# francescovidaich964/TensorNetworkForML

Hardware: AMD Instinct MI355X
Metric: sweep-steps/sec, 28x28 MNIST-shaped, bond=20, batch=5000 per GPU (higher is better)
Workload: dtype f32; 1 GPU; c3: N=784 sites, D=2, L=2, bond 20, batch 5000/GPU, softmax+full_cross_ent, trunc=fixed, L2_flag=True; pass = hand-over of one of 4 staged batches + forward + 783-step sweep; global_batch=5000, sweep_steps_per_pass=783, parallelism=dp1, distinct_batches=4

## Files before the change

include/tnml.h:

```cpp
#ifndef TNML_H
#define TNML_H

#include <stddef.h>
#include <stdint.h>

#ifdef __cplusplus
extern "C" {
#endif

typedef struct tnml_ctx tnml_ctx;

typedef enum {
  TNML_OK = 0,
  TNML_ERR_ARG = -1,
  TNML_ERR_STATE = -2,
  TNML_ERR_HIP = -3,
  TNML_ERR_NOGPU = -4,
  TNML_ERR_COMM = -5,
  TNML_ERR_SHAPE = -6,
  TNML_ERR_NONFINITE = -7
} tnml_status;

enum { TNML_ACT_LINEAR = 0, TNML_ACT_SIGMOID = 1, TNML_ACT_SOFTMAX = 2 };
enum { TNML_LOSS_MSE = 0, TNML_LOSS_CROSS_ENTROPY = 1, TNML_LOSS_FULL_CROSS_ENT = 2 };
// ... 10 lines not shown
};

const char *tnml_last_error(void);
const char *tnml_version(void);
int tnml_device_count(void);

int tnml_create(tnml_ctx **out, int N, int D, int L, int Mmax, int b_capacity, int device);
int tnml_destroy(tnml_ctx *ctx);
int tnml_synchronize(tnml_ctx *ctx);

int tnml_comm_unique_id(void *uid128);
int tnml_comm_init(tnml_ctx *ctx, int rank, int nranks, const void *uid128);
int tnml_set_comm_overlap(tnml_ctx *ctx, int on);
int tnml_comm_probe(tnml_ctx *ctx, int n_floats, int reps, double *us_per_allreduce);

int tnml_set_cores(tnml_ctx *ctx, const float *cores_flat, size_t n_floats, const int32_t *bond,
                   int l_pos);
int tnml_cores_size(tnml_ctx *ctx, size_t *n_floats);
int tnml_get_cores(tnml_ctx *ctx, float *cores_flat, size_t capacity, int32_t *bond, int *l_pos);
int tnml_scale_cores(tnml_ctx *ctx, double factor);
int tnml_get_core_slots(tnml_ctx *ctx, float *slots, size_t slots_capacity, float *label_buffer, size_t label_capacity);

int tnml_set_input(tnml_ctx *ctx, const float *X, const int32_t *y, int b);
int tnml_stage_batch(tnml_ctx *ctx, int slot, const float *X, const int32_t *y, int b);
int tnml_select_batch(tnml_ctx *ctx, int slot);
int tnml_set_labels(tnml_ctx *ctx, const int32_t *y, int b);

int tnml_forward(tnml_ctx *ctx, float *f_out);
int tnml_f_absmax(tnml_ctx *ctx, double *out);
int tnml_forward_logabsmax(tnml_ctx *ctx, double *out);
int tnml_set_f(tnml_ctx *ctx, const float *f);
int tnml_get_f(tnml_ctx *ctx, float *f_out);

int tnml_sweep(tnml_ctx *ctx, int left_dir, int n_steps, int first_of_sweep, float lr,
               float weight_dec, int l2_flag, int act_fn, int loss_fn, float T, int trunc_policy,
               float *metrics_out, float *f_out);

int tnml_update_B(tnml_ctx *ctx, const float *B_canon, int left_dir, float lr, float weight_dec, int l2_flag,
                  int act_fn, int loss_fn, float T, double *Bnew_canon, size_t capacity, float *metrics2);
int tnml_l2_term(tnml_ctx *ctx, const float *B_canon, int left_dir, float weight_dec, double *loss,
                 double *grad_canon, size_t capacity);
int tnml_svd_split(tnml_ctx *ctx, const float *mat, int rows, int cols, int m, float *US, float *SVh,
                   double *sigma);

int tnml_predict(tnml_ctx *ctx, const float *X, int b, float *f_out);

int tnml_set_any_position(tnml_ctx *ctx, int on);

enum { TNML_DATASET_FEATURES = 0, TNML_DATASET_PIXELS = 1 };
int tnml_dataset_attach(tnml_ctx *ctx, const float *data, const int32_t *labels, int n, int N, int D, int form);
int tnml_dataset_detach(tnml_ctx *ctx);
int tnml_dataset_size(tnml_ctx *ctx);
int tnml_select_indices(tnml_ctx *ctx, const int32_t *idx, int b);
int tnml_predict_indices(tnml_ctx *ctx, const int32_t *idx, int b, float *f_out);
int tnml_eval_indices(tnml_ctx *ctx, const int32_t *idx, int b, int act_fn, float T, double *out3);
int tnml_resident_metrics(tnml_ctx *ctx, int act_fn, float T, double *out3);
int tnml_dataset_read(tnml_ctx *ctx, const int32_t *idx, int b, float *X_out);

enum { TNML_WRT_FEATURES = 0, TNML_WRT_PIXELS = 1 };
int tnml_input_grad(tnml_ctx *ctx, const float *X, int b, const float *cot, float *grad_out, float *cf_out);
int tnml_input_grad_indices(tnml_ctx *ctx, const int32_t *idx, int b, const float *cot, int wrt, float *grad_out, float *cf_out);
int tnml_set_input_grad_chunk(tnml_ctx *ctx, int samples);

int tnml_core_grad(tnml_ctx *ctx, const float *X, int b, const float *cot, float *grad_flat, size_t capacity, float *cf_out);
int tnml_core_grad_indices(tnml_ctx *ctx, const int32_t *idx, int b, const float *cot, float *grad_flat, size_t capacity, float *cf_out);
int tnml_set_core_grad_chunk(tnml_ctx *ctx, int samples);

enum { TNML_OPT_SGD = 0, TNML_OPT_ADAM = 1 };
int tnml_optim_config(tnml_ctx *ctx, int kind, double momentum, double beta1, double beta2, double eps, int clip);
int tnml_optim_reset(tnml_ctx *ctx);
int tnml_gd_train_indices(tnml_ctx *ctx, const int32_t *idx, int n, int batch, float lr, float weight_dec, int act_fn, int loss_fn,
                          float T, double *metrics_out);
int tnml_gd_step(tnml_ctx *ctx, const float *X, const int32_t *y, int b, float lr, float weight_dec, int act_fn, int loss_fn, float T,
                 double *metrics3);

int tnml_set_chain_scaling(tnml_ctx *ctx, int on);
int tnml_predict_scaled(tnml_ctx *ctx, const float *X, int b, float *mant_out, int32_t *expo_out);

int tnml_set_svd_stop(tnml_ctx *ctx, double stop2);

int tnml_set_step_pipeline(tnml_ctx *ctx, int on);

int tnml_set_persistent(tnml_ctx *ctx, int on);

int tnml_set_sync_interval(tnml_ctx *ctx, int n_steps);

int tnml_set_narrow_path(tnml_ctx *ctx, int force_large);

int tnml_set_flag_handoffs(tnml_ctx *ctx, int on);

int tnml_set_chain_path(tnml_ctx *ctx, int force_plain);

int tnml_set_trunc_threshold(tnml_ctx *ctx, double threshold);

int tnml_activation(tnml_ctx *ctx, int act_fn, int loss_fn, float T, int input_is_activated,
                    float *act_out, float *lossder_out);

int tnml_get_env(tnml_ctx *ctx, int side, int site, float *out, size_t capacity, int *m);
int tnml_debug_enable(tnml_ctx *ctx, int on);
int tnml_get_step_debug(tnml_ctx *ctx, int what, double *out, size_t capacity, size_t *n);
int tnml_l_pos(tnml_ctx *ctx);
int tnml_batch(tnml_ctx *ctx);

int tnml_timer_start(tnml_ctx *ctx);
int tnml_marker(tnml_ctx *ctx, int id);
int tnml_timer_stop(tnml_ctx *ctx, double *elapsed_ms);
int tnml_profile_enable(tnml_ctx *ctx, int on);
int tnml_profile_get(tnml_ctx *ctx, int which, double *ms, long long *launches);
int tnml_profile_reset(tnml_ctx *ctx);
int tnml_get_counters(tnml_ctx *ctx, double *out8);
int tnml_svd_stats(tnml_ctx *ctx, int reset, double *out3);
int tnml_svd_stats_ex(tnml_ctx *ctx, int reset, double *out, int capacity);

int tnml_orthogonalize(tnml_ctx *ctx, double rank_tol, int32_t *bond_out, double *log_norm_out);
int tnml_compress(tnml_ctx *ctx, int m_max, double threshold, double rank_tol, int32_t *bond_out, double *sigma_out,
                  double *discarded_out, double *log_norm_out);
int tnml_bond_spectra(tnml_ctx *ctx, double rank_tol, int32_t *rank_out, double *sigma_out, double *log_norm_out);

int tnml_trunc_rank(int policy, int left_dir, int p, int N, int ml, int D, int mr, int L, int M);

#ifdef __cplusplus
}
#endif
#endif
```

tensornetworkforml_amd/_hip.py:

```python
import ctypes as C
import os

import numpy as np

_HERE = os.path.dirname(os.path.abspath(__file__))
LIB_PATH = os.environ.get('TNML_LIB', os.path.join(_HERE, 'libtnml_hip.so'))

ACT = {'linear': 0, 'sigmoid': 1, 'softmax': 2}
LOSS = {'MSE': 0, 'cross_entropy': 1, 'full_cross_ent': 2}
TRUNC = {'reference': 0, 'fixed': 1, 'adaptive': 2}
SIDE_LEFT, SIDE_RIGHT = 0, 1
DATASET_FORM = {'features': 0, 'pixels': 1}
WRT = {'features': 0, 'pixels': 1}
OPTIM = {'sgd': 0, 'adam': 1}
DBG = {'B': 0, 'dB_raw': 1, 'B_new': 2, 'sigma': 3, 'scalars': 4, 'L2_grad': 5}

SYMBOLS = [
    'tnml_last_error', 'tnml_version', 'tnml_device_count', 'tnml_create', 'tnml_destroy',
    'tnml_synchronize', 'tnml_comm_unique_id', 'tnml_comm_init', 'tnml_set_cores', 'tnml_cores_size',
    'tnml_get_cores', 'tnml_scale_cores', 'tnml_set_input', 'tnml_set_labels', 'tnml_forward', 'tnml_forward_logabsmax', 'tnml_f_absmax',
    'tnml_set_f', 'tnml_get_f', 'tnml_sweep', 'tnml_activation', 'tnml_get_env', 'tnml_debug_enable',
    'tnml_get_step_debug', 'tnml_l_pos', 'tnml_batch', 'tnml_timer_start', 'tnml_timer_stop',
    'tnml_profile_enable', 'tnml_profile_get', 'tnml_profile_reset', 'tnml_svd_stats', 'tnml_trunc_rank',
    'tnml_update_B', 'tnml_l2_term', 'tnml_svd_split', 'tnml_set_svd_stop', 'tnml_set_narrow_path', 'tnml_predict', 'tnml_set_trunc_threshold',
    'tnml_set_sync_interval', 'tnml_set_step_pipeline', 'tnml_stage_batch', 'tnml_select_batch', 'tnml_get_counters',
    'tnml_svd_stats_ex', 'tnml_set_persistent', 'tnml_set_chain_path', 'tnml_marker', 'tnml_set_comm_overlap', 'tnml_comm_probe', 'tnml_set_flag_handoffs',
    'tnml_dataset_attach', 'tnml_dataset_detach', 'tnml_dataset_size', 'tnml_select_indices', 'tnml_predict_indices', 'tnml_eval_indices',
    'tnml_resident_metrics', 'tnml_dataset_read', 'tnml_set_any_position',
    'tnml_input_grad', 'tnml_input_grad_indices', 'tnml_set_input_grad_chunk',
    'tnml_core_grad', 'tnml_core_grad_indices', 'tnml_set_core_grad_chunk',
    'tnml_optim_config', 'tnml_optim_reset', 'tnml_gd_train_indices', 'tnml_gd_step', 'tnml_get_core_slots',
    'tnml_orthogonalize', 'tnml_compress', 'tnml_bond_spectra',
    'tnml_set_chain_scaling', 'tnml_predict_scaled',
]


class TnmlError(RuntimeError):
    def __init__(self, code, msg):
        super().__init__('tnml error %d: %s' % (code, msg))
        self.code = code


_lib = None


def lib():
    global _lib
    if _lib is None:
        if not os.path.exists(LIB_PATH):
            raise RuntimeError(
                "%s is missing: build the HIP extension first (python -c 'import __graft_entry__ as g; "
                "g.build()' or make -C tensornetworkforml_amd/csrc).  There is no CPU fallback." % LIB_PATH)
        L = C.CDLL(LIB_PATH)
        L.tnml_last_error.restype = C.c_char_p
        L.tnml_version.restype = C.c_char_p
        f32p, i32p, f64p = C.POINTER(C.c_float), C.POINTER(C.c_int32), C.POINTER(C.c_double)
        vp = C.c_void_p
        L.tnml_create.argtypes = [C.POINTER(vp), C.c_int, C.c_int, C.c_int, C.c_int, C.c_int, C.c_int]
        L.tnml_destroy.argtypes = [vp]
        L.tnml_synchronize.argtypes = [vp]
        L.tnml_comm_unique_id.argtypes = [vp]
        L.tnml_comm_init.argtypes = [vp, C.c_int, C.c_int, vp]
        L.tnml_set_cores.argtypes = [vp, f32p, C.c_size_t, i32p, C.c_int]
        L.tnml_cores_size.argtypes = [vp, C.POINTER(C.c_size_t)]
        L.tnml_get_cores.argtypes = [vp, f32p, C.c_size_t, i32p, C.POINTER(C.c_int)]
        L.tnml_scale_cores.argtypes = [vp, C.c_double]
        L.tnml_set_input.argtypes = [vp, f32p, i32p, C.c_int]
        L.tnml_set_labels.argtypes = [vp, i32p, C.c_int]
        L.tnml_forward.argtypes = [vp, f32p]
        L.tnml_f_absmax.argtypes = [vp, f64p]
        L.tnml_forward_logabsmax.argtypes = [vp, f64p]
        L.tnml_set_f.argtypes = [vp, f32p]
        L.tnml_get_f.argtypes = [vp, f32p]
        L.tnml_sweep.argtypes = [vp, C.c_int, C.c_int, C.c_int, C.c_float, C.c_float, C.c_int, C.c_int,
                                 C.c_int, C.c_float, C.c_int, f32p, f32p]
        L.tnml_activation.argtypes = [vp, C.c_int, C.c_int, C.c_float, C.c_int, f32p, f32p]
        L.tnml_get_env.argtypes = [vp, C.c_int, C.c_int, f32p, C.c_size_t, C.POINTER(C.c_int)]
        L.tnml_debug_enable.argtypes = [vp, C.c_int]
        L.tnml_get_step_debug.argtypes = [vp, C.c_int, f64p, C.c_size_t, C.POINTER(C.c_size_t)]
        L.tnml_l_pos.argtypes = [vp]
        L.tnml_batch.argtypes = [vp]
        L.tnml_timer_start.argtypes = [vp]
        L.tnml_timer_stop.argtypes = [vp, f64p]
        L.tnml_profile_enable.argtypes = [vp, C.c_int]
        L.tnml_profile_get.argtypes = [vp, C.c_int, f64p, C.POINTER(C.c_longlong)]
        L.tnml_profile_reset.argtypes = [vp]
        L.tnml_svd_stats.argtypes = [vp, C.c_int, f64p]
        L.tnml_svd_stats_ex.argtypes = [vp, C.c_int, f64p, C.c_int]
        L.tnml_set_persistent.argtypes = [vp, C.c_int]
        L.tnml_trunc_rank.argtypes = [C.c_int] * 9
        L.tnml_update_B.argtypes = [vp, f32p, C.c_int, C.c_float, C.c_float, C.c_int, C.c_int, C.c_int, C.c_float,
                                    f64p, C.c_size_t, f32p]
        L.tnml_l2_term.argtypes = [vp, f32p, C.c_int, C.c_float, f64p, f64p, C.c_size_t]
        L.tnml_set_svd_stop.argtypes = [vp, C.c_double]
        L.tnml_set_narrow_path.argtypes = [vp, C.c_int]
        L.tnml_set_chain_path.argtypes = [vp, C.c_int]
        L.tnml_set_any_position.argtypes = [vp, C.c_int]
        L.tnml_marker.argtypes = [vp, C.c_int]
        L.tnml_set_comm_overlap.argtypes = [vp, C.c_int]
        L.tnml_set_flag_handoffs.argtypes = [vp, C.c_int]
        L.tnml_comm_probe.argtypes = [vp, C.c_int, C.c_int, C.POINTER(C.c_double)]
        L.tnml_predict.argtypes = [vp, f32p, C.c_int, f32p]
        L.tnml_set_trunc_threshold.argtypes = [vp, C.c_double]
        L.tnml_set_sync_interval.argtypes = [vp, C.c_int]
        L.tnml_set_step_pipeline.argtypes = [vp, C.c_int]
        L.tnml_stage_batch.argtypes = [vp, C.c_int, f32p, i32p, C.c_int]
        L.tnml_select_batch.argtypes = [vp, C.c_int]
        L.tnml_get_counters.argtypes = [vp, f64p]
        L.tnml_svd_split.argtypes = [vp, f32p, C.c_int, C.c_int, C.c_int, f32p, f32p, f64p]
        L.tnml_dataset_attach.argtypes = [vp, f32p, i32p, C.c_int, C.c_int, C.c_int, C.c_int]
        L.tnml_dataset_detach.argtypes = [vp]
        L.tnml_dataset_size.argtypes = [vp]
        L.tnml_select_indices.argtypes = [vp, i32p, C.c_int]
        L.tnml_predict_indices.argtypes = [vp, i32p, C.c_int, f32p]
        L.tnml_eval_indices.argtypes = [vp, i32p, C.c_int, C.c_int, C.c_float, f64p]
        L.tnml_resident_metrics.argtypes = [vp, C.c_int, C.c_float, f64p]
        L.tnml_dataset_read.argtypes = [vp, i32p, C.c_int, f32p]
        L.tnml_input_grad.argtypes = [vp, f32p, C.c_int, f32p, f32p, f32p]
        L.tnml_input_grad_indices.argtypes = [vp, i32p, C.c_int, f32p, C.c_int, f32p, f32p]
        L.tnml_set_input_grad_chunk.argtypes = [vp, C.c_int]
        L.tnml_core_grad.argtypes = [vp, f32p, C.c_int, f32p, f32p, C.c_size_t, f32p]
        L.tnml_core_grad_indices.argtypes = [vp, i32p, C.c_int, f32p, f32p, C.c_size_t, f32p]
        L.tnml_set_core_grad_chunk.argtypes = [vp, C.c_int]
        L.tnml_optim_config.argtypes = [vp, C.c_int, C.c_double, C.c_double, C.c_double, C.c_double, C.c_int]
        L.tnml_optim_reset.argtypes = [vp]
        L.tnml_get_core_slots.argtypes = [vp, f32p, C.c_size_t, f32p, C.c_size_t]
        L.tnml_gd_train_indices.argtypes = [vp, i32p, C.c_int, C.c_int, C.c_float, C.c_float, C.c_int, C.c_int, C.c_float, f64p]
        L.tnml_gd_step.argtypes = [vp, f32p, i32p, C.c_int, C.c_float, C.c_float, C.c_int, C.c_int, C.c_float, f64p]
        L.tnml_orthogonalize.argtypes = [vp, C.c_double, i32p, f64p]
        L.tnml_compress.argtypes = [vp, C.c_int, C.c_double, C.c_double, i32p, f64p, f64p, f64p]
        L.tnml_bond_spectra.argtypes = [vp, C.c_double, i32p, f64p, f64p]
        L.tnml_set_chain_scaling.argtypes = [vp, C.c_int]
        L.tnml_predict_scaled.argtypes = [vp, f32p, C.c_int, f32p, i32p]
        _lib = L
    return _lib


def device_count():
    return int(lib().tnml_device_count())


def _chk(rc):
    if rc != 0:
        raise TnmlError(rc, lib().tnml_last_error().decode('utf-8', 'replace'))


def _f32(a):
    return np.ascontiguousarray(a, dtype=np.float32)


def _ptr(a, ctype):
    return a.ctypes.data_as(C.POINTER(ctype))


def trunc_rank(policy, left_dir, p, N, ml, D, mr, L, M):
    return int(lib().tnml_trunc_rank(TRUNC[policy], int(left_dir), p, N, ml, D, mr, L, M))


def comm_unique_id():
    buf = (C.c_ubyte * 128)()
    _chk(lib().tnml_comm_unique_id(C.cast(buf, C.c_void_p)))
    return bytes(buf)


def core_shapes(bond, l_pos, D, L):
    N = len(bond) + 1
    shapes = []
    for i in range(N):
        ml = 1 if i == 0 else int(bond[i - 1])
        mr = 1 if i == N - 1 else int(bond[i])
        shapes.append((ml, D, mr, L) if i == l_pos else (ml, D, mr))
    return shapes
# ... 282 lines not shown

    def set_f(self, f):
        f = _f32(f)
        assert f.shape == (self.L, self.b)
        _chk(lib().tnml_set_f(self._h, _ptr(f, C.c_float)))

    def get_f(self):
        f = np.empty((self.L, self.b), dtype=np.float32)
        _chk(lib().tnml_get_f(self._h, _ptr(f, C.c_float)))
        return f

    def sweep(self, left_dir, n_steps, first_of_sweep, lr, weight_dec, L2_flag, act_fn, loss_fn, T, trunc,
              want_metrics=True, want_f=True):
        met = np.empty((n_steps, 2), dtype=np.float32) if want_metrics else None
        f = np.empty((self.L, self.b), dtype=np.float32) if want_f else None
        _chk(lib().tnml_sweep(self._h, int(bool(left_dir)), int(n_steps), int(bool(first_of_sweep)), float(lr),
                              float(weight_dec), int(bool(L2_flag)), ACT[act_fn], LOSS[loss_fn], float(T),
                              TRUNC[trunc], _ptr(met, C.c_float) if want_metrics else None,
                              _ptr(f, C.c_float) if want_f else None))
        return met, f

    def update_B(self, B, left_dir, lr, weight_dec, L2_flag, act_fn, loss_fn, T):
        shape = None
        bp = None
        if B is not None:
            B = _f32(B)
            shape = B.shape
            bp = _ptr(B, C.c_float)
        cap = 4 * max(self.M, self.D * self.L) ** 2 * self.D * self.D * self.L
        out = np.empty(cap, dtype=np.float64)
        met = np.empty(2, dtype=np.float32)
        _chk(lib().tnml_update_B(self._h, bp, int(bool(left_dir)), float(lr), float(weight_dec), int(bool(L2_flag)),
                                 ACT[act_fn], LOSS[loss_fn], float(T), _ptr(out, C.c_double), out.size,
                                 _ptr(met, C.c_float)))
        return (out[:int(np.prod(shape))].reshape(shape).copy() if shape is not None else out), met

    def l2_term(self, B, left_dir, weight_dec):
        B = _f32(B)
        grad = np.empty(B.size, dtype=np.float64)
        loss = C.c_double()
        _chk(lib().tnml_l2_term(self._h, _ptr(B, C.c_float), int(bool(left_dir)), float(weight_dec), C.byref(loss),
                                _ptr(grad, C.c_double), grad.size))
        return loss.value, grad.reshape(B.shape)

    def svd_split(self, mat, m):
        mat = _f32(mat)
        rows, cols = mat.shape
        US = np.empty((rows, int(m)), dtype=np.float32)
        SVh = np.empty((int(m), cols), dtype=np.float32)
        sig = np.empty(min(rows, cols), dtype=np.float64)
        _chk(lib().tnml_svd_split(self._h, _ptr(mat, C.c_float), rows, cols, int(m), _ptr(US, C.c_float),
                                  _ptr(SVh, C.c_float), _ptr(sig, C.c_double)))
        return US, SVh, sig

    def activation(self, act_fn, loss_fn, T, want_act=True, want_der=False, input_is_activated=False):
        a = np.empty((self.L, self.b), dtype=np.float32) if want_act else None
        d = np.empty((self.L, self.b), dtype=np.float32) if want_der else None
        _chk(lib().tnml_activation(self._h, ACT[act_fn], LOSS[loss_fn], float(T), int(bool(input_is_activated)),
                                   _ptr(a, C.c_float) if want_act else None,
                                   _ptr(d, C.c_float) if want_der else None))
        return a, d

    def loss_derivative_of_activated(self, act_fn, loss_fn, T):
        return self.activation(act_fn, loss_fn, T, want_act=False, want_der=True, input_is_activated=True)[1]

    def get_env(self, side, site):
        out = np.empty(self.b * max(self.M, self.D * self.L) * 2, dtype=np.float32)
        m = C.c_int()
        _chk(lib().tnml_get_env(self._h, int(side), int(site), _ptr(out, C.c_float), out.size, C.byref(m)))
        return out[:self.b * m.value].reshape(self.b, m.value).copy()

    def set_svd_stop(self, stop2):
        _chk(lib().tnml_set_svd_stop(self._h, float(stop2)))

    def set_trunc_threshold(self, threshold):
        _chk(lib().tnml_set_trunc_threshold(self._h, float(threshold)))

    def set_step_pipeline(self, on):
        _chk(lib().tnml_set_step_pipeline(self._h, int(on)))

    def set_persistent(self, on=True):
        _chk(lib().tnml_set_persistent(self._h, int(on)))

    def set_sync_interval(self, n_steps):
        _chk(lib().tnml_set_sync_interval(self._h, int(n_steps)))

    def set_comm_overlap(self, on=True):
        _chk(lib().tnml_set_comm_overlap(self._h, int(bool(on))))

    def comm_probe(self, n_floats, reps=200):
        v = C.c_double()
        _chk(lib().tnml_comm_probe(self._h, int(n_floats), int(reps), C.byref(v)))
        return v.value

    def set_flag_handoffs(self, on=True):
        _chk(lib().tnml_set_flag_handoffs(self._h, int(bool(on))))

    def set_chain_path(self, force_plain):
        _chk(lib().tnml_set_chain_path(self._h, int(bool(force_plain))))

    def set_any_position(self, on=True):
        _chk(lib().tnml_set_any_position(self._h, int(bool(on))))

    def set_chain_scaling(self, on=True):
        _chk(lib().tnml_set_chain_scaling(self._h, int(on)))

    def set_narrow_path(self, force_large):
        _chk(lib().tnml_set_narrow_path(self._h, int(bool(force_large))))

    def debug_enable(self, on=True):
        _chk(lib().tnml_debug_enable(self._h, int(on)))

    def step_debug(self, what):
        cap = max(4 * max(self.M, self.D * self.L) ** 2 * self.D * self.D * self.L + 64, 512)
        out = np.empty(cap, dtype=np.float64)
        n = C.c_size_t()
        _chk(lib().tnml_get_step_debug(self._h, DBG[what], _ptr(out, C.c_double), out.size, C.byref(n)))
        return out[:n.value].copy()

    @property
    def l_pos(self):
        return int(lib().tnml_l_pos(self._h))

    def synchronize(self):
        _chk(lib().tnml_synchronize(self._h))

    def marker(self, marker_id):
        _chk(lib().tnml_marker(self._h, int(marker_id)))

    def timer_start(self):
        _chk(lib().tnml_timer_start(self._h))

    def timer_stop(self):
        ms = C.c_double()
        _chk(lib().tnml_timer_stop(self._h, C.byref(ms)))
        return ms.value

    def profile_enable(self, on=True):
        _chk(lib().tnml_profile_enable(self._h, int(on)))

    def profile_reset(self):
        _chk(lib().tnml_profile_reset(self._h))

    def svd_stats(self, reset=False):
        out = (C.c_double * 4)()
        _chk(lib().tnml_svd_stats_ex(self._h, int(bool(reset)), out, 4))
        self.cholesky_steps = out[3]
        return out[0], out[1], out[2]

    def counters(self):
        out = (C.c_double * 8)()
        _chk(lib().tnml_get_counters(self._h, out))
        keys = ('sweep_steps', 'algorithmic_bytes', 'algorithmic_flops', 'forwards', 'forward_bytes', 'launches', 'pipelined_steps', 'sweep_device_ms')
        return dict(zip(keys, [float(v) for v in out]))

    def profile_get(self, which):
        ms, n = C.c_double(), C.c_longlong()
        _chk(lib().tnml_profile_get(self._h, int(which), C.byref(ms), C.byref(n)))
        return ms.value, n.value
```

tensornetworkforml_amd/csrc/kernels_narrow.hip:

```cpp
#include "tnml_internal.h"
#include "jacobi_device.h"
#include "small_gemm_device.h"
#include "wide_pipe_device.h"

namespace tnml {

__device__ inline double wave_sum_f64(double v) {
  v += dpp_f64<0xB1>(v);
  v += dpp_f64<0x4E>(v);
  v += dpp_f64<0x141>(v);
  v += dpp_f64<0x140>(v);
  const double r0 = wave_read_f64(v, 0), r1 = wave_read_f64(v, 16), r2 = wave_read_f64(v, 32), r3 = wave_read_f64(v, 48);
  return (r0 + r1) + (r2 + r3);
}

template <int BUF>
__device__ inline void block_sum3(double &a, double &b, double &c, double *scratch) {
  const int lane = threadIdx.x & 63, wave = threadIdx.x >> 6, nw = blockDim.x >> 6;
  double *s = scratch + BUF * 64;
  a = wave_sum_f64(a); b = wave_sum_f64(b); c = wave_sum_f64(c);
  if (lane == 0) { s[wave] = a; s[16 + wave] = b; s[32 + wave] = c; }
  lds_barrier();
  const int w = lane & 15;
  double ta = w < nw ? s[w] : 0.0, tb = w < nw ? s[16 + w] : 0.0, tc = w < nw ? s[32 + w] : 0.0;
// ... 32 lines not shown
  k.dVs = d; d += (size_t)ne * m;
  float *f = (float *)d;
  k.fB = f; f += Bs;
  k.fBp = f; f += Bs + (size_t)(D * h < D * g * L ? D * h : D * g * L) + 4;
  k.sLab = f; f += (size_t)h * D * s * L;
  k.sPl = f; f += (size_t)s * D * g;
  k.sCb = f; f += (size_t)r * m;
  f += (size_t)m * c;
  int *ip = (int *)f;
  k.sOrd = ip; ip += ne;
  k.sFlag = ip; ip += 8;
  k.sPi = ip; ip += ne;
  k.sPiInv = ip; ip += ne;
  k.sTail = (float *)ip; ip += kMetricSlots;
  k.sWave = ip; ip += 16;
  k.bytes = (size_t)((unsigned char *)ip - base);
  return k;
}

size_t narrow_lds_bytes(int h, int g, int s, int L, int m) {
  alignas(16) static unsigned char origin[16];
  return narrow_carve(origin, h, g, s, L, m).bytes + 16;
}

__device__ inline void narrow_helper_block(const NarrowParams &p, unsigned char *smem_raw) {
  const int tid = threadIdx.x;
  const int h = p.h, g = p.g, s = p.s, L = p.L, Bs = p.bsize;
  const int blk = blockIdx.x - 1;
  const unsigned long long t_start = __builtin_amdgcn_s_memrealtime();
  if (blk < p.nred) {
    float *part = (float *)smem_raw;
    const int el = tid & 63, chunk = tid >> 6;
    const int e = blk * 64 + el, n = Bs + kMetricSlots;
    const int per = (p.nslabs + 15) / 16;
    const int k0 = chunk * per, k1 = min(p.nslabs, k0 + per);
    float a0 = 0.f, a1 = 0.f;
    if (e < n) {
      int kk = k0;
      for (; kk + 2 <= k1; kk += 2) {
        a0 += p.slabs[(size_t)kk * p.slab_stride + e];
        a1 += p.slabs[(size_t)(kk + 1) * p.slab_stride + e];
      }
      if (kk < k1) a0 += p.slabs[(size_t)kk * p.slab_stride + e];
    }
    part[chunk * 64 + el] = a0 + a1;
    __syncthreads();
    if (chunk == 0 && e < n) {
      float t = 0.f;
#pragma unroll
      for (int c = 0; c < 16; ++c) t += part[c * 64 + el];
      __hip_atomic_store(p.red_out + e, t, __ATOMIC_RELAXED, __HIP_MEMORY_SCOPE_AGENT);
    }
  } else {
    PrepParams q{};
    q.lab = p.lab; q.pl = p.pl; q.Nh = p.Nh; q.Ng = p.Ng; q.h = h; q.g = g; q.s = s; q.L = L; q.l2_flag = p.l2_flag;
    q.prepB = p.prepB; q.prepG = p.prepG;
    q.nparts = p.pipe ? (p.wait_count - p.nred) / (kD * kD) : 1;
    prep_slice_block(q, blk - p.nred, smem_raw, true);
  }
  asm volatile("s_waitcnt vmcnt(0)" ::: "memory");
  __syncthreads();
  if (tid == 0) {
    if (p.stamps && p.counters) {
      atomicMin(p.counters + (blk < p.nred ? 4 : 5), t_start);
      atomicMax(p.counters + (blk < p.nred ? 6 : 7), __builtin_amdgcn_s_memrealtime());
    }
    __hip_atomic_fetch_add(p.sync, 1u, __ATOMIC_RELAXED, __HIP_MEMORY_SCOPE_AGENT);
  }
}

struct StepArgs : NarrowParams {
  __device__ __forceinline__ StepArgs(const NarrowParams &q) : NarrowParams(q) {}
  static constexpr int persist = 0;
};

template <class T>
struct RecField {
  const __attribute__((address_space(4))) T *a;
  __device__ __forceinline__ operator T() const { return *a; }
};
template <class T>
__device__ __forceinline__ RecField<T> rec_field(const T *field) { return RecField<T>{(const __attribute__((address_space(4))) T *)field}; }

struct PersistArgs {
  int L, h, g, s, m, bsize, l2_flag;
  float lr, wd;
  const double *Nh;
  int persist_off, Mcap;
  const unsigned *pready; unsigned pwant;
  unsigned *abort_flag;
  const float *zred; int zsize;
  const float *prepRaw; float *prepB; double *prepG;
  float *Bnew;
  unsigned *flag; unsigned token;
  double chol_thr, svd_stop2;
  double *stamps;
  RecField<float *> out_behind, out_ahead;
  RecField<int> ob_s_h, ob_s_d, ob_s_m, oa_s_m, oa_s_d, oa_s_g, write_ahead;
  RecField<double *> Nh_new, Apub;
  RecField<float *> metrics;
  RecField<unsigned long long *> counters;
  RecField<int *> status;
  RecField<unsigned *> aflag, coreflag;
  RecField<unsigned> coretoken;
  static constexpr int D = kD, fused = 0, prep_ready = 0, pipe = 1, persist = 1, z_first = 0, z_rows = 0, stop_after_update = 0, left_dir = 0;
  static constexpr int wait_count = 0;
  static constexpr unsigned zpoll_want = 0, done_val = 0;
  static constexpr double trunc_thr = 0.0;
  static constexpr const float *red = nullptr, *Bdirect = nullptr;
  static constexpr const double *Ng = nullptr;
  static constexpr double *dbg = nullptr;
  static constexpr int *m_out = nullptr;
  unsigned *sync = nullptr, *done_flag = nullptr;
  const unsigned *zpoll_flag = nullptr;
  CoreView lab{}, pl{}, zcore{};

  __device__ __forceinline__ explicit PersistArgs(const NarrowParams *rec)
      : out_behind(rec_field(&rec->out_behind)), out_ahead(rec_field(&rec->out_ahead)),
        ob_s_h(rec_field(&rec->ob_s_h)), ob_s_d(rec_field(&rec->ob_s_d)), ob_s_m(rec_field(&rec->ob_s_m)),
        oa_s_m(rec_field(&rec->oa_s_m)), oa_s_d(rec_field(&rec->oa_s_d)), oa_s_g(rec_field(&rec->oa_s_g)),
        write_ahead(rec_field(&rec->write_ahead)), Nh_new(rec_field(&rec->Nh_new)), Apub(rec_field(&rec->Apub)),
        metrics(rec_field(&rec->metrics)), counters(rec_field(&rec->counters)), status(rec_field(&rec->status)),
        aflag(rec_field(&rec->aflag)), coreflag(rec_field(&rec->coreflag)), coretoken(rec_field(&rec->coretoken)) {
    const auto *r = (const __attribute__((address_space(4))) NarrowParams *)rec;
    L = r->L; h = r->h; g = r->g; s = r->s; m = r->m; bsize = r->bsize; l2_flag = r->l2_flag;
    lr = r->lr; wd = r->wd; Nh = r->Nh; persist_off = r->persist_off; Mcap = r->Mcap;
    pready = r->pready; pwant = r->pwant; abort_flag = r->abort_flag; zred = r->zred; zsize = r->zsize;
    prepRaw = r->prepRaw; prepB = r->prepB; prepG = r->prepG; Bnew = r->Bnew; flag = r->flag; token = r->token;
    chol_thr = r->chol_thr; svd_stop2 = r->svd_stop2; stamps = r->stamps;
  }
};

template <class NP>
__device__ __forceinline__ bool narrow_body(const NP &p, unsigned char *smem_raw) {
  __builtin_assume(p.h >= 1 && p.h <= 64 && p.g >= 1 && p.g <= 64 && p.s >= 1 && p.s <= 128 && p.m >= 1 && p.m <= 64);
  __builtin_assume(p.L >= 1 && p.L <= 2048 && p.bsize >= 1 && p.bsize <= 8192);
  const NarrowCarve k = narrow_carve(smem_raw, p.h, p.g, p.s, p.L, p.m);
  int tid_step = threadIdx.x;
  if (p.persist) {
    asm volatile("" : "+v"(tid_step));
    __builtin_assume(tid_step >= 0 && tid_step < kNarrowThreads);
  }
  const int tid = tid_step, NT = kNarrowThreads;
  const int wave_u = __builtin_amdgcn_readfirstlane(tid >> 6);
  const int D = kD, h = p.h, g = p.g, s = p.s, L = p.L, m = p.m, Bs = p.bsize;
  auto ldred = [&](int e) -> float {
    return (p.fused && !p.pipe) ? __hip_atomic_load(p.red + e, __ATOMIC_RELAXED, __HIP_MEMORY_SCOPE_AGENT) : p.red[e];
  };
  if (p.zpoll_flag) {
    if (tid == 0) {
      bool ok = false;
      for (int spin = 0; spin < (1 << 22) && !ok; ++spin) {
        ok = (int)(__hip_atomic_load(p.zpoll_flag, __ATOMIC_RELAXED, __HIP_MEMORY_SCOPE_AGENT) - p.zpoll_want) >= 0;
        if (!ok) __builtin_amdgcn_s_sleep(16);
      }
      if (!ok) atomicOr(p.status, 64);
    }
    __syncthreads();
    __builtin_amdgcn_fence(__ATOMIC_ACQUIRE, "agent");
  }
  if (p.pipe && !p.persist && tid == 0)
    for (int i = 0; i < kMetricSlots; ++i) k.sTail[i] = p.zred[p.zsize + i];
  auto ldtail = [&](int i) -> float { return p.pipe ? k.sTail[i] : ldred(p.bsize + i); };
  const int r = D * h, c = D * g * L;
  const bool short_rows = (r <= c);
  const int n = short_rows ? r : c, ne = n + (n & 1), len = short_rows ? c : r;

  unsigned long long t_c0 = 0, t_r0 = 0, t_c1 = 0, t_c2 = 0, t_c2b = 0, t_c2c = 0;
  unsigned long long t_p[5] = {0, 0, 0, 0, 0};
#define TNML_STAMP(i) if (p.stamps && tid == 0) t_p[i] = __builtin_amdgcn_s_memtime()
  if (p.stamps && tid == 0) { t_c0 = __builtin_amdgcn_s_memtime(); t_r0 = __builtin_amdgcn_s_memrealtime(); }
  const int RWz = kD * kD * p.g * p.L;
  const bool fast0 = p.pipe && !p.persist && (size_t)p.z_rows * RWz + (size_t)p.z_rows * h <= (size_t)((float *)k.sOrd - k.fBp) &&
                     Bs <= 8 * NT && p.z_rows * RWz <= 16 * NT && p.z_rows * h <= 4 * NT && h * h <= 2 * NT && g * g <= 2 * NT;
  const PersistLds PL = persist_lds(smem_raw + p.persist_off, p.Mcap);
  float *sRaw = k.fBp;
  if (p.persist) {
    if (tid == 0) {
      const int bad = spin_wait_ge(p.pready, p.pwant, p.abort_flag, 1);
      if (bad == 1) { atomicOr(p.status, 4); __hip_atomic_store(p.abort_flag, 1u, __ATOMIC_RELAXED, __HIP_MEMORY_SCOPE_AGENT); }
      k.sFlag[3] = bad;
    }
    lds_barrier();
    if (k.sFlag[3]) return true;
    if (p.stamps && tid == 0) { p.stamps[20] = (double)(__builtin_amdgcn_s_memtime() - t_c0); p.stamps[28] = (double)(t_r0 & ((1ull << 40) - 1)); p.stamps[29] = (double)(__builtin_amdgcn_s_memrealtime() & ((1ull << 40) - 1)); }
    if (tid < kMetricSlots) k.sTail[tid] = ld_sc1(p.zred + p.zsize + tid);
    for (int e = tid; e < h * h; e += NT) k.dNh[e] = p.Nh ? PL.Nh[e] : 1.0;
    const __amdgpu_buffer_rsrc_t rR = sc1_rsrc(p.prepRaw), rB = sc1_rsrc(p.prepB), rG = sc1_rsrc(p.prepG);
    tn_uvec4 qr[2], qb[2], qg[4];
#pragma unroll
    for (int u = 0; u < 2; ++u) { const int e = 4 * (tid + u * NT); if (e < Bs) { qr[u] = ld_sc1_b128(rR, (unsigned)e * 4u); qb[u] = ld_sc1_b128(rB, (unsigned)e * 4u); } }
#pragma unroll
    for (int u = 0; u < 4; ++u) { const int e = 2 * (tid + u * NT); if (p.l2_flag && e < Bs) qg[u] = ld_sc1_b128(rG, (unsigned)e * 8u); }
#pragma unroll
    for (int u = 0; u < 2; ++u) { const int e = 4 * (tid + u * NT); if (e < Bs) { *reinterpret_cast<tn_uvec4 *>(sRaw + e) = qr[u]; *reinterpret_cast<tn_uvec4 *>(k.fB + e) = qb[u]; } }
#pragma unroll
    for (int u = 0; u < 4; ++u) { const int e = 2 * (tid + u * NT); if (p.l2_flag && e < Bs) *reinterpret_cast<tn_uvec4 *>(k.dG + e) = qg[u]; }
  }
  float *sZ = k.fBp, *sZc = sZ + (size_t)p.z_rows * RWz;
  if (fast0) {
    const int zr = p.z_rows, nz = p.z_first ? 0 : zr * RWz, nzc = p.z_first ? 0 : zr * h;
    const float *zc = p.zcore.base;
    float4 rz[4], rb[2];
    double2 rg[4];
    float rc[4];
    double rnh[2], rng[2];
#pragma unroll
    for (int u = 0; u < 4; ++u) { const int e = 4 * (tid + u * NT); rz[u] = e < nz ? *reinterpret_cast<const float4 *>(p.zred + e) : make_float4(0.f, 0.f, 0.f, 0.f); }
// ... 172 lines not shown
    sumB += fabs(bv);
    sumD += fabs(dv);
  }
  block_sum3<0>(sumB, sumD, l2, k.dRed);

  double factor = (double)p.lr;
  if (sumD > sumB) factor = (double)p.lr * (sumB / sumD);
  const bool bad = !isfinite(sumD) || !isfinite(sumB);
  if ((c & 3) == 0) {
    const float inv_c = 1.0f / (float)c;
    const __amdgpu_buffer_rsrc_t rN = sc1_rsrc(p.Bnew);
    for (int e = 4 * tid; e < Bs; e += 4 * NT) {
      const int row = (int)(((float)e + 0.5f) * inv_c), x = e - row * c;
      const float4 b4 = *reinterpret_cast<const float4 *>(k.fB + e);
      const double2 g01 = *reinterpret_cast<const double2 *>(k.dG + e), g23 = *reinterpret_cast<const double2 *>(k.dG + e + 2);
      float4 v;
      v.x = (float)((double)b4.x + factor * g01.x); v.y = (float)((double)b4.y + factor * g01.y);
      v.z = (float)((double)b4.z + factor * g23.x); v.w = (float)((double)b4.w + factor * g23.y);
      *reinterpret_cast<float4 *>(k.fB + e) = v;
      float *bp = k.fBp + row * (c + 1) + x;
      bp[0] = v.x; bp[1] = v.y; bp[2] = v.z; bp[3] = v.w;
      if (p.flag) {
        tn_uvec4 o; o.x = __float_as_uint(v.x); o.y = __float_as_uint(v.y); o.z = __float_as_uint(v.z); o.w = __float_as_uint(v.w);
        st_sc1_b128(rN, (unsigned)(4 * e), o);
      } else {
        *reinterpret_cast<float4 *>(p.Bnew + e) = v;
      }
      if (p.dbg) { double *dd = p.dbg + 2 * (size_t)Bs + e; dd[0] = v.x; dd[1] = v.y; dd[2] = v.z; dd[3] = v.w; }
    }
  } else {
    for (int row = wave_u; row < r; row += NT >> 6)
      for (int x = tid & 63; x < c; x += 64) {
        const int e = row * c + x;
        const float v = (float)((double)k.fB[e] + factor * k.dG[e]);
        k.fB[e] = v;
        k.fBp[row * (c + 1) + x] = v;
        if (p.flag) st_sc1(p.Bnew + e, v); else p.Bnew[e] = v;
        if (p.dbg) p.dbg[2 * (size_t)Bs + e] = (double)v;
      }
  }
  if (p.flag) asm volatile("s_waitcnt vmcnt(0)" ::: "memory");
  if (tid == 0) {
    if (bad) atomicOr(p.status, 1);
    if (p.dbg) {
      double *sc = p.dbg + 4 * (size_t)Bs + kDbgSigma;
      sc[0] = (double)p.wd * l2;
      sc[1] = sumB;
      sc[2] = sumD;
    }
  }
  lds_barrier();
  if (p.flag && tid == 0) __hip_atomic_store(p.flag, p.token, __ATOMIC_RELAXED, __HIP_MEMORY_SCOPE_AGENT);
  if (p.stop_after_update) {
    if (tid == 0 && p.metrics) {
      const double cnt = (double)ldtail(3);
      const double inv = cnt > 0 ? 1.0 / cnt : 0.0;
      p.metrics[0] = (float)((double)ldtail(0) * inv);
      p.metrics[1] = (float)((double)ldtail(1) * inv / (double)L);
    }
    return false;
  }

  TNML_STAMP(3);
  double *G0 = k.Z, *G1 = k.Z + ne * ne, *V0 = k.Z + 2 * ne * ne;
  double g_tr = 0.0, g_dg2 = 0.0, g_off2 = 0.0;
  auto gram_phase = [&]() {
    double a_tr = 0.0, a_dg2 = 0.0, a_off2 = 0.0;
    double *P0 = G0, *P1 = G1, *P2 = V0, *P3 = k.Z + 3 * ne * ne;
    const int lane = tid & 63, wave = wave_u, rr = lane & 15, qq = lane >> 4;
    const int tm = (n + 15) >> 4, ntile_g = (tm * (tm + 1)) >> 1;
    const int gshift = ntile_g * 4 <= (NT >> 6) ? 2 : (ntile_g * 2 <= (NT >> 6) ? 1 : (ntile_g <= (NT >> 6) ? 0 : 2));
    const int gsplit = 1 << gshift;
    const int kchunk = ((len + gsplit - 1) / gsplit + 3) & ~3;
    const int wave_s = wave;
    const float *Wb = short_rows ? k.fBp : k.fB;
    const int rs = short_rows ? c + 1 : 1, cs = short_rows ? 1 : c;
    const int nitems = ntile_g * gsplit;
    for (int item = wave_s; item < nitems; item += NT >> 6) {
      const int ks = item & (gsplit - 1);
      int t = item >> gshift, ti = 0, rowlen = tm;
      while (t >= rowlen) { t -= rowlen; ++ti; --rowlen; }
      const int tj = ti + t;
      const int i0 = ti << 4, j0 = tj << 4;
      const bool va = i0 + rr < n, vb = j0 + rr < n;
      const float *pa = Wb + min(i0 + rr, n - 1) * rs, *pb = Wb + min(j0 + rr, n - 1) * rs;
      const int k_lo = ks * kchunk, k_hi = min(len, k_lo + kchunk);
      dvec4 acc0 = {0.0, 0.0, 0.0, 0.0}, acc1 = {0.0, 0.0, 0.0, 0.0};
      for (int k0 = k_lo; k0 < k_hi; k0 += 16) {
        float fa[4], fb[4];
#pragma unroll
        for (int u = 0; u < 4; ++u) {
          const int kc = min(k0 + 4 * u + qq, k_hi - 1) * cs;
          fa[u] = pa[kc];
          fb[u] = pb[kc];
        }
#pragma unroll
        for (int u = 0; u < 4; ++u) {
          const bool vk = k0 + 4 * u + qq < k_hi;
          const double av = (va && vk) ? (double)fa[u] : 0.0, bv = (vb && vk) ? (double)fb[u] : 0.0;
          if (k0 + 4 * u < k_hi) {
            if (u & 1) acc1 = __builtin_amdgcn_mfma_f64_16x16x4f64(av, bv, acc1, 0, 0, 0);
            else acc0 = __builtin_amdgcn_mfma_f64_16x16x4f64(av, bv, acc0, 0, 0, 0);
          }
        }
      }
      const dvec4 acc = acc0 + acc1;
      const int j = j0 + rr;
      double *Pk = P0 + (size_t)ks * ne * ne;
#pragma unroll
      for (int reg = 0; reg < 4; ++reg) {
        const int i = i0 + qq + 4 * reg;
        if (i < ne && j < ne) Pk[i * ne + j] = (i < n && j < n) ? acc[reg] : 0.0;
      }
    }
    lds_barrier();
    for (int i = wave_u; i < ne; i += NT >> 6)
      for (int j = tid & 63; j < ne; j += 64)
        if (i <= j) {
          const int e = i * ne + j;
          double v = P0[e];
          if (gsplit > 1) v += P1[e];
          if (gsplit > 2) v = (v + P2[e]) + P3[e];
          P0[e] = v;
          if (i < j) { G0[j * ne + i] = v; a_off2 += 2.0 * v * v; }
          else { a_tr += v; a_dg2 += v * v; }
        }
    g_tr = a_tr; g_dg2 = a_dg2; g_off2 = a_off2;
  };
  gram_phase();
  const int np = ne / 2;
  for (int pos = tid; pos < ne; pos += NT) {
    const int kq = pos >> 1;
    int nxt;
    if (pos & 1) nxt = (kq == 0) ? (np > 1 ? 2 : 1) : 2 * (kq - 1) + 1;
    else nxt = (kq == 0) ? 0 : (kq == np - 1 ? 2 * kq + 1 : 2 * (kq + 1));
    k.sPi[pos] = nxt;
    k.sPiInv[nxt] = pos;
  }
  TNML_STAMP(4);
  double tr = 0.0, off2 = 0.0;
  int sc_exp = 0;
  auto scale_phase = [&]() {
    block_sum3<1>(g_tr, g_dg2, g_off2, k.dRed);
    tr = g_tr; off2 = g_off2;
    sc_exp = (tr > 0.0 && isfinite(tr)) ? __builtin_amdgcn_frexp_exp(tr) : 0;
    for (int i = wave_u; i < ne; i += NT >> 6)
      for (int j = tid & 63; j < ne; j += 64) G0[i * ne + j] = __builtin_amdgcn_ldexp(G0[i * ne + j], -sc_exp);
    lds_barrier();
  };
  scale_phase();
  const bool chol_possible = p.chol_thr > 0.0 && n > 4;

  constexpr int kVR = 2;
  const int gpw = 64 / np;
  const int vr = ((np + gpw - 1) / gpw + (np * (np + 1) / 2 + 127) / 128 <= (NT >> 6) - 1) ? 1 : 2;
  const int NVW = (np + vr * gpw - 1) / (vr * gpw);
  const int nwork = (NT >> 6) - 1, wrank = wave_u - 1;
  const int nGw = min(nwork - NVW, (np * (np + 1) / 2 + 63) / 64);
  const int NW = nGw * 64;
  const int gtid = (wrank - NVW) * 64 + (tid & 63);
  const int vlane = tid & 63, vgrp = vlane / np, vQ = vlane - vgrp * np;
  const bool isVwave = wrank >= 0 && wrank < NVW;
  const int vP0 = (wrank * gpw + vgrp) * vr;
  const bool vLaneOk = isVwave && vgrp < gpw;
  constexpr int MAXI = 2;
  const int nG = np * (np + 1) / 2;
  bool itValid[MAXI], itDiag[MAXI];
  int itSrc[MAXI], itCsQ[MAXI], itCsP[MAXI], itD11[MAXI], itD12[MAXI], itD21[MAXI], itD22[MAXI];
#pragma unroll
  for (int u = 0; u < MAXI; ++u) {
    const int it = gtid + u * NW;
    itValid[u] = wrank >= NVW && gtid < NW && it < nG;
    int P = 0, Q = 0;
    if (itValid[u]) {
      int rem = it;
      while (rem >= np - P) { rem -= np - P; ++P; }
      Q = P + rem;
    }
    const int c1 = k.sPi[2 * Q], c2 = k.sPi[2 * Q + 1];
    const int o1 = k.sPi[2 * P], o2 = k.sPi[2 * P + 1];
    itSrc[u] = (2 * P) * ne + 2 * Q;
    itCsQ[u] = 4 * Q; itCsP[u] = 4 * P;
    itDiag[u] = P == Q;
    itD11[u] = min(o1, c1) * ne + max(o1, c1); itD12[u] = min(o1, c2) * ne + max(o1, c2);
    itD21[u] = min(o2, c1) * ne + max(o2, c1); itD22[u] = min(o2, c2) * ne + max(o2, c2);
  }
  const double abs2 = kJacobiAbs * kJacobiAbs;
  const bool isParam = tid < np;
  int pa = 0, pb = 1;
  if (isParam) { pa = k.sPiInv[2 * tid]; pb = k.sPiInv[2 * tid + 1]; }
  const int pA = pa >> 1, ra = pa & 1, pB = pb >> 1, rb = pb & 1;
  const int oAd = (2 * pA) * ne + 2 * pA, oAb = (2 * pA + 1) * ne + 2 * pA + 1;
  const int oBd = (2 * pB) * ne + 2 * pB, oBb = (2 * pB + 1) * ne + 2 * pB + 1;
  const int oR0 = pA <= pB ? (2 * pA) * ne + 2 * pB : (2 * pB) * ne + 2 * pA, oR1 = oR0 + ne;

  if (p.stamps && tid == 0) t_c1 = __builtin_amdgcn_s_memtime();
  double *Lm = k.Z + 3 * ne * ne;
  const double cthr = n >= 32 ? p.chol_thr : fmax(p.chol_thr, kCholThrSmall);
  const bool use_chol = __builtin_amdgcn_readfirstlane((int)(chol_possible && off2 > cthr * cthr * tr * tr)) != 0;
  if (use_chol) {
    for (int e = tid; e < ne * ne; e += NT) Lm[e] = 0.0;
    constexpr int kCholPer = 3;
    const int hn = n / 2, npairs = n * hn;
    int ei[kCholPer], ej[kCholPer];
#pragma unroll
    for (int u = 0; u < kCholPer; ++u) {
      const int pe = (tid - 64) + u * (NT - 64);
      const bool ok = tid >= 64 && pe < npairs;
      ei[u] = ok ? pe / hn : -1;
      ej[u] = ok ? 2 * (pe - (pe / hn) * hn) : 0;
    }
    double dgi = (tid < n) ? G0[tid * ne + tid] : -1.0;
    auto pivot_search = [&](int slot) {
      const float key = (float)dgi;
      const float mx = wave_max_f32(key);
      const unsigned long long hit = __ballot(key == mx);
      const int jp = (mx > 1e-26f && hit) ? __ffsll((long long)hit) - 1 : -1;
      const double piv = wave_read_f64(dgi, jp < 0 ? 0 : jp);
      double inv0 = (double)__builtin_amdgcn_rsqf((float)piv);
      inv0 = inv0 * fma(-0.5 * piv, inv0 * inv0, 1.5);
      if (tid == 0) { k.sFlag[4 + slot] = jp; k.dRed[61 + slot] = inv0; }
    };
    if (wave_u == 0) pivot_search(0);
    for (int kc = 0; kc < n; ++kc) {
      lds_barrier();
      const double *src = (kc & 1) ? G1 : G0;
      double *dst = (kc & 1) ? G0 : G1;
      const int jp = __builtin_amdgcn_readfirstlane(k.sFlag[4 + (kc & 1)]);
      if (jp < 0) break;
      const double inv = k.dRed[61 + (kc & 1)];
      if (wave_u == 0) {
        const double l = (tid < n && dgi >= 0.0) ? src[jp * ne + tid] * inv : 0.0;
        if (tid < n) Lm[kc * ne + tid] = l;
        dgi = (tid == jp) ? -1.0 : (dgi >= 0.0 ? dgi - l * l : dgi);
        if (kc + 1 < n) pivot_search((kc + 1) & 1);
      } else {
#pragma unroll
        for (int u = 0; u < kCholPer; ++u)
          if (ei[u] >= 0) {
            const double li = src[jp * ne + ei[u]] * inv;
            const double2 c2 = *reinterpret_cast<const double2 *>(src + jp * ne + ej[u]);
            double2 v = *reinterpret_cast<const double2 *>(src + ei[u] * ne + ej[u]);
            v.x -= li * (c2.x * inv);
            v.y -= li * (c2.y * inv);
            *reinterpret_cast<double2 *>(dst + ei[u] * ne + ej[u]) = v;
          }
      }
    }
    lds_barrier();
    mm_lds(1, n, n, n, Lm, 0, ne, 1, Lm, 0, 1, ne, [&](int, int a, int b, double v) { G0[a * ne + b] = v; });
    lds_barrier();
    for (int i = wave_u; i < n; i += NT >> 6)
      for (int j = tid & 63; j < i; j += 64) G0[i * ne + j] = G0[j * ne + i];
    lds_barrier();
  }

  double vb[kVR][4];
#pragma unroll
  for (int r = 0; r < kVR; ++r) {
    const double one = (vP0 + r == vQ) ? 1.0 : 0.0;
    vb[r][0] = one; vb[r][1] = 0.0; vb[r][2] = 0.0; vb[r][3] = one;
  }
  int sweeps = 0, converged = 0;
  double *Gc = G0, *Gn = G1;
  auto kept_scale = [&](const double *G) -> double {
    const int i = tid & 63;
    const double li = i < n ? G[i * ne + i] : 0.0;
    for (int j = wave_u; j < n; j += NT >> 6) {
      const double lj = G[j * ne + j];
      const int rank = __popcll(__ballot(i < n && ((li > lj) || (li == lj && i < j))));
      if (i == 0 && rank == m - 1) k.dRed[60] = lj;
    }
    lds_barrier();
    const double lm = kKeptFrac * fmax(k.dRed[60], 0.0);
    return lm * lm;
  };

  int cur = 0;
  double kept2 = 0.0;
  const float kept_lo = 1e-36f;
  auto publish = [&](double *o, const RotT &r, int applied) {
    *reinterpret_cast<double2 *>(o) = make_double2((double)r.t, (double)r.c0);
    *reinterpret_cast<float2 *>(o + 2) = make_float2(r.t, r.c0);
    if (r.level >= 2) k.sFlag[6 + (applied & 1)] = applied + 1;
  };
  int round_idx = 0, last_big1 = 0;
  auto jacobi_round = [&]() {
        const double *csc = k.dCS + cur * np * 4;
        const int big_slot = k.sFlag[6 + (round_idx & 1)];
        if (isParam) {
          const float2 fA = *reinterpret_cast<const float2 *>(csc + 4 * pA + 2);
          const float2 fB = *reinterpret_cast<const float2 *>(csc + 4 * pB + 2);
          const double2 dA = *reinterpret_cast<const double2 *>(Gc + oAd);
          const double bA = Gc[oAb];
          const double2 dB = *reinterpret_cast<const double2 *>(Gc + oBd);
          const double bB = Gc[oBb];
          double2 r0, r1;
          if (pA < pB) {
            r0 = *reinterpret_cast<const double2 *>(Gc + oR0);
            r1 = *reinterpret_cast<const double2 *>(Gc + oR1);
          } else if (pA > pB) {
            const double2 s0 = *reinterpret_cast<const double2 *>(Gc + oR0);
            const double2 s1 = *reinterpret_cast<const double2 *>(Gc + oR1);
            r0 = make_double2(s0.x, s1.x);
            r1 = make_double2(s0.y, s1.y);
          } else {
            r0 = dA;
            r1 = make_double2(dA.y, bA);
          }
          const float tA = fA.x, cA = fA.y, sA = fA.x * fA.y, tB = fB.x, cB = fB.y, sB = fB.x * fB.y;
          const float aAx = (float)dA.x, aAy = (float)dA.y, aAb = (float)bA, aBx = (float)dB.x, aBy = (float)dB.y, aBb = (float)bB;
          const float q0x = (float)r0.x, q0y = (float)r0.y, q1x = (float)r1.x, q1y = (float)r1.y;
          const float na = ra ? fmaf(tA, aAy, aAb) : fmaf(-tA, aAy, aAx);
          const float nb = rb ? fmaf(tB, aBy, aBb) : fmaf(-tB, aBy, aBx);
          const float h0 = ra ? fmaf(sA, q0x, cA * q1x) : fmaf(cA, q0x, -sA * q1x);
          const float h1 = ra ? fmaf(sA, q0y, cA * q1y) : fmaf(cA, q0y, -sA * q1y);
          const float ng = rb ? fmaf(sB, h0, cB * h1) : fmaf(cB, h0, -sB * h1);
          const RotT r = jacobi_rot_f32(na, nb, ng, fmaxf((float)kept2, kept_lo), (float)abs2, (float)p.svd_stop2);
          publish(k.dCS + ((cur ^ 1) * np + tid) * 4, r, round_idx + 1);
        }
        if (isVwave) {
          const double2 tc = *reinterpret_cast<const double2 *>(csc + 4 * (vLaneOk ? vQ : 0));
          const double cq = tc.y * rot_corr(tc.x, tc.y);
#pragma unroll
          for (int r = 0; r < kVR; ++r) {
            if (r >= vr) break;
            const double n11 = cq * fma(-tc.x, vb[r][1], vb[r][0]), n12 = cq * fma(tc.x, vb[r][0], vb[r][1]);
            const double n21 = cq * fma(-tc.x, vb[r][3], vb[r][2]), n22 = cq * fma(tc.x, vb[r][2], vb[r][3]);
            if (np > 1) {
              const double t1 = dpp_f64<0x138>(n11), t2 = dpp_f64<0x138>(n21);
              const double b1 = dpp_f64<0x138>(n12), b2 = dpp_f64<0x138>(n22);
              const double c1 = dpp_f64<0x130>(n12), c2 = dpp_f64<0x130>(n22);
              vb[r][0] = vQ == 0 ? n11 : (vQ == 1 ? b1 : t1);
              vb[r][2] = vQ == 0 ? n21 : (vQ == 1 ? b2 : t2);
              vb[r][1] = vQ == np - 1 ? n11 : c1;
              vb[r][3] = vQ == np - 1 ? n21 : c2;
            } else {
              vb[r][0] = n11; vb[r][1] = n12; vb[r][2] = n21; vb[r][3] = n22;
            }
          }
        }
#pragma unroll
        for (int u = 0; u < MAXI; ++u) {
          if (!itValid[u]) continue;
          const double2 tq = *reinterpret_cast<const double2 *>(csc + itCsQ[u]);
          const double2 tp = *reinterpret_cast<const double2 *>(csc + itCsP[u]);
          const double *src = Gc + itSrc[u];
          const double2 r0 = *reinterpret_cast<const double2 *>(src);
          double2 r1 = *reinterpret_cast<const double2 *>(src + ne);
          if (itDiag[u]) r1.x = r0.y;
          const double a11 = fma(-tp.x, r1.x, r0.x), a12 = fma(-tp.x, r1.y, r0.y);
          const double a21 = fma(tp.x, r0.x, r1.x), a22 = fma(tp.x, r0.y, r1.y);
          const double b11 = fma(-tq.x, a12, a11), b12 = fma(tq.x, a11, a12);
          const double b21 = fma(-tq.x, a22, a21), b22 = fma(tq.x, a21, a22);
          const double c00 = tp.y * tq.y, corr = rot_corr(tp.x, tp.y) * rot_corr(tq.x, tq.y);
          double n11 = (b11 * c00) * corr, n12 = (b12 * c00) * corr, n21 = (b21 * c00) * corr, n22 = (b22 * c00) * corr;
          if (itDiag[u] && tq.x != 0.0) { n12 = 0.0; n21 = 0.0; }
          Gn[itD11[u]] = n11; Gn[itD12[u]] = n12;
          if (!itDiag[u]) Gn[itD21[u]] = n21;
          Gn[itD22[u]] = n22;
        }
        lds_barrier();
        double *tsw = Gc; Gc = Gn; Gn = tsw;
        cur ^= 1;
        last_big1 = max(last_big1, big_slot);
        ++round_idx;
  };
  if (n > 1) {
    kept2 = kept_scale(Gc);
    if (tid == 0) { k.sFlag[6] = 0; k.sFlag[7] = 0; }
    if (isParam) {
      const double2 top = *reinterpret_cast<const double2 *>(Gc + (2 * tid) * ne + 2 * tid);
      const RotT r = jacobi_rot_f32((float)top.x, (float)Gc[(2 * tid + 1) * ne + 2 * tid + 1], (float)top.y,
                                    fmaxf((float)kept2, kept_lo), (float)abs2, (float)p.svd_stop2);
      publish(k.dCS + (cur * np + tid) * 4, r, 0);
    }
    lds_barrier();
    for (; sweeps < kJacobiMaxSweeps && !converged; ++sweeps) {
      for (int rnd = 0; rnd < ne - 1; ++rnd) {
        jacobi_round();
        if (round_idx - __builtin_amdgcn_readfirstlane(last_big1) >= ne - 1) { converged = 1; break; }
      }
      if (!converged) kept2 = kept_scale(Gc);
    }
  } else {
    converged = 1;
  }
  double *V = V0;
  if (vLaneOk) {
#pragma unroll
    for (int r = 0; r < kVR; ++r) {
      const int P = vP0 + r;
      if (r < vr && P < np) {
        *reinterpret_cast<double2 *>(V + (2 * P) * ne + 2 * vQ) = make_double2(vb[r][0], vb[r][1]);
        *reinterpret_cast<double2 *>(V + (2 * P + 1) * ne + 2 * vQ) = make_double2(vb[r][2], vb[r][3]);
      }
    }
  }
  if (p.stamps && tid == 0) t_c2 = __builtin_amdgcn_s_memtime();

  for (int j = tid; j < n; j += NT) k.dLam[j] = __builtin_amdgcn_ldexp(fmax(Gc[j * ne + j], 0.0), sc_exp);
  lds_barrier();
  if (use_chol) {
    for (int j = tid; j < n; j += NT) {
      const double ls = Gc[j * ne + j];
      k.dSq[j] = ls > 1e-300 ? 1.0 / sqrt(ls) : 0.0;
    }
    lds_barrier();
    mm_lds(1, n, n, n, Lm, 0, 1, ne, V, 0, ne, 1, [&](int, int i, int j, double v) { Gn[i * ne + j] = v * k.dSq[j]; });
    V = Gn;
    lds_barrier();
  }
  for (int j = wave_u; j < n; j += NT >> 6) {
    const int i = tid & 63;
    const double lj = k.dLam[j];
    const double li = i < n ? k.dLam[i] : 0.0;
    const int rank = __popcll(__ballot(i < n && ((li > lj) || (li == lj && i < j))));
    if (i == 0) {
      k.sOrd[rank] = j;
      if (p.dbg) p.dbg[4 * (size_t)Bs + rank] = sqrt(lj);
    }
  }
  if (tid == 0) {
    if (p.counters) {
      atomicAdd(p.counters, (unsigned long long)sweeps);
      atomicAdd(p.counters + 1, 1ull);
      atomicAdd(p.counters + 2, (unsigned long long)round_idx);
      if (use_chol) atomicAdd(p.counters + 3, 1ull);
    }
    if (!converged) atomicOr(p.status, 2);
    if (p.dbg) {
      double *sc = p.dbg + 4 * (size_t)Bs + kDbgSigma;
      sc[3] = (double)sweeps;
      sc[4] = (double)n;
    }
  }
  lds_barrier();

  if (p.stamps && tid == 0) t_c2b = __builtin_amdgcn_s_memtime();
  int mk = m, ob_s_h = p.ob_s_h, ob_s_d = p.ob_s_d, oa_s_d = p.oa_s_d, oa_s_g = p.oa_s_g;
  const int ob_s_m = p.ob_s_m, oa_s_m = p.oa_s_m;
  float *const out_behind = p.out_behind, *const out_ahead = p.out_ahead;
  double *const Nh_new = p.Nh_new;
  if (p.trunc_thr > 0.0) {
    if (tid == 0) {
      double tot = 0.0;
      for (int j = 0; j < n; ++j) tot += sqrt(k.dLam[k.sOrd[j]]);
      double cum = 0.0;
      int idx = 0;
      bool found = false;
      for (int j = 0; j < n && !found; ++j) {
        cum += sqrt(k.dLam[k.sOrd[j]]);
        if (cum / tot > p.trunc_thr) { idx = j; found = true; }
      }
      const int me = min(m, idx + 1);
      k.sFlag[2] = me;
      if (p.m_out) *p.m_out = me;
    }
    lds_barrier();
    mk = k.sFlag[2];
    if (!p.left_dir) { ob_s_h = D * mk; ob_s_d = mk; } else { oa_s_d = mk * L; oa_s_g = D * mk * L; }
  }
  auto st_behind = [&](int off, float v) { if (p.persist) st_sc1(out_behind + off, v); else out_behind[off] = v; };
  const double lam_max = k.dLam[k.sOrd[0]];
  for (int sp = tid; sp < mk; sp += NT) {
    const double lam = k.dLam[k.sOrd[sp]];
    const bool ok = lam > 1e-300 && lam > 1e-30 * lam_max;
    const double sq = ok ? sqrt(sqrt(lam)) : 0.0;
    k.dSq[sp] = sq;
    k.dSq[ne + sp] = ok ? 1.0 / sq : 0.0;
  }
  lds_barrier();
  for (int kk = wave_u; kk < n; kk += NT >> 6)
   for (int sp = tid & 63; sp < mk; sp += 64) {
    const int j = k.sOrd[sp];
    const double vq = V[kk * ne + j];
    const float v = (float)(vq * k.dSq[sp]);
    k.dVs[kk * mk + sp] = vq * k.dSq[ne + sp];
    if (short_rows) {
      k.sCb[kk * mk + sp] = v;
      if (p.persist) PL.Ad[kk * mk + sp] = vq * k.dSq[sp];
      st_behind((kk / D) * ob_s_h + (kk % D) * ob_s_d + sp * ob_s_m, v);
    } else {
      const int l = kk % L, q = kk / L;
      out_ahead[sp * oa_s_m + (q / g) * oa_s_d + (q % g) * oa_s_g + l] = v;
    }
   }
  lds_barrier();
  const int DM = D * mk;
  auto store_T2 = [&](int, int i, int j, double v) { k.dT2[i * DM + j] = v; };
  if (short_rows) {
    int slot = 0;
    if (!p.persist || p.write_ahead)
      slot = mm_lds(L, D * g, mk, n, k.fB, 1, L, c, k.dVs, 0, mk, 1,
           [&](int l, int qq, int sp, double acc) {
             const int dk1 = qq >= g ? 1 : 0;
             out_ahead[__mul24(sp, oa_s_m) + dk1 * oa_s_d + __mul24(qq - dk1 * g, oa_s_g) + l] = (float)acc;
           });
    if (Nh_new) mm_lds(1, h, DM, h, k.dNh, 0, h, 1, k.sCb, 0, DM, 1, store_T2, false, slot);
  } else {
    mm_lds(D, h, mk, n, k.fBp, c + 1, D * (c + 1), 1, k.dVs, 0, mk, 1,
           [&](int dk, int h_, int sp, double acc) {
             const float v = (float)acc;
             k.sCb[__mul24(h_ * D + dk, mk) + sp] = v;
             if (p.persist) PL.Ad[__mul24(h_ * D + dk, mk) + sp] = acc;
             st_behind(__mul24(h_, ob_s_h) + dk * ob_s_d + __mul24(sp, ob_s_m), v);
           });
  }
  lds_barrier();
  if (p.persist) {
    if (wave_u == (NT >> 6) - 1) {
      const int ln = tid & 63;
      const __amdgpu_buffer_rsrc_t rP = sc1_rsrc(p.Apub);
      for (int e = ln; e < (r * mk) >> 1; e += 64) st_sc1_b128(rP, (unsigned)e * 16u, pack_d2(PL.Ad[2 * e], PL.Ad[2 * e + 1]));
      for (int e = ln; e < (mk + 1) >> 1; e += 64) {
        const double i0 = k.dSq[ne + 2 * e], i1 = 2 * e + 1 < mk ? k.dSq[ne + 2 * e + 1] : 0.0;
        st_sc1_b128(rP, (unsigned)(r * mk + 2 * e) * 8u, pack_d2(i0 * i0, i1 * i1));
      }
      asm volatile("s_waitcnt vmcnt(0)" ::: "memory");
      if (ln == 0) { unsigned *const aflag = p.aflag; __hip_atomic_store(aflag, (unsigned)p.coretoken, __ATOMIC_RELAXED, __HIP_MEMORY_SCOPE_AGENT); }
    }
  }

  if (p.stamps && tid == 0) t_c2c = __builtin_amdgcn_s_memtime();
  if (Nh_new) {
    if (!short_rows) {
      mm_lds(1, h, DM, h, k.dNh, 0, h, 1, k.sCb, 0, DM, 1, store_T2);
      lds_barrier();
    }
    mm_lds(1, mk, mk, h * D, k.sCb, 0, 1, mk, k.dT2, 0, mk, 1,
           [&](int, int i, int j, double v) {
             Nh_new[i * mk + j] = v;
             if (p.persist) PL.Nh[i * mk + j] = v;
           });
    if (p.persist) {
      lds_barrier();
      const __amdgpu_buffer_rsrc_t rP = sc1_rsrc(p.Apub);
      const int oN = persist_pub_off(r * mk, mk), nn2 = mk * mk;
      for (int e = tid; e < (nn2 + 1) >> 1; e += NT)
        st_sc1_b128(rP, (unsigned)(oN + 2 * e) * 8u, pack_d2(PL.Nh[2 * e], 2 * e + 1 < nn2 ? PL.Nh[2 * e + 1] : 0.0));
    }
  }

  if (p.stamps && tid == 0) {
    const unsigned long long t_c3 = __builtin_amdgcn_s_memtime(), t_r3 = __builtin_amdgcn_s_memrealtime();
    p.stamps[0] = (double)(t_c1 - t_c0); p.stamps[1] = (double)(t_c2 - t_c1); p.stamps[2] = (double)(t_c3 - t_c2);
    p.stamps[3] = (double)(t_r3 - t_r0); p.stamps[4] = (double)sweeps; p.stamps[5] = (double)n;
    p.stamps[50] = (double)round_idx;
    for (int i = 0; i < 5; ++i) p.stamps[9 + i] = (double)(t_p[i] - (i ? t_p[i - 1] : t_c0));
    p.stamps[6] = (double)(t_c2b - t_c2); p.stamps[7] = (double)(t_c2c - t_c2b); p.stamps[8] = (double)(t_c3 - t_c2c);
  }

  if (tid == 0 && p.metrics) {
    const double cnt = (double)ldtail(3);
    const double inv = cnt > 0 ? 1.0 / cnt : 0.0;
    p.metrics[0] = (float)((double)ldtail(0) * inv);
    p.metrics[1] = (float)((double)ldtail(1) * inv / (double)L);
    if (ldtail(2) != 0.f) atomicOr(p.status, 1);
  }
  if (p.persist) {
    asm volatile("s_waitcnt vmcnt(0)" ::: "memory");
    lds_barrier();
    if (tid == 0) { unsigned *const coreflag = p.coreflag; __hip_atomic_store(coreflag, (unsigned)p.coretoken, __ATOMIC_RELAXED, __HIP_MEMORY_SCOPE_AGENT); }
  }
  if (p.done_flag) {
    asm volatile("s_waitcnt vmcnt(0)" ::: "memory");
    __syncthreads();
    if (wave_u == 0) {
      __builtin_amdgcn_fence(__ATOMIC_RELEASE, "agent");
      if (tid == 0) __hip_atomic_store(p.done_flag, p.done_val, __ATOMIC_RELAXED, __HIP_MEMORY_SCOPE_AGENT);
    }
  }
  return false;
}

__global__ __launch_bounds__(kNarrowThreads) void narrow_step_kernel(NarrowParams p) {
  extern __shared__ __attribute__((aligned(16))) unsigned char smem_raw[];
  if (p.fused && blockIdx.x > 0) { narrow_helper_block(p, smem_raw); return; }
  narrow_body(StepArgs(p), smem_raw);
}

void launch_narrow(const NarrowParams &p, size_t lds_bytes, hipStream_t st) {
  hipLaunchKernelGGL(narrow_step_kernel, dim3(p.fused ? 1 + p.wait_count : 1), dim3(kNarrowThreads), lds_bytes, st, p);
}

__global__ __launch_bounds__(kNarrowThreads) void step_pipe_kernel(NarrowParams p, WidePipeParams w) {
  extern __shared__ __attribute__((aligned(16))) unsigned char smem_raw[];
  const int blk = blockIdx.x;
  if (blk >= w.wg0) { wide_pipe_block(WidePipeArgs<0>(w), (float *)smem_raw); return; }
  if (blk > 0) { narrow_helper_block(p, smem_raw); return; }
  narrow_body(StepArgs(p), smem_raw);
}

void launch_step_pipe(const NarrowParams &p, const WidePipeParams &w, size_t lds_bytes, hipStream_t st) {
  const int grid = w.wg0 + (w.do_f || w.do_z || w.do_ext ? w.nwide : 0);
  hipLaunchKernelGGL(step_pipe_kernel, dim3(grid), dim3(kNarrowThreads), lds_bytes, st, p, w);
}

void launch_step_pipe_update(const NarrowParams &p, const WidePipeParams &w, size_t lds_bytes, hipStream_t st) {
  hipLaunchKernelGGL(step_pipe_kernel, dim3(w.wg0), dim3(kNarrowThreads), lds_bytes, st, p, w);
}

__device__ inline void st_sc1_elem(float *p, float v) { st_sc1(p, v); }
__device__ inline void st_sc1_elem(double *p, double v) { __hip_atomic_store(p, v, __ATOMIC_RELAXED, __HIP_MEMORY_SCOPE_AGENT); }
template <class T>
__device__ inline void st_sc1_rows(T *dst, const T *stage, int rows, int srs, int RW, int c0, int nc) {
  constexpr int V = 16 / (int)sizeof(T);
  if (nc <= 0) return;
  const __amdgpu_buffer_rsrc_t rD = sc1_rsrc(dst);
  const int ns = (nc + 2 * V - 2) / V;
  for (int it = threadIdx.x; it < rows * ns; it += kNarrowThreads) {
    const int i = it / ns, q = it - i * ns;
    const int gs = i * RW + c0, ge = gs + nc, lo = (gs & ~(V - 1)) + q * V;
    if (lo >= ge) continue;
    const T *src = stage + i * srs + (lo - gs);
    if (lo >= gs && lo + V <= ge) {
      T v[V];
#pragma unroll
      for (int u = 0; u < V; ++u) v[u] = src[u];
      tn_uvec4 w;
      __builtin_memcpy(&w, v, 16);
      st_sc1_b128(rD, (unsigned)lo * (unsigned)sizeof(T), w);
    } else {
#pragma unroll
      for (int u = 0; u < V; ++u) if (lo + u >= gs && lo + u < ge) st_sc1_elem(dst + lo + u, src[u]);
    }
  }
}

template <class HP>
__device__ __forceinline__ bool persist_helper_block(const HP &t, int hid, int nH, unsigned char *smem_raw, bool do_part2) {
  int tid_step = threadIdx.x;
  asm volatile("" : "+v"(tid_step));
  __builtin_assume(tid_step >= 0 && tid_step < kNarrowThreads);
  const int tid = tid_step, NT = kNarrowThreads;
  const int D = kD, zr = t.zr, s = t.s, g = t.g, L = t.L, h = t.h;
  const int DG = D * g, RW = D * DG * L;
  __shared__ int sBad;
  auto give_up = [&](int bad) {
    if (bad == 1) { atomicOr(t.status, 4); __hip_atomic_store(t.abort_flag, 1u, __ATOMIC_RELAXED, __HIP_MEMORY_SCOPE_AGENT); }
    sBad = bad;
  };
  if (!do_part2) {
    const int R1 = zr * D, per = (R1 + nH - 1) / nH, r0 = min(R1, hid * per), nr = min(R1, r0 + per) - r0;
    float *sW = (float *)smem_raw;
    float *sP = sW + (((size_t)per * s * L + 3) & ~(size_t)3);
    double *sNg = (double *)(sP + (((size_t)s * DG + 3) & ~(size_t)3));
    double *oT = sNg + (((size_t)g * g + 1) & ~(size_t)1);
    double *oN = oT + (size_t)per * DG * L;
    if (tid == 0) give_up(t.want ? spin_wait_ge(t.flag, t.want, t.abort_flag) : 0);
    lds_barrier();
    if (sBad) return true;
    if (nr > 0) {
      const int nW = nr * s * L;
      if (t.W) {
        const float *Wsrc = t.W + (size_t)r0 * s * L;
        for (int e = tid; e < nW; e += NT) sW[e] = ld_sc1(Wsrc + e);
      } else {
        for (int e = tid; e < nW; e += NT) {
          const int l = e % L, q = e / L, s_ = q % s, d = r0 + q / s;
          sW[e] = t.lab.base[d * t.lab.s_d + s_ * t.lab.s_out + l];
        }
      }
      for (int e = tid; e < s * DG; e += NT) {
        const int g_ = e % g, q = e / g, d = q % D, s_ = q / D;
        sP[e] = t.pl.base[s_ * t.pl.s_in + d * t.pl.s_d + g_ * t.pl.s_out];
      }
      if (t.l2_flag) for (int e = tid; e < g * g; e += NT) sNg[e] = t.Ng ? t.Ng[e] : 1.0;
      lds_barrier();
      mm_lds(L, nr, DG, s, sW, 1, s * L, L, sP, 0, DG, 1, [&](int l, int row, int col, double v) { oT[(row * DG + col) * L + l] = v; });
      lds_barrier();
      if (t.l2_flag)
        mm_lds(L, nr * D, g, g, oT, 1, g * L, L, sNg, 0, g, 1, [&](int l, int i, int j, double v) { oN[(i * g + j) * L + l] = v; });
      const int nT = nr * DG * L;
      double *Tdst = t.T + (size_t)r0 * DG * L, *Ndst = t.TN + (size_t)r0 * DG * L;
      for (int e = tid; e < nT; e += NT) __hip_atomic_store(Tdst + e, oT[e], __ATOMIC_RELAXED, __HIP_MEMORY_SCOPE_AGENT);
      if (t.l2_flag) {
        lds_barrier();
        for (int e = tid; e < nT; e += NT) __hip_atomic_store(Ndst + e, oN[e], __ATOMIC_RELAXED, __HIP_MEMORY_SCOPE_AGENT);
      }
    }
    asm volatile("s_waitcnt vmcnt(0)" ::: "memory");
    lds_barrier();
    if (tid == 0) __hip_atomic_fetch_add(t.tcnt, 1u, __ATOMIC_RELAXED, __HIP_MEMORY_SCOPE_AGENT);
    return false;
  }
  const int cw = (RW + nH - 1) / nH, c0 = min(RW, hid * cw), nc = min(RW, c0 + cw) - c0;
  const int cw2 = 2 * cw;
  double *sA = (double *)smem_raw;
  double *sIv = sA + (((size_t)zr * h + 1) & ~(size_t)1);
  double *sNh = sIv + ((h + 1) & ~1);
  double *sS = sNh + (((size_t)h * h + 1) & ~(size_t)1);
  float *sOut = (float *)(sS + persist_helper_ss_doubles(zr, h, cw));
  double *sP2 = (double *)sOut + (size_t)h * cw;
  float *sZf = (float *)(sP2 + (size_t)h * cw);
  float *sAff = sZf + (size_t)zr * cw;
  double *hst = (t.stamps && hid == 0 && tid == 0) ? t.stamps : nullptr;
  double *hst2 = (t.stamps && hid == 0) ? t.stamps : nullptr;
  auto rt = []() { return (double)(__builtin_amdgcn_s_memrealtime() & ((1ull << 40) - 1)); };
  if (tid == 0) { if (hst) hst[22] = rt(); give_up(spin_wait_ge(t.tcnt, (unsigned)nH, t.abort_flag)); if (hst) hst[30] = rt(); }
  lds_barrier();
  if (sBad) return true;
  for (int e = tid; e < zr * nc; e += NT) {
    const int i = e / nc, cc = e - i * nc;
    const size_t src = (size_t)i * RW + c0 + cc;
    sS[i * cw2 + cc] = __hip_atomic_load(t.T + src, __ATOMIC_RELAXED, __HIP_MEMORY_SCOPE_AGENT);
    sS[i * cw2 + cw + cc] = t.l2_flag ? __hip_atomic_load(t.TN + src, __ATOMIC_RELAXED, __HIP_MEMORY_SCOPE_AGENT) : 0.0;
  }
  lds_barrier();
  if (tid == 0) { give_up(spin_wait_ge(t.zready, t.zwant, t.abort_flag)); if (hst) hst[24] = rt(); }
  lds_barrier();
  if (sBad) return true;
  for (int e = tid; e < zr * nc; e += NT) {
    const int i = e / nc, cc = e - i * nc;
    sZf[i * cw + cc] = ld_sc1(t.Z + (size_t)i * RW + c0 + cc);
  }
  lds_barrier();
  if (tid == 0) { give_up(t.awant ? spin_wait_ge(t.aflag, t.awant, t.abort_flag) : 0); if (hst) hst[23] = rt(); }
  lds_barrier();
  if (sBad) return true;
  if (t.awant) {
    const __amdgpu_buffer_rsrc_t rP = sc1_rsrc(t.Apub);
    const int n1 = persist_pub_off(zr * h, h) >> 1, nA = (zr * h) >> 1;
    for (int e = tid; e < n1; e += NT) {
      const tn_uvec4 q = ld_sc1_b128(rP, (unsigned)e * 16u);
      *reinterpret_cast<tn_uvec4 *>(sA + 2 * e) = q;
      if (e < nA) { const dvec2_t a = __builtin_bit_cast(dvec2_t, q); sAff[2 * e] = (float)a[0]; sAff[2 * e + 1] = (float)a[1]; }
    }
  } else if (tid == 0) {
    sA[0] = 1.0; sAff[0] = 1.f; sIv[0] = 1.0; sNh[0] = 1.0;
  }
  lds_barrier();
  if (hst) hst[25] = rt();
  if (nc > 0) {
    mm_lds_f32(h, nc, zr, sAff, 1, h, sZf, cw, 1, [&](int i, int j, float v) { sOut[i * cw + j] = v; });
    const int slot = (((h + 15) >> 4) * ((nc + 15) >> 4)) & ((NT >> 6) - 1);
    mm_lds(1, h, t.l2_flag ? 2 * cw : cw, zr, sA, 0, 1, h, sS, 0, cw2, 1,
           [&](int, int i, int j, double v) {
             if (j < cw) { if (j < nc) sOut[(h + i) * cw + j] = (float)(v * sIv[i]); }
             else sP2[i * cw + (j - cw)] = v * sIv[i];
           }, false, slot);
  }
  if (t.l2_flag) {
    if (t.awant && (tid >> 6) == (NT >> 6) - 1) {
      const int ln = tid & 63;
      int bad = 0;
      if (ln == 0) { if (hst2) hst2[31] = rt(); bad = spin_wait_ge(t.nflag, t.awant, t.abort_flag); give_up(bad); if (hst2) hst2[21] = rt(); }
      if (!__builtin_amdgcn_readfirstlane(bad)) {
        const __amdgpu_buffer_rsrc_t rP = sc1_rsrc(t.Apub);
        const int oN = persist_pub_off(zr * h, h), nq = (h * h + 1) >> 1;
        for (int e0 = ln; e0 < nq; e0 += 4 * 64) {
          tn_uvec4 q[4];
#pragma unroll
          for (int u = 0; u < 4; ++u) if (e0 + 64 * u < nq) q[u] = ld_sc1_b128(rP, (unsigned)(oN + 2 * (e0 + 64 * u)) * 8u);
#pragma unroll
          for (int u = 0; u < 4; ++u) if (e0 + 64 * u < nq) *reinterpret_cast<tn_uvec4 *>(sNh + 2 * (e0 + 64 * u)) = q[u];
        }
      }
    }
  }
  lds_barrier();
  if (t.l2_flag && sBad) return true;
  st_sc1_rows(t.prepRaw, sOut, h, cw, RW, c0, nc);
  st_sc1_rows(t.prepB, sOut + (size_t)h * cw, h, cw, RW, c0, nc);
  if (t.l2_flag) {
    if (nc > 0) {
      mm_lds(1, h, nc, h, sNh, 0, 1, h, sP2, 0, cw, 1, [&](int, int i, int j, double v) { sS[i * cw + j] = v; });
    }
    lds_barrier();
    st_sc1_rows(t.prepG, sS, h, cw, RW, c0, nc);
  }
  if (hst) hst[26] = rt();
  asm volatile("s_waitcnt vmcnt(0)" ::: "memory");
  lds_barrier();
  if (tid == 0) __hip_atomic_fetch_add(t.pcnt, 1u, __ATOMIC_RELAXED, __HIP_MEMORY_SCOPE_AGENT);
  if (hst) hst[27] = rt();
  return false;
}

__global__ __launch_bounds__(kNarrowThreads) void sweep_persist_kernel(const PersistStep *__restrict__ steps_g, int n_steps, int nH) {
  extern __shared__ __attribute__((aligned(16))) unsigned char smem_raw[];
  const int blk = blockIdx.x;
  if (blk == 0) {
#pragma nounroll
    for (int k = 0; k < n_steps; ++k)
      if (narrow_body(PersistArgs(&steps_g[k].n), smem_raw)) break;
  } else if (blk <= nH) {
#pragma nounroll
    for (int ph = 0; ph < 2 * n_steps; ++ph) {
      PersistHelperParams t;
      __builtin_memcpy(&t, &steps_g[ph >> 1].t, sizeof t);
      lds_barrier();
      if (persist_helper_block(t, blk - 1, nH, smem_raw, (ph & 1) != 0)) break;
    }
  } else {
#pragma nounroll
    for (int it = 0; it <= n_steps; ++it) {
      WidePipeParams w;
      __builtin_memcpy(&w, &steps_g[it == 0 ? n_steps : it - 1].w, sizeof w);
      lds_barrier();
      if (wide_pipe_block(WidePipeArgs<1>(w), (float *)smem_raw)) break;
    }
  }
}

void launch_sweep_persist(const PersistStep *steps_dev, int n_steps, int n_helpers, int grid, size_t lds_bytes, hipStream_t st) {
  hipLaunchKernelGGL(sweep_persist_kernel, dim3(grid), dim3(kNarrowThreads), lds_bytes, st, steps_dev, n_steps, n_helpers);
}

__global__ __launch_bounds__(kNarrowThreads) void persist_update_kernel(const PersistStep *__restrict__ steps_g, int n_steps) {
  extern __shared__ __attribute__((aligned(16))) unsigned char smem_raw[];
#pragma nounroll
  for (int k = 0; k < n_steps; ++k)
    if (narrow_body(PersistArgs(&steps_g[k].n), smem_raw)) break;
}
__global__ __launch_bounds__(kNarrowThreads) void persist_helper_kernel(const PersistStep *__restrict__ steps_g, int n_steps, int nH) {
  extern __shared__ __attribute__((aligned(16))) unsigned char smem_raw[];
#pragma nounroll
  for (int ph = 0; ph < 2 * n_steps; ++ph) {
    PersistHelperParams t;
    __builtin_memcpy(&t, &steps_g[ph >> 1].t, sizeof t);
    lds_barrier();
    if (persist_helper_block(t, (int)blockIdx.x, nH, smem_raw, (ph & 1) != 0)) break;
  }
}
__global__ __launch_bounds__(kNarrowThreads) void persist_batch_kernel(const PersistStep *__restrict__ steps_g, int n_steps) {
  extern __shared__ __attribute__((aligned(16))) unsigned char smem_raw[];
#pragma nounroll
  for (int it = 0; it <= n_steps; ++it) {
    WidePipeParams w;
    __builtin_memcpy(&w, &steps_g[it == 0 ? n_steps : it - 1].w, sizeof w);
    w.wg0 = 0;
    lds_barrier();
    if (wide_pipe_block(WidePipeArgs<1>(w), (float *)smem_raw)) break;
  }
}
void launch_sweep_persist_split(const PersistStep *steps_dev, int n_steps, int n_helpers, int n_wide, size_t lds_update, size_t lds_helper,
                                size_t lds_wide, hipStream_t st_update, hipStream_t st_helper, hipStream_t st_wide) {
  hipLaunchKernelGGL(persist_batch_kernel, dim3(n_wide), dim3(kNarrowThreads), lds_wide, st_wide, steps_dev, n_steps);
  hipLaunchKernelGGL(persist_helper_kernel, dim3(n_helpers), dim3(kNarrowThreads), lds_helper, st_helper, steps_dev, n_steps, n_helpers);
  hipLaunchKernelGGL(persist_update_kernel, dim3(1), dim3(kNarrowThreads), lds_update, st_update, steps_dev, n_steps);
}

__global__ __launch_bounds__(256) void norm_chain_kernel(const NormChainSite *__restrict__ sites, int n_sites,
                                                         const float *__restrict__ cores,
                                                         double *__restrict__ env_base, int Mmax) {
  extern __shared__ __attribute__((aligned(16))) unsigned char smem_raw[];
  double *env = (double *)smem_raw;
  double *T = env + (size_t)Mmax * Mmax;
  float *sA = (float *)(T + (size_t)Mmax * kD * Mmax);
  const int tid = threadIdx.x;
  if (tid == 0) env[0] = 1.0;
  __syncthreads();
  for (int i = 0; i < n_sites; ++i) {
    const NormChainSite cs = sites[i];
    const int ni = cs.n_in, no = cs.n_out;
    for (int e = tid; e < ni * kD * no; e += 256) {
      const int o = e % no, q = e / no;
      sA[e] = cores[cs.core_off + (q / kD) * cs.s_in + (q % kD) * cs.s_d + o * cs.s_out];
    }
    __syncthreads();
    for (int e = tid; e < ni * kD * no; e += 256) {
      const int o = e % no, q = e / no;
      const int d = q % kD, in = q / kD;
      double acc = 0.0;
      for (int j = 0; j < ni; ++j) acc += env[in * ni + j] * (double)sA[(j * kD + d) * no + o];
      T[e] = acc;
    }
    __syncthreads();
    for (int e = tid; e < no * no; e += 256) {
      const int o2 = e % no, o1 = e / no;
      double acc = 0.0;
      for (int q = 0; q < ni * kD; ++q) acc += (double)sA[q * no + o1] * T[q * no + o2];
      env_base[cs.env_out_off + e] = acc;
      env[e] = acc;
    }
    __syncthreads();
  }
}

void launch_norm_chain(const NormChainSite *sites_dev, int n_sites, const float *cores, double *env_base,
                       int Mmax, hipStream_t st) {
  size_t lds = ((size_t)Mmax * Mmax + (size_t)Mmax * kD * Mmax) * sizeof(double) +
               (size_t)Mmax * kD * Mmax * sizeof(float);
  hipLaunchKernelGGL(norm_chain_kernel, dim3(1), dim3(256), lds, st, sites_dev, n_sites, cores, env_base, Mmax);
}

}
```

tensornetworkforml_amd/csrc/san/hip_stub.cpp:

```cpp
#include <hip/hip_runtime.h>
#include <rccl/rccl.h>
#include <sys/mman.h>
#include <cstdarg>
#include <cstdio>
#include <cstdlib>
#include <cstring>
#include <map>
#include <string>
#include <vector>
#include <cxxabi.h>
#include "../tnml_internal.h"
#include "../wide_pipe_device.h"
#include "../grad_chain_device.h"

using namespace tnml;

namespace san {
static char *g_base = nullptr;
static size_t g_used = 0;
static constexpr size_t kArena = (size_t)1 << 38, kGap = (size_t)1 << 20;
static std::map<uintptr_t, size_t> &alloc_map() { static auto *m = new std::map<uintptr_t, size_t>; return *m; }
static std::map<const void *, std::string> &kernel_map() { static auto *m = new std::map<const void *, std::string>; return *m; }
static std::map<std::string, long> &launch_map() { static auto *m = new std::map<std::string, long>; return *m; }
#define g_alloc alloc_map()
#define g_kernels kernel_map()
#define g_launches launch_map()
static long g_checked_ptrs = 0, g_allreduces = 0;
static long g_alloc_calls = 0, g_fail_call = 0;
static bool alloc_fails() {
  if (++g_alloc_calls != g_fail_call) return false;
  g_fail_call = 0;
  return true;
}
static const char *g_ctx = "";

[[noreturn]] static void die(const char *fmt, ...) {
  va_list ap;
  va_start(ap, fmt);
  fprintf(stderr, "san-stub VIOLATION [%s]: ", g_ctx);
  vfprintf(stderr, fmt, ap);
  fprintf(stderr, "\n");
  va_end(ap);
  abort();
}
static bool in_arena(const void *p) { return g_base && (const char *)p >= g_base && (const char *)p < g_base + kArena; }
static void need(const void *p, size_t bytes, const char *what) {
  ++g_checked_ptrs;
  if (!p) die("%s: null pointer (%zu bytes wanted)", what, bytes);
  if (!in_arena(p)) die("%s: %p is not device memory", what, p);
  auto it = g_alloc.upper_bound((uintptr_t)p);
  if (it == g_alloc.begin()) die("%s: %p below every allocation", what, p);
  --it;
  const uintptr_t lo = it->first, hi = lo + it->second;
  if ((uintptr_t)p + bytes > hi) die("%s: [%p, +%zu) leaves its allocation [%p, +%zu) by %zu bytes", what, p, bytes, (void *)lo, it->second, (uintptr_t)p + bytes - hi);
}
static void opt(const void *p, size_t bytes, const char *what) { if (p) need(p, bytes, what); }
static void scan(const void *blk, size_t bytes, const char *what) {
  for (size_t o = 0; o + 8 <= bytes; o += 8) {
    void *v;
    memcpy(&v, (const char *)blk + o, 8);
    if (in_arena(v)) need(v, 1, what);
  }
}
static size_t view_extent(const CoreView &v, int tail) {
  return (size_t)(v.n_in - 1) * v.s_in + (size_t)(kD - 1) * v.s_d + (size_t)(v.n_out - 1) * v.s_out + tail;
}

static void check_wide(const WideParams &p, int nblk, bool f_only = false) {
  const size_t bp = p.b_pad;
  if (p.b < 1 || p.b > p.b_pad || p.b_pad % 64) die("WideParams: b %d b_pad %d", p.b, p.b_pad);
  scan(&p, sizeof p, "WideParams");
  if (f_only) {
    opt(p.Hprev, (size_t)p.hp * bp * 4, "WideParams.Hprev"); opt(p.Gprev, (size_t)p.gp * bp * 4, "WideParams.Gprev");
    need(p.x_km1, bp * kD * 4, "WideParams.x_km1"); need(p.x_k, bp * kD * 4, "WideParams.x_k");
    need(p.Bprev, (size_t)p.hp * kD * kD * p.gp * p.L * 4, "WideParams.Bprev"); need(p.f, (size_t)p.L * bp * 4, "WideParams.f");
    if ((size_t)nblk * kTS != bp) die("f_only grid %d x %d samples != b_pad %zu", nblk, kTS, bp);
    return;
  }
  opt(p.x_km1, bp * kD * 4, "WideParams.x_km1"); need(p.x_k, bp * kD * 4, "WideParams.x_k"); need(p.x_kp1, bp * kD * 4, "WideParams.x_kp1");
  if (p.do_ext && !p.first_ext) need(p.Hprev, (size_t)p.hp * bp * 4, "WideParams.Hprev");
  opt(p.Hcur, (size_t)p.h * bp * 4, "WideParams.Hcur");
  if (p.do_f) { opt(p.Gprev, (size_t)p.gp * bp * 4, "WideParams.Gprev"); need(p.Bprev, (size_t)p.hp * kD * kD * p.gp * p.L * 4, "WideParams.Bprev"); }
  opt(p.Gcur, (size_t)p.g * bp * 4, "WideParams.Gcur");
  if (p.do_ext) need(p.ext_core.base, view_extent(p.ext_core, 1) * 4, "WideParams.ext_core");
  need(p.y, bp * 4, "WideParams.y"); need(p.f, (size_t)p.L * bp * 4, "WideParams.f");
  if (p.slabs) {
    if (p.bsize != p.h * kD * kD * p.g * p.L) die("WideParams.bsize %d != h D D g L", p.bsize);
    if (p.slab_stride < p.bsize + kMetricSlots) die("WideParams.slab_stride %d < bsize + tail %d", p.slab_stride, p.bsize + kMetricSlots);
    need(p.slabs, (size_t)nblk * p.slab_stride * 4, "WideParams.slabs");
  }
}
struct BigExtArgs { const float *Eprev, *x_km1, *x_k; CoreView A; int b_pad; float *Ecur, *Pk; };
static void check_big_ext(const BigExtArgs &a, size_t shm) {
  const CoreView &A = a.A;
  const size_t bp = (size_t)a.b_pad;
  need(a.Eprev, (size_t)A.n_in * bp * 4, "big_ext: E_{k-1}");
  need(a.x_km1, bp * kD * 4, "big_ext: x_{k-1}"); need(a.x_k, bp * kD * 4, "big_ext: x_k");
  need(A.base, view_extent(A, 1) * 4, "big_ext: core");
  need(a.Ecur, (size_t)A.n_out * bp * 4, "big_ext: E_k"); need(a.Pk, (size_t)kD * A.n_out * bp * 4, "big_ext: P'_k");
  if (shm < (size_t)A.n_in * kD * ((A.n_out + 3) & ~3) * 4) die("big_ext: %zu bytes of LDS for a %d x %d x %d core", shm, A.n_in, kD, A.n_out);
}
static void check_narrow(const NarrowParams &p) {
  scan(&p, sizeof p, "NarrowParams");
  if (p.bsize != p.h * kD * kD * p.g * p.L) die("NarrowParams.bsize %d != h D D g L (%d %d %d)", p.bsize, p.h, p.g, p.L);
  const int rows = p.h * kD, cols = kD * p.g * p.L;
  if (p.m < 1 || p.m > (rows < cols ? rows : cols) * p.L) die("NarrowParams.m %d for a %d x %d tensor", p.m, rows, cols);
  if (!p.pipe) opt(p.red, (size_t)(p.bsize + kMetricSlots) * 4, "NarrowParams.red");
  if (!p.Bdirect) { need(p.lab.base, view_extent(p.lab, p.L) * 4, "NarrowParams.lab"); need(p.pl.base, view_extent(p.pl, 1) * 4, "NarrowParams.pl"); }
  else need(p.Bdirect, (size_t)p.bsize * 4, "NarrowParams.Bdirect");
  opt(p.Nh, (size_t)p.h * p.h * 8, "NarrowParams.Nh"); opt(p.Ng, (size_t)p.g * p.g * 8, "NarrowParams.Ng");
// ... 234 lines not shown
  if (g.y != 1 || g.z != 1 || (size_t)g.x * b.x < (size_t)p.b_pad) die("loss_cot_kernel: grid %u x %u for b_pad %d", g.x, b.x, p.b_pad);
  if (shm < loss_cot_lds_bytes(p.L) || shm < (size_t)2 * p.L * b.x * 4) die("loss_cot_kernel: %zu bytes of LDS for L %d", shm, p.L);
  need(p.f, ((size_t)(p.L - 1) * p.f_bpad + p.b) * 4, "LossCotParams.f");
  need(p.y, (size_t)p.b * 4, "LossCotParams.y");
  need(p.cot, (size_t)p.L * p.b_pad * 4, "LossCotParams.cot");
}
static void check_optim_step(const OptimStepParams &p, dim3 g, dim3 b) {
  scan(&p, sizeof p, "OptimStepParams");
  if (p.N < 2 || p.D < 2 || p.D > kMaxD || p.L < 1 || p.l_pos < 0 || p.l_pos >= p.N) die("OptimStepParams: N %d D %d L %d l_pos %d", p.N, p.D, p.L, p.l_pos);
  if (g.x != (unsigned)p.N || g.y != 1 || g.z != 1 || b.x != 256) die("optim_step_kernel: grid %u block %u for N %d", g.x, b.x, p.N);
  if (p.kind != TNML_OPT_SGD && p.kind != TNML_OPT_ADAM) die("OptimStepParams: kind %d", p.kind);
  if (p.kind == TNML_OPT_ADAM && (p.clip || !p.s0 || !p.s1)) die("OptimStepParams: Adam with clip %d, m %p, v %p", p.clip, (void *)p.s0, (void *)p.s1);
  if (p.kind == TNML_OPT_ADAM && !(p.corr1 > 0 && p.corr1 <= 1 && p.corr2 > 0 && p.corr2 <= 1)) die("OptimStepParams: bias corrections %g %g", p.corr1, p.corr2);
  if (p.kind == TNML_OPT_SGD && (p.mu > 0) != (p.s0 != nullptr)) die("OptimStepParams: momentum %g with vel %p", p.mu, (void *)p.s0);
  need(p.tab, (size_t)2 * p.N * 4, "OptimStepParams.tab");
  size_t off = 0;
  for (int i = 0; i < p.N; ++i) {
    const int ml = i == 0 ? 1 : p.tab[i - 1], mr = i == p.N - 1 ? 1 : p.tab[i];
    if (ml < 1 || mr < 1) die("OptimStepParams: site %d is %d x %d", i, ml, mr);
    const size_t ne = (size_t)ml * p.D * mr * (i == p.l_pos ? p.L : 1);
    if ((size_t)p.tab[p.N + i] != off) die("OptimStepParams: core %d at offset %d, the flat layout has it at %zu", i, p.tab[p.N + i], off);
    if (i == p.l_pos) need(p.labcore, ne * 4, "OptimStepParams.labcore");
    else {
      if (ne > p.core_stride) die("OptimStepParams: core %d of %zu floats in a slot of %zu", i, ne, p.core_stride);
      need(p.cores + (size_t)i * p.core_stride, ne * 4, "OptimStepParams.cores");
    }
    need(p.G + off, ne * 4, "OptimStepParams.G");
    if (p.s0) need(p.s0 + off, ne * 4, "OptimStepParams.s0");
    if (p.s1) need(p.s1 + off, ne * 4, "OptimStepParams.s1");
    off += ne;
  }
}

static FILE *g_tr = nullptr;
static long g_tr_lines = 0;
static bool tracing() {
  static const bool on = [] { const char *f = getenv("TNML_SAN_TRACE"); return f && *f && (g_tr = fopen(f, "w")); }();
  return on;
}
static void tr(const char *fmt, ...) __attribute__((format(printf, 1, 2)));
static void tr(const char *fmt, ...) {
  if (!tracing()) return;
  va_list ap;
  va_start(ap, fmt);
  vfprintf(g_tr, fmt, ap);
  va_end(ap);
  if (fmt[strlen(fmt) - 1] == '\n') ++g_tr_lines;
}
static std::string dp(const void *p) {
  if (!p) return "0";
  if (!in_arena(p)) return "host";
  char b[24];
  snprintf(b, sizeof b, "@%zx", (size_t)((const char *)p - g_base));
  return b;
}
static void *new_handle(int kind) { static long next[2]; long *h = (long *)malloc(sizeof(long)); *h = next[kind]++; return h; }
static long id(const void *h) { return h ? *(const long *)h : -1; }
#define I(f) tr(" " #f "=%lld", (long long)p.f);
#define R(f) tr(" " #f "=%.17g", (double)p.f);
#define P(f) tr(" " #f "=%s", dp(p.f).c_str());
#define V(f) tr(" " #f "=[%s %d %d %d %d %d]", dp(p.f.base).c_str(), p.f.n_in, p.f.n_out, p.f.s_in, p.f.s_d, p.f.s_out);
static void tr_struct(const NarrowParams &p) {
  I(L) I(D) I(h) I(g) I(s) I(m) I(bsize) I(l2_flag) R(lr) R(wd) R(inv_b_global) P(red) V(lab) V(pl) P(Nh) P(Ng) P(Bnew)
  P(out_behind) I(ob_s_h) I(ob_s_d) I(ob_s_m) P(out_ahead) I(oa_s_m) I(oa_s_d) I(oa_s_g) P(Nh_new) P(metrics) P(dbg) P(stamps)
  P(counters) P(Bdirect) I(stop_after_update) I(fused) I(prep_ready) P(slabs) I(nslabs) I(slab_stride) I(nred) P(red_out) P(prepB)
  P(prepG) P(sync) R(trunc_thr) I(left_dir) P(m_out) R(chol_thr) R(svd_stop2) P(status) I(wait_count) I(pipe) I(z_first) I(z_rows)
  I(zsize) P(zred) V(zcore) P(flag) I(token) I(persist) I(write_ahead) I(persist_off) I(Mcap) P(prepRaw) P(pready) I(pwant) P(Apub)
  P(aflag) P(coreflag) I(coretoken) P(zpoll_flag) I(zpoll_want) P(done_flag) I(done_val) P(abort_flag)
}
static void tr_struct(const WideParams &p) {
  I(b) I(b_pad) I(L) I(h) I(g) I(hp) I(gp) I(do_f) I(do_ext) I(first_ext) I(act_fn) I(loss_fn) R(T) P(x_km1) P(x_k) P(x_kp1) P(Hprev)
  P(Hcur) P(Gprev) P(Gcur) P(Bprev) V(ext_core) P(y) P(f) P(slabs) I(slab_stride) I(bsize) P(stamps)
}
static void tr_struct(const WidePipeParams &p) {
  I(b) I(b_pad) I(L) I(hj) I(gj) I(gn) I(hprev) I(first) I(do_ext) I(first_ext) I(do_f) I(wait_flag) I(do_z) I(act_fn) I(loss_fn) R(T)
  P(x_jm1) P(x_j) P(x_jp1) P(x_jp2) P(Eprev) P(Ecur) V(ext_core) P(Gj) P(Gn) P(Bnew) P(y) P(f) I(zsize) I(slab_stride) P(slabs) P(gslabs)
  P(zred) P(gcnt) P(tcnt) I(nwide) I(gsz) I(ngroups) I(one_level) I(wg0) I(tiles_per_wg) I(ntiles) P(flag) I(token) P(status) I(persist)
  P(coreflag) I(corewant) P(zready) I(zpublish) P(abort_flag) P(stamps)
}
static void tr_struct(const PersistHelperParams &p) {
  I(zr) I(s) I(g) I(L) I(h) I(l2_flag) P(W) V(lab) V(pl) P(Ng) P(T) P(TN) P(Z) P(prepRaw) P(prepB) P(prepG) P(Apub) P(flag) I(want)
  P(aflag) P(nflag) I(awant) P(zready) I(zwant) P(tcnt) P(pcnt) P(abort_flag) P(status) P(stamps)
}
static void tr_struct(const PersistStep &p) { tr(" n:"); tr_struct(p.n); tr(" w:"); tr_struct(p.w); tr(" t:"); tr_struct(p.t); }
static void tr_struct(const PrepParams &p) { V(lab) V(pl) P(Nh) P(Ng) I(h) I(g) I(s) I(L) I(l2_flag) P(prepB) P(prepG) I(nparts) }
static void tr_struct(const MeetParams &p) { P(Lenv) P(Renv) P(x) P(core) P(f) I(b) I(b_pad) I(ml) I(mr) I(D) I(L) I(rows_per_chunk) }
static void tr_struct(const InputGradParams &p) {
  P(bond) P(cores) P(labcore) P(X) P(cot) P(stack) P(g) P(cf) I(core_stride) I(b) I(b_pad) I(x_bpad) I(N) I(D) I(L) I(l_pos) I(cap) I(mb)
}
static void tr_struct(const CoreGradParams &p) {
  P(tab) P(cores) P(labcore) P(X) P(cot) P(stackP) P(stackQ) P(G) P(cf) I(core_stride) I(b) I(b_pad) I(x_bpad) I(N) I(D) I(L) I(l_pos) I(cap)
  I(mb) I(first)
}
static void tr_struct(const InputGradScaledParams &p) { tr_struct(p.base); P(estack) }
static void tr_struct(const CoreGradScaledParams &p) { tr_struct(p.base); P(estack) }
static void tr_struct(const ScaledPredParams &p) { P(bond) P(cores) P(labcore) P(X) P(mant) P(expo) P(f) I(core_stride) I(b) I(b_pad) I(N) I(D) I(L) I(l_pos) I(mb) }
static void tr_struct(const LossCotParams &p) { P(f) P(y) P(cot) I(L) I(b) I(b_pad) I(f_bpad) I(act_fn) I(loss_fn) R(T) }
static void tr_struct(const OptimStepParams &p) {
  P(tab) P(cores) P(labcore) P(G) P(s0) P(s1) I(core_stride) I(N) I(D) I(L) I(l_pos) I(kind) I(clip) R(lr) R(wd) R(mu) R(beta1) R(beta2) R(eps)
  R(corr1) R(corr2)
}
static void tr_struct(const InputGradPixels &p) { P(g) P(data) P(idx) P(out) I(b) I(N) I(D) }
static void tr_struct(const BigExtArgs &p) { P(Eprev) P(x_km1) P(x_k) V(A) I(b_pad) P(Ecur) P(Pk) }
static void tr_struct(const ChainSite &p) { I(core_off) I(is_label) I(n_in) I(n_out) I(s_in) I(s_d) I(s_out) I(x_site) I(env_out_off) }
static void tr_struct(const NormChainSite &p) { I(core_off) I(n_in) I(n_out) I(s_in) I(s_d) I(s_out) I(env_out_off) }
#undef I
#undef R
#undef P
#undef V
template <class S> static void tr_rows(const char *what, const S *rows, int n) {
  for (int i = 0; i < n; ++i) { tr("  %s %d:", what, i); tr_struct(rows[i]); tr("\n"); }
}
static void tr_launch(const std::string &name, dim3 g, dim3 b, size_t shm, hipStream_t st, void **args) {
  const size_t lp = name.find('('), rp = name.rfind(')');
  tr("launch %s grid=%u,%u,%u block=%u,%u,%u lds=%zu stream=s%ld", name.substr(0, lp).c_str(), g.x, g.y, g.z, b.x, b.y, b.z, shm, id(st));
  std::vector<std::string> types;
  for (size_t i = lp + 1, from = i, depth = 0; lp != std::string::npos && i <= rp; ++i) {
    const char ch = name[i];
    depth += (ch == '<') - (ch == '>');
    if ((ch == ',' && !depth) || i == rp) { if (i > from) types.push_back(name.substr(from, i - from)); from = i + 1; }
  }
  for (size_t i = 0; i < types.size(); ++i) {
    const std::string &t = types[i];
    auto is = [&](const char *s) { return t.find(s) != std::string::npos; };
    tr(" |");
    if (is("*")) tr(" %s", dp(*(void **)args[i]).c_str());
    else if (is("NarrowParams")) tr_struct(*(const NarrowParams *)args[i]);
    else if (is("WidePipeParams")) tr_struct(*(const WidePipeParams *)args[i]);
    else if (is("WideParams")) tr_struct(*(const WideParams *)args[i]);
    else if (is("PrepParams")) tr_struct(*(const PrepParams *)args[i]);
    else if (is("MeetParams")) tr_struct(*(const MeetParams *)args[i]);
    else if (is("InputGradScaledParams")) tr_struct(*(const InputGradScaledParams *)args[i]);
    else if (is("CoreGradScaledParams")) tr_struct(*(const CoreGradScaledParams *)args[i]);
    else if (is("ScaledPredParams")) tr_struct(*(const ScaledPredParams *)args[i]);
    else if (is("InputGradParams")) tr_struct(*(const InputGradParams *)args[i]);
    else if (is("CoreGradParams")) tr_struct(*(const CoreGradParams *)args[i]);
    else if (is("InputGradPixels")) tr_struct(*(const InputGradPixels *)args[i]);
    else if (is("LossCotParams")) tr_struct(*(const LossCotParams *)args[i]);
    else if (is("OptimStepParams")) tr_struct(*(const OptimStepParams *)args[i]);
    else if (is("BigExtArgs")) tr_struct(*(const BigExtArgs *)args[i]);
    else if (is("CoreView")) { const CoreView &v = *(const CoreView *)args[i]; tr(" [%s %d %d %d %d %d]", dp(v.base).c_str(), v.n_in, v.n_out, v.s_in, v.s_d, v.s_out); }
    else if (is("BigFrontTiles")) tr(" %d %d", ((int *)args[i])[0], ((int *)args[i])[1]);
    else if (is("float")) tr(" %.9g", *(float *)args[i]);
    else if (is("long")) tr(" %lld", *(long long *)args[i]);
    else if (is("int") || is("bool")) tr(" %d", *(int *)args[i]);
    else tr(" ?");
  }
  tr("\n");
  if (types.size() < 2 || types[0].find('*') == std::string::npos) return;
  const void *tab = *(void **)args[0];
  const int n = *(int *)args[1];
  if (types[0].find("NormChainSite") != std::string::npos) tr_rows("site", (const NormChainSite *)tab, n);
  else if (types[0].find("ChainSite") != std::string::npos) tr_rows("site", (const ChainSite *)tab, n);
  else if (types[0].find("PersistStep") != std::string::npos) tr_rows("step", (const PersistStep *)tab, n + 1);
}
static void tr_copy(const char *what, hipMemcpyKind k, const void *d, const void *s, size_t n, hipStream_t st) {
  const char *kind = k == hipMemcpyHostToDevice ? "H2D" : k == hipMemcpyDeviceToHost ? "D2H" : k == hipMemcpyDeviceToDevice ? "D2D" : k == hipMemcpyHostToHost ? "H2H" : "default";
  tr("%s %s dst=%s src=%s n=%zu stream=s%ld\n", what, kind, dp(d).c_str(), dp(s).c_str(), n, id(st));
}
}
using namespace san;

extern "C" {
void **__hipRegisterFatBinary(const void *) { static void *h; return &h; }
void __hipUnregisterFatBinary(void **) {}
void __hipRegisterFunction(void **, const void *host_fn, char *, const char *dev_name, unsigned, void *, void *, void *, void *, int *) {
  int st = 0;
  char *dm = abi::__cxa_demangle(dev_name, nullptr, nullptr, &st);
  std::string nm = dm ? dm : dev_name;
  free(dm);
  for (size_t at; (at = nm.find("(anonymous namespace)::")) != std::string::npos;) nm.erase(at, 23);
  g_kernels[host_fn] = nm;
}
void __hipRegisterVar(void **, void *, char *, const char *, int, size_t, int, int) {}
static thread_local struct { dim3 g, b; size_t shm; hipStream_t st; } t_cfg;
hipError_t __hipPushCallConfiguration(dim3 g, dim3 b, size_t shm, hipStream_t st) { t_cfg = {g, b, shm, st}; return hipSuccess; }
hipError_t __hipPopCallConfiguration(dim3 *g, dim3 *b, size_t *shm, hipStream_t *st) { *g = t_cfg.g; *b = t_cfg.b; *shm = t_cfg.shm; *st = t_cfg.st; return hipSuccess; }

hipError_t hipLaunchKernel(const void *fn, dim3 g, dim3 b, void **args, size_t shm, hipStream_t st) {
  auto it = g_kernels.find(fn);
  const std::string name = it == g_kernels.end() ? "?" : it->second;
  g_ctx = name.c_str();
  const unsigned long long thr = (unsigned long long)b.x * b.y * b.z;
  if (g.x < 1 || g.y < 1 || g.z < 1 || g.y > 65535 || g.z > 65535 || thr < 1 || thr > 1024 || shm > 160 * 1024)
    die("illegal launch: grid (%u,%u,%u) block (%u,%u,%u) dynamic LDS %zu", g.x, g.y, g.z, b.x, b.y, b.z, shm);
  const std::string key = name.substr(0, name.find('('));
  g_launches[key]++;
  if (tracing()) tr_launch(name, g, b, shm, st, args);
  auto has = [&](const char *s) { return name.find(s) != std::string::npos; };
  if (has("sweep_persist") || has("persist_update_kernel") || has("persist_helper_kernel") || has("persist_batch_kernel")) {
    const PersistStep *st = *(const PersistStep **)args[0];
    const int n = *(int *)args[1];
    need(st, (size_t)(n + 1) * sizeof(PersistStep), "persistent step records");
    for (int k = 0; k < n; ++k) { check_narrow(st[k].n); check_pipe(st[k].w); scan(&st[k].t, sizeof st[k].t, "PersistHelperParams"); }
    check_pipe(st[n].w);
  } else if (has("step_pipe_kernel")) {
    const NarrowParams &n = *(const NarrowParams *)args[0];
    const WidePipeParams &w = *(const WidePipeParams *)args[1];
    if (n.bsize > 0) check_narrow(n);
    check_pipe(w);
    if (g.x > 256) die("step_pipe_kernel: %u workgroups cannot be co-resident on 256 CUs", g.x);
  } else if (has("label_meet_kernel")) {
    check_meet(*(const MeetParams *)args[0], g, b, shm);
  } else if (has("input_grad_scaled_kernel")) {
    check_input_grad_scaled(*(const InputGradScaledParams *)args[0], g, b, shm);
  } else if (has("core_grad_chain_scaled_kernel")) {
    check_core_grad_scaled(*(const CoreGradScaledParams *)args[0], g, b, shm);
  } else if (has("scaled_pred_kernel")) {
    check_scaled_pred(*(const ScaledPredParams *)args[0], g, b, shm);
  } else if (has("input_grad_kernel")) {
    check_input_grad(*(const InputGradParams *)args[0], g, b, shm);
  } else if (has("core_grad_chain_kernel") || has("core_grad_reduce_kernel")) {
    check_core_grad(*(const CoreGradParams *)args[0], g, b, shm, has("core_grad_reduce_kernel"));
  } else if (has("loss_cot_kernel")) {
    check_loss_cot(*(const LossCotParams *)args[0], g, b, shm);
  } else if (has("optim_step_kernel")) {
    check_optim_step(*(const OptimStepParams *)args[0], g, b);
  } else if (has("orth_load_kernel") || has("orth_chain_kernel") || has("orth_store_kernel")) {
    check_orth(*(const OrthParams *)args[0], g, b, shm, has("orth_chain_kernel") ? 1 : has("orth_store_kernel") ? 2 : 0);
  } else if (has("input_grad_onehot_kernel")) {
    const int fbp = *(int *)args[1], L = *(int *)args[2], bb = *(int *)args[3], bp = *(int *)args[5];
    if (bb < 1 || bb > bp || bp > fbp || (size_t)g.x * b.x < (size_t)bp) die("input_grad_onehot_kernel: b %d b_pad %d f_bpad %d grid %u x %u", bb, bp, fbp, g.x, b.x);
    need(*(const float **)args[0], ((size_t)(L - 1) * fbp + bb) * 4, "one-hot: f"); need(*(float **)args[4], (size_t)L * bp * 4, "one-hot: cot");
  } else if (has("input_grad_pixels_kernel")) {
    const InputGradPixels &q = *(const InputGradPixels *)args[0];
    scan(&q, sizeof q, "InputGradPixels");
    if (q.b < 1 || q.N < 1 || q.D < 2 || q.D > kMaxD || (size_t)g.x * b.x < (size_t)q.b * q.N) die("input_grad_pixels_kernel: b %d N %d D %d grid %u x %u", q.b, q.N, q.D, g.x, b.x);
    need(q.g, (size_t)q.b * q.N * q.D * 4, "pixels: g"); need(q.out, (size_t)q.b * q.N * 4, "pixels: out"); need(q.idx, (size_t)q.b * 4, "pixels: index list");
    for (int i = 0; i < q.b; ++i) need(q.data + (size_t)q.idx[i] * q.N, (size_t)q.N * 4, "pixels: dataset row");
  } else if (has("narrow_step_kernel")) {
    check_narrow(*(const NarrowParams *)args[0]);
  } else if (has("wide_step") || has("f_only_kernel")) {
    check_wide(*(const WideParams *)args[0], has("wide_step_mfma_kernel") ? *(int *)args[2] : (int)g.x, has("f_only_kernel"));
  } else if (has("env_chain_roles_kernel")) {
    check_chain(*(const ChainSite **)args[0], *(int *)args[1], *(const float **)args[2], *(const float **)args[3], *(const float **)args[4],
                *(float **)args[5], *(float **)args[6], *(int *)args[7], 1);
    if ((int)g.x * 16 != *(int *)args[7]) die("chain grid %u x 16 samples != b_pad %d", g.x, *(int *)args[7]);
  } else if (has("env_chain_kernel")) {
    check_chain(*(const ChainSite **)args[0], *(int *)args[1], *(const float **)args[2], *(const float **)args[3], *(const float **)args[4],
                has("<true>") ? nullptr : *(float **)args[5], *(float **)args[6], *(int *)args[8], *(int *)args[9]);
  } else if (has("big_merge_wd_kernel") || has("big_merge_wd_mfma_kernel")) {
    const NarrowParams &n = *(const NarrowParams *)args[0];
    check_narrow(n);
    need(*(float **)args[1], (size_t)n.bsize * 4, "large-tensor path: merged tensor");
    if (n.l2_flag) {
      need(*(const double **)args[2], (size_t)n.h * kD * n.s * n.L * 8, "large-tensor path: NL");
      need(*(const double **)args[3], (size_t)n.s * kD * n.g * 8, "large-tensor path: PR");
    }
    if (g.x > (unsigned)kBigParts) die("big_merge_wd_kernel: %u blocks leave partials, room for %d", g.x, kBigParts);
    need(*(double **)args[5], (size_t)g.x * 3 * 8, "large-tensor path: block partials");
  } else if (has("big_wd_kernel")) {
    const NarrowParams &n = *(const NarrowParams *)args[0];
    check_narrow(n);
    need(*(const float **)args[1], (size_t)n.bsize * 4, "large-tensor path: merged tensor");
    if (n.l2_flag) need(*(const double **)args[2], (size_t)n.bsize * 8, "large-tensor path: Nh^T.B");
    if (g.x > (unsigned)kBigParts) die("big_wd_kernel: %u blocks leave partials, room for %d", g.x, kBigParts);
    need(*(double **)args[4], (size_t)g.x * 3 * 8, "large-tensor path: block partials");
  } else if (has("big_nlpr_kernel")) {
    const NarrowParams &n = *(const NarrowParams *)args[0];
    check_narrow(n);
    need(*(double **)args[1], (size_t)n.h * kD * n.s * n.L * 8, "big_nlpr: NL");
    need(*(double **)args[2], (size_t)n.s * kD * n.g * 8, "big_nlpr: PR");
    if (*(double **)args[2] < *(double **)args[1] + (size_t)n.h * kD * n.s * n.L) die("big_nlpr: PR overlaps NL");
  } else if (has("big_gram_kernel")) {
    const int n = *(int *)args[1], len = *(int *)args[2];
    need(*(const float **)args[0], (size_t)n * len * 4, "large-tensor path: B_new");
    need(*(double **)args[5], (size_t)8 * kBigMaxN * kBigMaxN * 8, "large-tensor path: partial Gram matrices");
    if (n > kBigMaxN || (n & 1)) die("big_gram_kernel: short side %d", n);
    if ((int)g.x * 16 < n || (int)g.y * 16 < n) die("big_gram_kernel: grid (%u, %u) of 16 x 16 tiles for n = %d", g.x, g.y, n);
    if (*(unsigned **)args[6]) need(*(unsigned **)args[6], 4, "big_gram: flag word of the side stream");
  } else if (has("big_ext_kernel")) {
    check_big_ext(*(const BigExtArgs *)args[0], shm);
    const BigExtArgs &a = *(const BigExtArgs *)args[0];
    if ((int)g.x * 64 != a.b_pad) die("big_ext_kernel: grid %u x 64 samples != b_pad %d", g.x, a.b_pad);
    if ((int)g.y * 16 < a.A.n_out) die("big_ext_kernel: %u workgroup rows of 16 for %d bond indices", g.y, a.A.n_out);
  } else if (has("big_contract_kernel")) {
    const CoreView &A = *(const CoreView *)args[1];
    const size_t nc = *(int *)args[2];
// ... 72 lines not shown
  const bool sd = k == hipMemcpyDeviceToHost || k == hipMemcpyDeviceToDevice || (k == hipMemcpyDefault && in_arena(s));
  if (dd) need(d, n, "copy destination"); else if (in_arena(d)) die("host destination %p is device memory", d);
  if (sd) need(s, n, "copy source"); else if (in_arena(s)) die("host source %p is device memory", s);
  memmove(d, s, n);
  g_ctx = "";
}
hipError_t hipMemcpy(void *d, const void *s, size_t n, hipMemcpyKind k) { tr_copy("memcpy", k, d, s, n, nullptr); copy_checked(d, s, n, k, "hipMemcpy"); return hipSuccess; }
hipError_t hipMemcpyAsync(void *d, const void *s, size_t n, hipMemcpyKind k, hipStream_t st) { tr_copy("memcpy_async", k, d, s, n, st); copy_checked(d, s, n, k, "hipMemcpyAsync"); return hipSuccess; }
hipError_t hipMemcpy2DAsync(void *d, size_t dpitch, const void *s, size_t spitch, size_t w, size_t h, hipMemcpyKind k, hipStream_t st) {
  tr("memcpy2d_async rows=%zu dst_pitch=%zu src_pitch=%zu of ", h, dpitch, spitch);
  tr_copy("row", k, d, s, w, st);
  if (w > dpitch || w > spitch) die("hipMemcpy2DAsync: width %zu exceeds a pitch (%zu, %zu)", w, dpitch, spitch);
  for (size_t r = 0; r < h; ++r) copy_checked((char *)d + r * dpitch, (const char *)s + r * spitch, w, k, "hipMemcpy2DAsync");
  return hipSuccess;
}
hipError_t hipMemsetAsync(void *d, int v, size_t n, hipStream_t st) {
  tr("memset dst=%s v=%d n=%zu stream=s%ld\n", dp(d).c_str(), v, n, id(st));
  g_ctx = "hipMemset";
  if (n) { need(d, n, "memset"); memset(d, v, n); }
  g_ctx = "";
  return hipSuccess;
}
hipError_t hipMemset(void *d, int v, size_t n) { return hipMemsetAsync(d, v, n, nullptr); }

hipError_t hipGetDeviceCount(int *n) { *n = 1; return hipSuccess; }
hipError_t hipSetDevice(int d) { return d == 0 ? hipSuccess : hipErrorInvalidDevice; }
hipError_t hipGetDevicePropertiesR0600(hipDeviceProp_tR0600 *p, int) {
  memset(p, 0, sizeof *p);
  strcpy(p->gcnArchName, "gfx950:sramecc+:xnack-");
  strcpy(p->name, "sanitizer stand-in for MI355X");
  p->multiProcessorCount = 256;
  p->sharedMemPerBlock = 160 * 1024;
  p->maxSharedMemoryPerMultiProcessor = 160 * 1024;
  p->totalGlobalMem = (size_t)288 << 30;
  p->warpSize = 64;
  p->maxThreadsPerBlock = 1024;
  return hipSuccess;
}
const char *hipGetErrorString(hipError_t e) { return e == hipSuccess ? "no error" : "error (stub)"; }
hipError_t hipGetLastError() { return hipSuccess; }
hipError_t hipStreamCreateWithFlags(hipStream_t *s, unsigned) { *s = (hipStream_t)new_handle(0); return hipSuccess; }
hipError_t hipStreamDestroy(hipStream_t s) { free(s); return hipSuccess; }
hipError_t hipStreamSynchronize(hipStream_t s) { tr("stream_sync s%ld\n", id(s)); return hipSuccess; }
hipError_t hipStreamWaitEvent(hipStream_t s, hipEvent_t e, unsigned) { tr("stream_wait s%ld e%ld\n", id(s), id(e)); return hipSuccess; }
hipError_t hipEventCreate(hipEvent_t *e) { *e = (hipEvent_t)new_handle(1); return hipSuccess; }
hipError_t hipEventCreateWithFlags(hipEvent_t *e, unsigned) { return hipEventCreate(e); }
hipError_t hipEventDestroy(hipEvent_t e) { free(e); return hipSuccess; }
hipError_t hipEventRecord(hipEvent_t e, hipStream_t s) { tr("event_record e%ld s%ld\n", id(e), id(s)); return hipSuccess; }
hipError_t hipEventSynchronize(hipEvent_t e) { tr("event_sync e%ld\n", id(e)); return hipSuccess; }
hipError_t hipEventElapsedTime(float *ms, hipEvent_t, hipEvent_t) { *ms = 0.01f; return hipSuccess; }

ncclResult_t ncclGetUniqueId(ncclUniqueId *id) { memset(id, 7, sizeof *id); return ncclSuccess; }
ncclResult_t ncclCommInitRank(ncclComm_t *c, int n, ncclUniqueId, int r) { if (n != 1 || r != 0) return ncclInvalidArgument; *c = (ncclComm_t)malloc(8); return ncclSuccess; }
ncclResult_t ncclCommDestroy(ncclComm_t c) { free(c); return ncclSuccess; }
const char *ncclGetErrorString(ncclResult_t) { return "rccl (stub)"; }
ncclResult_t ncclAllReduce(const void *s, void *d, size_t count, ncclDataType_t t, ncclRedOp_t, ncclComm_t, hipStream_t st) {
  tr("allreduce send=%s recv=%s count=%zu stream=s%ld\n", dp(s).c_str(), dp(d).c_str(), count, id(st));
  g_ctx = "ncclAllReduce";
  ++g_allreduces;
  const size_t el = t == ncclFloat ? 4 : (t == ncclDouble ? 8 : 4);
  need(s, count * el, "send buffer"); need(d, count * el, "receive buffer");
  if (s != d) memmove(d, s, count * el);
  g_ctx = "";
  return ncclSuccess;
}

void san_stub_report(void) {
  long total = 0;
  for (auto &kv : g_launches) total += kv.second;
  printf("san-stub: %ld launches checked (%zu kernels), %ld pointer extents checked, %zu live allocations\n", total, g_launches.size(), g_checked_ptrs, g_alloc.size());
  for (auto &kv : g_launches) printf("    %-60s %ld\n", kv.first.c_str(), kv.second);
  if (tracing()) { fflush(g_tr); printf("san-stub: call trace of %ld lines written\n", g_tr_lines); }
}
long san_stub_allreduces(void) { return g_allreduces; }
long san_stub_launches(const char *substr) {
  long n = 0;
  for (auto &kv : g_launches) if (kv.first.find(substr) != std::string::npos) n += kv.second;
  return n;
}
long san_stub_alloc_calls(void) { return g_alloc_calls; }
void san_stub_fail_alloc(long nth) { g_fail_call = nth > 0 ? g_alloc_calls + nth : 0; }
int san_stub_fail_pending(void) { return g_fail_call != 0; }
void san_stub_poke_int(void *dev, int v) { need(dev, 4, "poke"); memcpy(dev, &v, 4); }
}
```

tensornetworkforml_amd/csrc/tnml_api.hip:

```cpp
#include <rccl/rccl.h>

#include <algorithm>
#include <climits>
#include <cmath>
#include <cstdarg>
#include <cstdio>
#include <cstring>
#include <cstdlib>
#include <initializer_list>
#include <memory>
#include <utility>

#include "tnml_internal.h"
#include "small_gemm_device.h"
#include "wide_pipe_device.h"
#include "grad_chain_device.h"

using namespace tnml;

static thread_local std::string g_err;

static int fail(int code, const char *fmt, ...) {
  char buf[1024];
  va_list ap;
// ... 110 lines not shown
  int persist_mode = 1;
  hipEvent_t ev_main = nullptr, ev_prep = nullptr;
  struct {
    hipEvent_t ev_upd[2] = {nullptr, nullptr}, ev_bat[2] = {nullptr, nullptr};
    int upd = 0, bat = 0;
    bool pending = false;
    bool enabled = true;
    unsigned *flags = nullptr;
    unsigned zseq = 0, dseq = 0;
    bool flags_enabled = true, done_valid = false, zsig_valid = false;
  } split;
  struct {
    bool enabled = true;
    ZTicket Z;
    float *Pk = nullptr;
    hipEvent_t ev_upd = nullptr, ev_z = nullptr;
    bool pending = false;
    unsigned *flags = nullptr;
    unsigned zsig_seq = 0, bsig_seq = 0;
    bool flags_enabled = true;
    bool ext_on_side = false;
  } bigpipe;
  hipEvent_t ev0 = nullptr, ev1 = nullptr, pev0 = nullptr, pev1 = nullptr;
  std::vector<int> bond;
  int l_pos = 0;
  bool cores_set = false;
  bool have_input = false, have_labels = false;
  bool envs_valid_L = false, envs_valid_R = false;
  bool Ln_valid = false, Rn_valid = false;
  bool f_current = false;
  bool Bnew_valid = false;
  int prev_h = 0, prev_g = 0;
  int prev_left_dir = 0;
  int last_bsize = 0, last_n = 0, last_h = 0, last_g = 0, last_left_dir = 0;
  bool debug = false, profile = false, stamps = false;
  bool check_launches = false;
  int sync_interval = 256;
  double svd_stop2 = kSvdStop2Default;
  double chol_thr = kCholThrDefault;
  double trunc_thr = 0.999;
  double prof_ms[4] = {0, 0, 0, 0};
  long long prof_n[4] = {0, 0, 0, 0};
  bool sweep_timing = false;
  std::vector<hipEvent_t> sweep_ev;
  size_t sweep_ev_used = 0;
  double sweep_ms = 0;
  long long sweep_launches = 0, step_launches = 0;
  double cnt_steps = 0, cnt_bytes = 0, cnt_flops = 0, cnt_fwd_bytes = 0, cnt_fwd = 0;
  static constexpr int kStageSlots = 8;
  float *stageX[kStageSlots] = {nullptr};
  int *stageY[kStageSlots] = {nullptr};
  int stageB[kStageSlots] = {0};
  size_t core_stride = 0, lab_elems = 0, bmax = 0;
  float *X = nullptr, *Xstage = nullptr;
  int *y = nullptr;
  float *f = nullptr, *ftmp = nullptr, *ftmp2 = nullptr;
  float *Lenv = nullptr, *Renv = nullptr;
  float *cores = nullptr, *lab[2] = {nullptr, nullptr};
  int lab_cur = 0;
  double *Ln = nullptr, *Rn = nullptr;
  float *Bnew = nullptr, *slabs = nullptr, *red = nullptr, *metrics = nullptr, *scal = nullptr;
  float *Bscr = nullptr, *Bscr2 = nullptr;
  BigScratch big{};
  bool big_ready = false;
  bool force_big = false;
  bool chain_plain = false;
  bool any_pos = false;
  bool seg_starting = false;
  float *predEnv = nullptr;
  float *prepB = nullptr;
  double *prepG = nullptr;
  unsigned *sync = nullptr;
  float *zslabs = nullptr, *gslabs = nullptr, *zred = nullptr;
  int zstride = 0;
  struct {
    bool enabled = true;
    int tiles = 2;
    unsigned *cnt = nullptr;
    int nwide = 0, tpw = 1, ngroups = 0;
    ZTicket Z;
    unsigned token = 0;
  } pipe;
  bool persist_enabled = true;
  PersistStep *pst_dev = nullptr, *pst_host[2] = {nullptr, nullptr};
  hipEvent_t pst_ev[2] = {nullptr, nullptr};
  int pst_cur = 0;
  float *zred2 = nullptr, *prepRaw = nullptr;
  double *Tbuf[2] = {nullptr, nullptr}, *TNbuf[2] = {nullptr, nullptr}, *Apub = nullptr;
  unsigned *pst_cnt = nullptr, *pst_flags = nullptr;
  long long persist_sweeps = 0;
  int num_cus = 256;
  float *Xpred_stage = nullptr, *Xpred = nullptr, *fpred = nullptr;
  int pred_cap = 0;
  bool scaled = false;
  float *pred_mant = nullptr;
  int *pred_expo = nullptr, *pred_bond = nullptr, *ig_estack = nullptr, *cg_estack = nullptr;
  int slab_stride = 0, nblk_cap = 0, metrics_cap = 0;
  double *dbg = nullptr;
  size_t dbg_elems = 0;
  int *status = nullptr;
  unsigned long long *counters = nullptr;
  char *tables = nullptr;
  size_t tables_bytes = 0;
  double *anyd_W = nullptr, *anyd_T2 = nullptr;
  float *ds_data = nullptr;
  int *ds_labels = nullptr;
  int ds_n = 0, ds_form = 0;
  double ds_coef[kMaxD] = {0};
  int *ds_idx = nullptr, *ds_idx_host[2] = {nullptr, nullptr};
  hipEvent_t ds_idx_ev[2] = {nullptr, nullptr};
  bool ds_idx_busy[2] = {false, false};
  int ds_idx_cap = 0, ds_idx_cur = 0;
  int *ds_ypred = nullptr;
  double *ds_part = nullptr, *ds_acc = nullptr;
  int ds_part_cap = 0;
  float *ig_stack = nullptr, *ig_cot = nullptr, *ig_g = nullptr, *ig_gpix = nullptr, *ig_cf = nullptr;
  int *ig_bond = nullptr;
  int ig_cap = 0, ig_chunk = 0;
  float *cg_stackP = nullptr, *cg_stackQ = nullptr, *cg_cot = nullptr, *cg_cf = nullptr, *cg_G = nullptr;
  int *cg_tab = nullptr;
  int cg_cap = 0, cg_chunk = 0;
  struct {
    int kind = TNML_OPT_SGD, clip = 1;
    double momentum = 0.0, beta1 = 0.9, beta2 = 0.999, eps = 1e-8;
    long long t = 0;
    std::vector<int> bond;
    int l_pos = -1;
  } opt;
  float *opt_s0 = nullptr, *opt_s1 = nullptr;
  double *opt_met = nullptr;
  int opt_met_cap = 0;
  std::vector<int> opt_tab;
  struct {
    double *W = nullptr, *Mbuf = nullptr, *aux = nullptr, *sigma = nullptr, *disc = nullptr, *result = nullptr;
    float *out_cores = nullptr, *out_lab = nullptr;
    OrthOp *ops = nullptr;
    int *bond = nullptr, *rank = nullptr, *status = nullptr;
    bool ready = false;
  } orth;
  ncclComm_t comm = nullptr;
  int rank = 0, nranks = 1;

  int ml(int i) const { return i == 0 ? 1 : bond[i - 1]; }
  int mr(int i) const { return i == N - 1 ? 1 : bond[i]; }
  float *env_slot(float *base, int site) const { return base + (size_t)site * Mmax * b_pad; }
  long long env_off(int site) const { return (long long)site * Mmax * b_pad; }
  float *core_slot(int site) const { return cores + (size_t)site * core_stride; }
  double *norm_slot(double *base, int site) const { return base + (size_t)site * Mmax * Mmax; }
};

static void drop_pregradients(tnml_ctx *c) { c->pipe.Z.valid = false; c->bigpipe.Z.valid = false; }

extern "C" const char *tnml_last_error(void) { return g_err.c_str(); }
extern "C" const char *tnml_version(void) { return "tnml-hip 0.1 (gfx950)"; }

extern "C" int tnml_device_count(void) {
  int n = 0;
  if (hipGetDeviceCount(&n) != hipSuccess) return 0;
  return n;
}

#include "host_plan.inc"

static int make_group(tnml_ctx *c, const char *what, std::initializer_list<Owner::Member> group) {
  const hipError_t e = c->own.make(group);
  return e == hipSuccess ? TNML_OK : fail(TNML_ERR_HIP, "allocating %s failed: %s", what, hipGetErrorString(e));
// ... 1803 lines not shown
  PersistStep *st = c->pst_host[buf];
  st[n_steps] = PersistStep{};
  WidePipeParams &pro = st[n_steps].w;
  const int ntiles = c->b_pad / kTS;
  int tpw = c->pipe.tpw;
  while ((ntiles + tpw - 1) / tpw + 1 + kPersistHelpers > c->num_cus) ++tpw;
  const int nwide = (ntiles + tpw - 1) / tpw;
  const int nH = kPersistHelpers;
  if (1 + nH + nwide > c->num_cus) return 0;
  const int Mcap = c->Mmax;
  const size_t pbytes = persist_lds_bytes(Mcap);
  unsigned *fl = c->pst_flags;
  float *zr2[2] = {c->zred, c->zred2};
  size_t lds_narrow = 0, lds_wide = 0, lds_help = 0;
  fill_wide_pipe(c, pro, sc, -1);
  pro.do_ext = 0; pro.wait_flag = 0; pro.do_z = 1; pro.do_f = 0;
  set_pipe_tiles(pro, tpw);
  pro.wg0 = 1 + nH; pro.persist = 1; pro.zred = zr2[0]; pro.zready = fl + 2; pro.zpublish = 1; pro.abort_flag = fl + 4;
  pro.gcnt = c->pst_cnt + (size_t)n_steps * 32; pro.tcnt = pro.gcnt + 16;
  if (!wide_pipe_fits(c, pro)) return give_up();
  pipe_try_one_level(pro);
  lds_wide = wide_pipe_lds_bytes(pro);
  double bytes = 0, flops = 0;
  for (int k = 0; k < n_steps; ++k) {
    const StepGeom q = step_geom(c, left_dir, trunc_policy);
    if (q.fail) return give_up();
    const int h = q.h, g = q.g, s = q.s, m = q.m;
    const size_t nlds = narrow_lds_bytes(h, g, s, L, m);
    if (q.nn > 64 || (q.nn & 1) || nlds + pbytes > kLdsMax || h > Mcap || m > Mcap || q.bsize > 8192) return give_up();
    PersistStep &ps = st[k];
    ps = PersistStep{};
    NarrowParams &n = ps.n;
    fill_update(c, n, q, sc.l2_flag, sc.lr, sc.weight_dec);
    n.out_ahead = c->lab[(c->lab_cur + (n_steps - k)) & 1];
    n.write_ahead = (k == n_steps - 1);
    n.metrics = c->metrics + 2 * (size_t)k;
    n.chol_thr = c->chol_thr;
    n.stamps = (c->stamps && k == n_steps / 2) ? c->dbg + 4 * c->bmax + kDbgSigma + 5 : nullptr;
    n.pipe = 1; n.persist = 1; n.z_first = (k == 0);
    fill_wide_pipe(c, ps.w, sc, k);
    WidePipeParams &wp = ps.w;
    const int zr = k == 0 ? 1 : wp.hprev * D;
    if (zr > 64) return give_up();
    n.z_rows = zr; n.zsize = zr * D * D * g * L;
    n.zred = zr2[k & 1]; n.red = n.zred;
    n.prepB = c->prepB; n.prepG = c->prepG; n.prepRaw = c->prepRaw;
    n.pready = c->pst_cnt + (size_t)k * 32 + 21; n.pwant = (unsigned)nH;
    n.flag = fl + 0; n.token = (unsigned)k + 1;
    n.Apub = c->Apub;
    n.aflag = fl + 5; n.coreflag = fl + 3; n.coretoken = (unsigned)k + 1; n.abort_flag = fl + 4;
    n.Mcap = Mcap;
    if (!persist_record_ok(n)) return give_up();
    lds_narrow = std::max(lds_narrow, nlds);
    wp.do_ext = k >= 1; wp.do_f = 1; wp.wait_flag = 1;
    wp.do_z = (k + 1 <= N - 2);
    set_pipe_tiles(wp, tpw);
    wp.wg0 = 1 + nH; wp.persist = 1; wp.flag = fl + 0; wp.token = (unsigned)k + 1;
    wp.coreflag = fl + 3; wp.corewant = (unsigned)k; wp.zready = fl + 2; wp.zpublish = (unsigned)k + 2; wp.abort_flag = fl + 4;
    wp.zred = zr2[(k + 1) & 1];
    wp.gcnt = c->pst_cnt + (size_t)k * 32; wp.tcnt = wp.gcnt + 16;
    wp.stamps = n.stamps;
    if (!wide_pipe_fits(c, wp)) return give_up();
    pipe_try_one_level(wp);
    lds_wide = std::max(lds_wide, wide_pipe_lds_bytes(wp));
    PersistHelperParams &t = ps.t;
    t.zr = zr; t.s = s; t.g = g; t.L = L; t.h = h; t.l2_flag = n.l2_flag;
    t.W = k == 0 ? nullptr : c->Bnew;
    t.lab = n.lab; t.pl = n.pl; t.Ng = n.Ng;
    t.T = c->Tbuf[k & 1]; t.TN = c->TNbuf[k & 1]; t.Z = zr2[k & 1];
    t.prepRaw = c->prepRaw; t.prepB = c->prepB; t.prepG = c->prepG; t.Apub = c->Apub;
    t.flag = fl + 0; t.want = (unsigned)k; t.aflag = fl + 5; t.nflag = fl + 3; t.awant = (unsigned)k; t.zready = fl + 2; t.zwant = (unsigned)k + 1;
    t.tcnt = c->pst_cnt + (size_t)k * 32 + 20; t.pcnt = c->pst_cnt + (size_t)k * 32 + 21;
    t.abort_flag = fl + 4; t.status = c->status; t.stamps = n.stamps;
    lds_help = std::max(lds_help, persist_helper_lds_bytes(zr, s, g, L, h, nH));
    if ((size_t)zr * D * D * g * L + kMetricSlots > (size_t)c->zstride) return give_up();
    advance_frame(c, q, m);
    if (!c->stamps || k <= n_steps / 2) note_last_step(c, q);
    add_step_work(c, q, bytes, flops);
  }
  const size_t lds = c->persist_mode >= 2 ? lds_narrow + pbytes : std::max(std::max(lds_narrow + pbytes, lds_wide), lds_help);
  if (lds > kLdsMax || lds_wide > kLdsMax || lds_help > kLdsMax) return give_up();
  const int persist_off = (int)((lds - pbytes) & ~(size_t)15);
  for (int k = 0; k < n_steps; ++k) st[k].n.persist_off = persist_off;
  HIP_TRY(hipMemcpyAsync(c->pst_dev, st, (size_t)(n_steps + 1) * sizeof(PersistStep), hipMemcpyHostToDevice, c->stream));
  HIP_TRY(hipEventRecord(c->pst_ev[buf], c->stream));
  c->pst_cur ^= 1;
  HIP_TRY(hipMemsetAsync(c->pst_flags, 0, 8 * sizeof(unsigned), c->stream));
  HIP_TRY(hipMemsetAsync(c->pst_cnt, 0, (size_t)(n_steps + 1) * 32 * sizeof(unsigned), c->stream));
  if (c->persist_mode >= 2) {
    HIP_TRY(hipEventRecord(c->ev_p0, c->stream));
    HIP_TRY(hipStreamWaitEvent(c->stream2, c->ev_p0, 0));
    HIP_TRY(hipStreamWaitEvent(c->stream3, c->ev_p0, 0));
    launch_sweep_persist_split(c->pst_dev, n_steps, nH, nwide, lds, lds_help, lds_wide, c->stream, c->stream2, c->stream3);
    HIP_TRY(hipGetLastError());
    HIP_TRY(hipEventRecord(c->ev_p2, c->stream2));
    HIP_TRY(hipEventRecord(c->ev_p3, c->stream3));
    HIP_TRY(hipStreamWaitEvent(c->stream, c->ev_p2, 0));
    HIP_TRY(hipStreamWaitEvent(c->stream, c->ev_p3, 0));
  } else {
    launch_sweep_persist(c->pst_dev, n_steps, nH, 1 + nH + nwide, lds, c->stream);
    HIP_TRY(hipGetLastError());
  }
  c->cnt_steps += n_steps; c->cnt_bytes += bytes; c->cnt_flops += flops;
  c->sweep_launches += 1; c->step_launches += n_steps; c->persist_sweeps += 1;
  c->Bnew_valid = true; c->f_current = true; drop_pregradients(c);
  return 1;
}

static int sweep_anyd(tnml_ctx *c, const SweepCall &sc);
static int standalone_anyd(tnml_ctx *c, NarrowParams &n);

static int norm_envs_for_label_site(tnml_ctx *c);

static bool slices_ride(const SweepCall &sc, int npath) { return npath == 0 && sc.mode == 0 && !sc.Bdirect_dev; }

struct PipePlan {
  WidePipeParams wp, wpro;
  bool need_prologue;
};

static int plan_pipe_step(const tnml_ctx *c, const SweepCall &sc, const StepGeom &q, int step, int npath, PipePlan &pp) {
  const int N = c->N, L = c->L, k = q.k;
  if (!c->pipe.enabled || !slices_ride(sc, npath) || (sc.seg_start && step == 0)) return 0;
  if (prep_slice_lds_bytes(q.h, q.g, q.s, L) > kLdsMax) return 0;
  WidePipeParams &wp = pp.wp, &wpro = pp.wpro;
  fill_wide_pipe(c, wp, sc, k);
  wp.do_ext = k >= 1; wp.do_f = 1; wp.wait_flag = 1;
  wp.do_z = (k + 1 <= N - 2);
  if (wp.do_z && !wide_pipe_fits(c, wp)) wp.do_z = 0;
  pipe_try_one_level(wp);
  if (wp.do_z && c->pipe.tiles > wp.tiles_per_wg && q.nn >= 32) {
    wp.tiles_per_wg = c->pipe.tiles;
    wp.nwide = (wp.ntiles + wp.tiles_per_wg - 1) / wp.tiles_per_wg;
    wp.ngroups = (wp.nwide + kPipeGroupMax - 1) / kPipeGroupMax;
  }
  if (!wide_pipe_fits(c, wp)) return 0;
  pp.need_prologue = !c->pipe.Z.matches(sc, k);
  if (pp.need_prologue) {
    fill_wide_pipe(c, wpro, sc, k - 1);
    wpro.do_ext = 0; wpro.wait_flag = 0; wpro.do_z = 1;
    wpro.do_f = (k >= 1 && c->Bnew_valid && !c->f_current) ? 1 : 0;
    if (wpro.do_f && (c->prev_h != wpro.hj || c->prev_g != wpro.gj))
      return fail(TNML_ERR_STATE, "internal: previous-step dims (%d,%d) do not match (%d,%d)", c->prev_h, c->prev_g, wpro.hj, wpro.gj);
    if (!wide_pipe_fits(c, wpro)) return 0;
  }
  return 1;
}

static int launch_pipe_prologue(tnml_ctx *c, WidePipeParams &wpro, bool split) {
  NarrowParams none{};
  wpro.wg0 = 0;
  if (split) { int rc = split_wait_update(c); if (rc) return rc; }
  prof_begin(c);
  launch_step_pipe(none, wpro, wide_pipe_lds_bytes(wpro), split ? c->stream2 : c->stream);
  prof_end(c, 1);
  c->sweep_launches++; c->step_launches++;
  if (split) { int rc = split_exchange(c, wpro.zsize); if (rc) return rc; }
  else if (c->comm) NCCL_TRY(ncclAllReduce(c->zred, c->zred, wpro.zsize + kMetricSlots, ncclFloat, ncclSum, c->comm, c->stream));
  if (wpro.do_f) c->f_current = true;
  return TNML_OK;
}

static void fill_pipe_update(tnml_ctx *c, NarrowParams &n, WidePipeParams &wp, const StepGeom &q) {
  const int D = c->D, L = c->L;
  n.fused = 1; n.nred = 0; n.sync = c->sync; n.red_out = nullptr;
  n.prep_ready = 0;
  n.wait_count = kD * kD * (q.h > 8 ? 2 : 1);
  n.pipe = 1; n.z_first = (q.k == 0); n.z_rows = wp.hprev * D;
  n.zsize = (q.k == 0 ? 1 : n.z_rows) * D * D * q.g * L;
  n.zred = c->zred; n.red = c->zred; n.zcore = wp.ext_core;
  n.flag = c->pipe.cnt + 17; n.token = ++c->pipe.token;
  wp.token = n.token;
  wp.wg0 = 1 + n.wait_count;
}
static size_t pipe_update_lds(const tnml_ctx *c, const StepGeom &q) {
  return std::max(narrow_lds_bytes(q.h, q.g, q.s, c->L, q.m), prep_slice_lds_bytes(q.h, q.g, q.s, c->L));
}

static int launch_pipe_step_fused(tnml_ctx *c, const SweepCall &sc, const StepGeom &q, NarrowParams &n, PipePlan &pp) {
  WidePipeParams &wp = pp.wp;
  { int rc = split_join(c); if (rc) return rc; }
  if (pp.need_prologue) { int rc = launch_pipe_prologue(c, pp.wpro, false); if (rc) return rc; }
  fill_pipe_update(c, n, wp, q);
  const size_t lds = std::max(pipe_update_lds(c, q), wide_pipe_lds_bytes(wp));
  if (lds > kLdsMax) return fail(TNML_ERR_ARG, "internal: pipelined step needs %zu bytes of LDS", lds);
// ... 478 lines not shown
  if (capacity < (size_t)m * c->b) return fail(TNML_ERR_ARG, "capacity too small");
  std::vector<float> tmp((size_t)m * c->b_pad);
  const float *src = c->env_slot(side == TNML_SIDE_LEFT ? c->Lenv : c->Renv, site);
  HIP_TRY(hipMemcpyAsync(tmp.data(), src, tmp.size() * sizeof(float), hipMemcpyDeviceToHost, c->stream));
  HIP_TRY(hipStreamSynchronize(c->stream));
  for (int s = 0; s < c->b; ++s)
    for (int a = 0; a < m; ++a) out[(size_t)s * m + a] = tmp[(size_t)a * c->b_pad + s];
  if (m_out) *m_out = m;
  return TNML_OK;
}

extern "C" int tnml_set_trunc_threshold(tnml_ctx *c, double threshold) {
  if (!c) return fail(TNML_ERR_ARG, "ctx is NULL");
  if (!(threshold > 0.0 && threshold < 1.0)) return fail(TNML_ERR_ARG, "threshold %g outside (0, 1)", threshold);
  c->trunc_thr = threshold;
  return TNML_OK;
}

extern "C" int tnml_set_narrow_path(tnml_ctx *c, int force_large) {
  if (!c) return fail(TNML_ERR_ARG, "ctx is NULL");
  c->force_big = force_large != 0;
  return TNML_OK;
}

extern "C" int tnml_comm_probe(tnml_ctx *c, int n_floats, int reps, double *us_per_allreduce) {
  if (!c || !us_per_allreduce || n_floats < 1 || reps < 1) return fail(TNML_ERR_ARG, "bad argument");
  *us_per_allreduce = 0.0;
  if (!c->comm) return TNML_OK;
  if ((size_t)n_floats > (size_t)c->zstride) return fail(TNML_ERR_ARG, "probe message of %d floats exceeds the pre-gradient buffer (%d)", n_floats, c->zstride);
  HIP_TRY(hipSetDevice(c->device));
  HIP_TRY(hipStreamSynchronize(c->stream));
  HIP_TRY(hipStreamSynchronize(c->stream2));
  float *buf = c->gslabs ? c->gslabs : c->zslabs;
  if (!buf) return fail(TNML_ERR_STATE, "no pipelined-step buffers yet: run a sweep first");
  for (int w = 0; w < 3; ++w) NCCL_TRY(ncclAllReduce(buf, buf, n_floats, ncclFloat, ncclSum, c->comm, c->stream2));
  HIP_TRY(hipEventRecord(c->ev0, c->stream2));
  for (int r = 0; r < reps; ++r) NCCL_TRY(ncclAllReduce(buf, buf, n_floats, ncclFloat, ncclSum, c->comm, c->stream2));
  HIP_TRY(hipEventRecord(c->ev1, c->stream2));
  HIP_TRY(hipEventSynchronize(c->ev1));
  float ms = 0;
  HIP_TRY(hipEventElapsedTime(&ms, c->ev0, c->ev1));
  *us_per_allreduce = 1e3 * ms / reps;
  return TNML_OK;
}

extern "C" int tnml_set_comm_overlap(tnml_ctx *c, int on) {
  if (!c) return fail(TNML_ERR_ARG, "ctx is NULL");
  c->split.enabled = on != 0;
  return TNML_OK;
}

extern "C" int tnml_set_flag_handoffs(tnml_ctx *c, int on) {
  if (!c) return fail(TNML_ERR_ARG, "ctx is NULL");
  HIP_TRY(hipSetDevice(c->device));
  HIP_TRY(hipStreamSynchronize(c->stream));
  if (c->stream2) HIP_TRY(hipStreamSynchronize(c->stream2));
  c->bigpipe.flags_enabled = on != 0; c->split.flags_enabled = on != 0;
  c->split.done_valid = false; c->split.zsig_valid = false;
  return TNML_OK;
}

extern "C" int tnml_set_any_position(tnml_ctx *c, int on) {
  if (!c) return fail(TNML_ERR_ARG, "ctx is NULL");
  if (c->comm) return fail(TNML_ERR_STATE, "sharded batches with the label at an intermediate site are not supported");
  c->any_pos = on != 0;
  return TNML_OK;
}

extern "C" int tnml_set_chain_path(tnml_ctx *c, int force_plain) {
  if (!c) return fail(TNML_ERR_ARG, "ctx is NULL");
  c->chain_plain = force_plain != 0;
  return TNML_OK;
}

extern "C" int tnml_set_step_pipeline(tnml_ctx *c, int on) {
  if (!c) return fail(TNML_ERR_ARG, "ctx is NULL");
  c->pipe.enabled = on != 0;
  c->bigpipe.enabled = on != 0;
  c->pipe.tiles = on >= 2 ? on : (on == 1 ? 2 : 1);
  drop_pregradients(c);
  return TNML_OK;
}

extern "C" int tnml_set_persistent(tnml_ctx *c, int on) {
  if (!c) return fail(TNML_ERR_ARG, "ctx is NULL");
  if (on < 0 || on > 2) return fail(TNML_ERR_ARG, "mode %d outside [0, 2]", on);
  c->persist_enabled = on != 0;
  if (on) c->persist_mode = on;
  return TNML_OK;
}

extern "C" int tnml_set_sync_interval(tnml_ctx *c, int n_steps) {
  if (!c) return fail(TNML_ERR_ARG, "ctx is NULL");
  if (n_steps < 0) return fail(TNML_ERR_ARG, "negative interval");
  c->sync_interval = n_steps;
  return TNML_OK;
}

extern "C" int tnml_set_svd_stop(tnml_ctx *c, double stop2) {
  if (!c) return fail(TNML_ERR_ARG, "ctx is NULL");
  if (!(stop2 >= 1e-12 && stop2 <= 1e-2)) return fail(TNML_ERR_ARG, "svd stop threshold %g outside [1e-12, 1e-2]", stop2);
  c->svd_stop2 = stop2;
  return TNML_OK;
}

extern "C" int tnml_debug_enable(tnml_ctx *c, int on) {
  if (!c) return fail(TNML_ERR_ARG, "ctx is NULL");
  c->debug = (on & 1) != 0;
  c->stamps = (on & 2) != 0;
  c->check_launches = (on & 4) != 0;
  return TNML_OK;
}

extern "C" int tnml_get_step_debug(tnml_ctx *c, int what, double *out, size_t capacity, size_t *n_out) {
  if (!c || !out) return fail(TNML_ERR_ARG, "NULL argument");
  if (!c->debug && !(c->stamps && what == TNML_DBG_L2)) return fail(TNML_ERR_STATE, "debug capture is off (tnml_debug_enable)");
  if (c->last_bsize <= 0) return fail(TNML_ERR_STATE, "no step has run yet");
  HIP_TRY(hipSetDevice(c->device));
  const size_t Bs = c->last_bsize;
  std::vector<double> hbuf(4 * Bs + kDbgSigma + kDbgScalars + 8);
  HIP_TRY(hipMemcpyAsync(hbuf.data(), c->dbg, (4 * Bs + kDbgSigma + 5) * sizeof(double), hipMemcpyDeviceToHost, c->stream));
  HIP_TRY(hipMemcpyAsync(hbuf.data() + 4 * Bs + kDbgSigma + 5, c->dbg + 4 * c->bmax + kDbgSigma + 5, (kDbgScalars - 5) * sizeof(double), hipMemcpyDeviceToHost, c->stream));
  HIP_TRY(hipStreamSynchronize(c->stream));
  auto tensor_out = [&](size_t block) -> int {
    if (capacity < Bs) return fail(TNML_ERR_ARG, "capacity too small");
    const int D = c->D, L = c->L, h = c->last_h, g = c->last_g;
    const double *src = hbuf.data() + block * Bs;
    if (!c->last_left_dir) {
      memcpy(out, src, Bs * sizeof(double));
    } else {
      for (int h_ = 0; h_ < h; ++h_) for (int dk = 0; dk < D; ++dk) for (int dk1 = 0; dk1 < D; ++dk1)
        for (int g_ = 0; g_ < g; ++g_) for (int l = 0; l < L; ++l)
          out[((((size_t)g_ * D + dk1) * D + dk) * h + h_) * L + l] = src[((((size_t)h_ * D + dk) * D + dk1) * g + g_) * L + l];
    }
    if (n_out) *n_out = Bs;
    return TNML_OK;
  };
  switch (what) {
    case TNML_DBG_B: return tensor_out(0);
    case TNML_DBG_DB_RAW: return tensor_out(1);
    case TNML_DBG_B_NEW: return tensor_out(2);
    case TNML_DBG_L2_GRAD: return tensor_out(3);
    case TNML_DBG_SIGMA:
      if (capacity < (size_t)c->last_n) return fail(TNML_ERR_ARG, "capacity too small");
      memcpy(out, hbuf.data() + 4 * Bs, c->last_n * sizeof(double));
      if (n_out) *n_out = c->last_n;
      return TNML_OK;
    case TNML_DBG_L2:
      if (capacity < (size_t)kDbgScalars) return fail(TNML_ERR_ARG, "capacity too small");
      memcpy(out, hbuf.data() + 4 * Bs + kDbgSigma, kDbgScalars * sizeof(double));
      if (n_out) *n_out = kDbgScalars;
      return TNML_OK;
  }
  return fail(TNML_ERR_ARG, "unknown debug selector %d", what);
}

__global__ void tnml_phase_marker_kernel() {}
extern "C" int tnml_marker(tnml_ctx *c, int id) {
  if (!c || id < 1 || id > 1024) return fail(TNML_ERR_ARG, "marker id outside [1, 1024]");
  HIP_TRY(hipSetDevice(c->device));
  hipLaunchKernelGGL(tnml_phase_marker_kernel, dim3(id), dim3(64), 0, c->stream);
  HIP_TRY(hipGetLastError());
  return TNML_OK;
}
extern "C" int tnml_timer_start(tnml_ctx *c) {
  if (!c) return fail(TNML_ERR_ARG, "ctx is NULL");
// ... 84 lines not shown
```

tensornetworkforml_amd/csrc/wide_pipe_device.h:

```cpp
#pragma once
#include "tnml_internal.h"
#include "act_device.h"
#include "jacobi_device.h"

namespace tnml {

typedef float fvec4 __attribute__((ext_vector_type(4)));
constexpr int kPipeThreads = 1024;
constexpr int kPTSP = kTS + 1;
constexpr int kPipeGroupMax = 16;

__host__ __device__ inline int upm(int x, int m) { return (x + m - 1) / m * m; }

__device__ inline void st_sc1(float *p, float v) { __hip_atomic_store(p, v, __ATOMIC_RELAXED, __HIP_MEMORY_SCOPE_AGENT); }
__device__ inline float ld_sc1(const float *p) { return __hip_atomic_load(p, __ATOMIC_RELAXED, __HIP_MEMORY_SCOPE_AGENT); }

struct WidePipeParams {
  int b, b_pad, L;
  int hj, gj;
  int gn;
  int hprev;
  int first;
  int do_ext;
  int first_ext;
// ... 48 lines not shown
__device__ inline int spin_wait_ge2(const unsigned *f1, unsigned w1, const unsigned *f2, unsigned w2, const unsigned *abort_flag) {
  for (int spins = 0; spins < (1 << 19); ++spins) {
    const unsigned a = __hip_atomic_load(f1, __ATOMIC_RELAXED, __HIP_MEMORY_SCOPE_AGENT), b = __hip_atomic_load(f2, __ATOMIC_RELAXED, __HIP_MEMORY_SCOPE_AGENT);
    if (a >= w1 && b >= w2) return 0;
    if ((spins & 63) == 63 && abort_flag && __hip_atomic_load(abort_flag, __ATOMIC_RELAXED, __HIP_MEMORY_SCOPE_AGENT)) return 2;
    __builtin_amdgcn_s_sleep(24);
  }
  return 1;
}

struct WidePipeDims { int nI, IP, JP, RS, KA, HS, I3, J3, EH; };
template <class WP>
__host__ __device__ inline WidePipeDims wide_pipe_dims(const WP &p) {
  WidePipeDims d;
  d.nI = p.first ? 1 : p.hj * kD;
  d.IP = upm(d.nI, 16);
  d.JP = upm(kD * p.gj, 4);
  d.RS = (d.JP * p.L) | 1;
  d.KA = upm(p.hprev * kD, 4);
  d.EH = upm(p.hj, 16);
  d.HS = d.EH + 1;
  d.I3 = upm(d.nI * kD, 16);
  d.J3 = upm(kD * p.gn, 16);
  return d;
}

struct WidePipeSmem { float *sX, *sF, *sGl, *sPpp, *sA, *sE, *sPp, *sQp, *sBp, *sPg, *sQn, *sFp, *sMet; size_t floats; };
template <class WP>
__host__ __device__ inline WidePipeSmem wide_pipe_carve(float *base, const WP &p, const WidePipeDims &d) {
  WidePipeSmem w;
  float *q = base;
  w.sX = q; q += 4 * kTS * kD;
  w.sF = q; q += p.L * kTS;
  w.sGl = q; q += p.L * kTS;
  w.sPpp = q; q += (p.do_ext ? d.KA : 0) * kPTSP;
  w.sA = q; q += (p.do_ext ? d.KA * d.HS : 0);
  w.sE = q; q += d.EH * kPTSP;
  w.sPp = q; q += d.IP * kPTSP;
  w.sQp = q; q += (p.do_f ? d.JP : 0) * kPTSP;
  w.sBp = q; q += (p.do_f ? (size_t)d.IP * d.RS : 0);
  w.sPg = q; q += (p.do_z ? (size_t)p.L * d.I3 * kPTSP : 0);
  w.sQn = q; q += (p.do_z ? d.J3 * kPTSP : 0);
  w.sFp = q; q += (p.do_f ? (size_t)(d.IP / 16) * p.L * kTS : 0);
  w.sMet = q; q += 4 * kTS;
  w.floats = (size_t)(q - base);
  return w;
}
inline size_t wide_pipe_lds_bytes(const WidePipeParams &p) {
  const WidePipeDims d = wide_pipe_dims(p);
  alignas(16) static float origin[4];
  return wide_pipe_carve(origin, p, d).floats * sizeof(float) + 16;
}
constexpr int kPipeMaxZT = 4;
inline int wide_pipe_ztiles(const WidePipeParams &p) {
  const WidePipeDims d = wide_pipe_dims(p);
  return p.L * (d.I3 / 16) * (d.J3 / 16);
}
void launch_step_pipe(const NarrowParams &p, const WidePipeParams &w, size_t lds_bytes, hipStream_t st);
void launch_step_pipe_update(const NarrowParams &p, const WidePipeParams &w, size_t lds_bytes, hipStream_t st);

struct PersistHelperParams {
  int zr, s, g, L, h;
  int l2_flag;
  const float *W;
  CoreView lab, pl;
  const double *Ng;
  double *T, *TN;
  const float *Z;
  float *prepRaw, *prepB;
  double *prepG;
  const double *Apub;
  const unsigned *flag;
  unsigned want;
  const unsigned *aflag;
  const unsigned *nflag;
  unsigned awant;
  const unsigned *zready;
  unsigned zwant;
  unsigned *tcnt, *pcnt;
  unsigned *abort_flag;
  int *status;
  double *stamps;
};
struct PersistStep { NarrowParams n; WidePipeParams w; PersistHelperParams t; };
constexpr int kPersistHelpers = 8;
__host__ __device__ inline int persist_pub_off(int na, int h) { return ((na + 1) & ~1) + ((h + 1) & ~1); }
__host__ __device__ inline size_t persist_pub_doubles(int na, int h) { return (size_t)persist_pub_off(na, h) + (((size_t)h * h + 1) & ~(size_t)1); }
__host__ __device__ inline size_t persist_helper_ss_doubles(int zr, int h, int cw) {
  const size_t a = 2 * (size_t)zr * cw, b = (size_t)h * cw;
  return ((a > b ? a : b) + 1) & ~(size_t)1;
}
inline size_t persist_helper_lds_bytes(int zr, int s, int g, int L, int h, int nH) {
  const size_t DG = (size_t)kD * g, RW = kD * DG * L;
  const size_t per = ((size_t)zr * kD + nH - 1) / nH, cw = (RW + nH - 1) / nH;
  const size_t p1 = (((per * s * L + 3) & ~(size_t)3) + (((size_t)s * DG + 3) & ~(size_t)3)) * sizeof(float) +
                    ((((size_t)g * g + 1) & ~(size_t)1) + 2 * per * DG * L) * sizeof(double);
  const size_t p2 = (persist_pub_doubles(zr * h, h) + persist_helper_ss_doubles(zr, h, (int)cw) + 2 * (size_t)h * cw) * sizeof(double) +
                    ((size_t)zr * cw + (size_t)zr * h) * sizeof(float);
  return (p1 > p2 ? p1 : p2) + 64;
}
void launch_sweep_persist(const PersistStep *steps_dev, int n_steps, int n_helpers, int grid, size_t lds_bytes, hipStream_t st);
void launch_sweep_persist_split(const PersistStep *steps_dev, int n_steps, int n_helpers, int n_wide, size_t lds_update, size_t lds_helper,
                                size_t lds_wide, hipStream_t st_update, hipStream_t st_helper, hipStream_t st_wide);


template <int PERSIST>
struct WidePipeArgs : WidePipeParams {
  __device__ __forceinline__ WidePipeArgs(const WidePipeParams &q) : WidePipeParams(q) {}
  static constexpr int persist = PERSIST;
};
template <class WP>
__device__ __forceinline__ bool wide_pipe_block(const WP &p, float *smem) {
  const WidePipeDims dm = wide_pipe_dims(p);
  const WidePipeSmem w = wide_pipe_carve(smem, p, dm);
  int tid_step = threadIdx.x;
  if (p.persist) {
    asm volatile("" : "+v"(tid_step));
    __builtin_assume(tid_step >= 0 && tid_step < kPipeThreads);
  }
  const int tid = tid_step, NT = kPipeThreads;
  const int lane = tid & 63, NWV = NT / 64;
  const int wave = __builtin_amdgcn_readfirstlane(tid >> 6);
  const int r = lane & 15, q = lane >> 4;
  const int L = p.L, hj = p.hj, gj = p.gj, gn = p.gn, hprev = p.hprev;
  const int nI = dm.nI, nJ = kD * gj;
  constexpr int ST = kTS / 16;
  const int wg = (int)blockIdx.x - p.wg0;
  const int IT3 = dm.I3 / 16, JT3 = dm.J3 / 16, QW = kD * gn;
  constexpr int kMaxZT = kPipeMaxZT;
  fvec4 zacc[kMaxZT];
#pragma unroll
  for (int u = 0; u < kMaxZT; ++u) zacc[u] = fvec4{0.f, 0.f, 0.f, 0.f};
  float met[4] = {0.f, 0.f, 0.f, 0.f};

  bool flag_seen = !p.wait_flag;
  __shared__ int sGiveUp;
  double *bst = (p.persist && p.stamps && blockIdx.x == (unsigned)p.wg0 && tid == 0) ? p.stamps : nullptr;
  auto rt = []() { return (double)(__builtin_amdgcn_s_memrealtime() & ((1ull << 40) - 1)); };
  if (bst) bst[32] = rt();
  if (p.persist) {
    if (tid == 0) {
      const int bad = p.do_ext ? spin_wait_ge(p.coreflag, p.corewant, p.abort_flag) : 0;
      if (bad == 1) { atomicOr(p.status, 8); __hip_atomic_store(p.abort_flag, 1u, __ATOMIC_RELAXED, __HIP_MEMORY_SCOPE_AGENT); }
      sGiveUp = bad;
    }
    lds_barrier();
    if (sGiveUp) return true;
    if (bst) bst[33] = rt();
  }
  for (int tt = 0; tt < p.tiles_per_wg; ++tt) {
    const int tile = wg + tt * p.nwide;
    if (tile >= p.ntiles) break;
    const int s0 = tile * kTS;
    if (tt > 0) lds_barrier();
    for (int e = tid; e < 4 * kTS * kD; e += NT) {
      const int which = e / (kTS * kD), rr = e % (kTS * kD);
      const float *src = which == 0 ? p.x_jm1 : (which == 1 ? p.x_j : (which == 2 ? p.x_jp1 : p.x_jp2));
      w.sX[e] = src ? src[(size_t)s0 * kD + rr] : 0.f;
    }
    if (!p.do_f)
      for (int e = tid; e < L * kTS; e += NT) w.sF[e] = p.f[(size_t)(e / kTS) * p.b_pad + s0 + (e % kTS)];
    if (p.do_ext) {
      for (int e = tid; e < dm.KA * dm.HS; e += NT) {
        const int o = e % dm.HS, i = e / dm.HS;
        float v = 0.f;
        if (i < hprev * kD && o < hj) {
          const float *src = p.ext_core.base + ((i >> 1) * p.ext_core.s_in + (i & 1) * p.ext_core.s_d + o * p.ext_core.s_out);
          v = p.persist ? ld_sc1(src) : *src;
        }
        w.sA[e] = v;
      }
    } else {
      for (int e = tid; e < dm.EH * kTS; e += NT) {
        const int sl = e % kTS, hn = e / kTS;
        w.sE[hn * kPTSP + sl] = hn < hj ? ((p.Ecur && !p.first) ? p.Ecur[(size_t)hn * p.b_pad + s0 + sl] : 1.0f) : 0.f;
      }
    }
    lds_barrier();
    const float *sXm = w.sX, *sXj = w.sX + kTS * kD, *sXp = w.sX + 2 * kTS * kD, *sXq = w.sX + 3 * kTS * kD;
    if (p.do_ext) {
      for (int e = tid; e < dm.KA * kTS; e += NT) {
        const int sl = e % kTS, i = e / kTS;
        float v = 0.f;
        if (i < hprev * kD) v = (p.first_ext ? 1.0f : p.Eprev[(size_t)(i >> 1) * p.b_pad + s0 + sl]) * sXm[sl * kD + (i & 1)];
// ... 290 lines not shown
```

Baseline: 21130 sweep-steps/s.

## Specialise persistent sweep kernel on compile-time step shapes for bond 10/20

Adds template-specialised persistent sweep kernels in which the narrow update and helper blocks see bond, label count, z_rows and helper count as compile-time constants when a step matches a table entry (H=10 or 20, L=2). The host marks matching steps and picks the specialised kernel; the remaining steps fall back to the dynamic-shape path. It also simplifies index arithmetic with __mul24, removes bounds checks for even k-splits in the Gram MFMA loop and for even helper column splits, and moves the Jacobi convergence test into the round. The aim is to cut integer address and bounds overhead and let the compiler unroll on the hot per-step path. In exchange the code grows, there are more kernel instantiations, and compile time and register use may rise.

```diff
diff --git a/include/tnml.h b/include/tnml.h
--- a/include/tnml.h
+++ b/include/tnml.h
@@ -116,6 +116,8 @@
 int tnml_set_step_pipeline(tnml_ctx *ctx, int on);
 
 int tnml_set_persistent(tnml_ctx *ctx, int on);
+int tnml_set_shape_kernels(tnml_ctx *ctx, int on);
+int tnml_fixed_shape_steps(tnml_ctx *ctx, int *n_steps);
 
 int tnml_set_sync_interval(tnml_ctx *ctx, int n_steps);
 
diff --git a/tensornetworkforml_amd/_hip.py b/tensornetworkforml_amd/_hip.py
--- a/tensornetworkforml_amd/_hip.py
+++ b/tensornetworkforml_amd/_hip.py
@@ -32,6 +32,7 @@
     'tnml_optim_config', 'tnml_optim_reset', 'tnml_gd_train_indices', 'tnml_gd_step', 'tnml_get_core_slots',
     'tnml_orthogonalize', 'tnml_compress', 'tnml_bond_spectra',
     'tnml_set_chain_scaling', 'tnml_predict_scaled',
+    'tnml_set_shape_kernels', 'tnml_fixed_shape_steps',
 ]
 
 
@@ -88,6 +89,8 @@
         L.tnml_svd_stats.argtypes = [vp, C.c_int, f64p]
         L.tnml_svd_stats_ex.argtypes = [vp, C.c_int, f64p, C.c_int]
         L.tnml_set_persistent.argtypes = [vp, C.c_int]
+        L.tnml_set_shape_kernels.argtypes = [vp, C.c_int]
+        L.tnml_fixed_shape_steps.argtypes = [vp, C.POINTER(C.c_int)]
         L.tnml_trunc_rank.argtypes = [C.c_int] * 9
         L.tnml_update_B.argtypes = [vp, f32p, C.c_int, C.c_float, C.c_float, C.c_int, C.c_int, C.c_int, C.c_float,
                                     f64p, C.c_size_t, f32p]
@@ -536,6 +539,14 @@
     def set_persistent(self, on=True):
         _chk(lib().tnml_set_persistent(self._h, int(on)))
 
+    def set_shape_kernels(self, on=True):
+        _chk(lib().tnml_set_shape_kernels(self._h, int(bool(on))))
+
+    def fixed_shape_steps(self):
+        v = C.c_int()
+        _chk(lib().tnml_fixed_shape_steps(self._h, C.byref(v)))
+        return v.value
+
     def set_sync_interval(self, n_steps):
         _chk(lib().tnml_set_sync_interval(self._h, int(n_steps)))
 
diff --git a/tensornetworkforml_amd/csrc/kernels_narrow.hip b/tensornetworkforml_amd/csrc/kernels_narrow.hip
--- a/tensornetworkforml_amd/csrc/kernels_narrow.hip
+++ b/tensornetworkforml_amd/csrc/kernels_narrow.hip
@@ -138,8 +138,16 @@
 template <class T>
 __device__ __forceinline__ RecField<T> rec_field(const T *field) { return RecField<T>{(const __attribute__((address_space(4))) T *)field}; }
 
-struct PersistArgs {
-  int L, h, g, s, m, bsize, l2_flag;
+struct DynShape {
+  static constexpr int id = 0;
+  int L, h, g, s, m, bsize;
+  __device__ __forceinline__ void load_shape(const __attribute__((address_space(4))) NarrowParams *r) {
+    L = r->L; h = r->h; g = r->g; s = r->s; m = r->m; bsize = r->bsize;
+  }
+};
+template <class Shape>
+struct PersistArgs : Shape {
+  int l2_flag;
   float lr, wd;
   const double *Nh;
   int persist_off, Mcap;
@@ -179,7 +187,7 @@
         metrics(rec_field(&rec->metrics)), counters(rec_field(&rec->counters)), status(rec_field(&rec->status)),
         aflag(rec_field(&rec->aflag)), coreflag(rec_field(&rec->coreflag)), coretoken(rec_field(&rec->coretoken)) {
     const auto *r = (const __attribute__((address_space(4))) NarrowParams *)rec;
-    L = r->L; h = r->h; g = r->g; s = r->s; m = r->m; bsize = r->bsize; l2_flag = r->l2_flag;
+    this->load_shape(r); l2_flag = r->l2_flag;
     lr = r->lr; wd = r->wd; Nh = r->Nh; persist_off = r->persist_off; Mcap = r->Mcap;
     pready = r->pready; pwant = r->pwant; abort_flag = r->abort_flag; zred = r->zred; zsize = r->zsize;
     prepRaw = r->prepRaw; prepB = r->prepB; prepG = r->prepG; Bnew = r->Bnew; flag = r->flag; token = r->token;
@@ -518,23 +526,24 @@
       while (t >= rowlen) { t -= rowlen; ++ti; --rowlen; }
       const int tj = ti + t;
       const int i0 = ti << 4, j0 = tj << 4;
-      const bool va = i0 + rr < n, vb = j0 + rr < n;
-      const float *pa = Wb + min(i0 + rr, n - 1) * rs, *pb = Wb + min(j0 + rr, n - 1) * rs;
-      const int k_lo = ks * kchunk, k_hi = min(len, k_lo + kchunk);
+      const float *pa = Wb + __mul24(min(i0 + rr, n - 1), rs), *pb = Wb + __mul24(min(j0 + rr, n - 1), rs);
+      const bool even_k = gsplit * kchunk == len;
+      const int k_lo = ks * kchunk, klen = even_k ? kchunk : min(len - k_lo, kchunk);
+      const float *pak = pa + __mul24(k_lo, cs), *pbk = pb + __mul24(k_lo, cs);
       dvec4 acc0 = {0.0, 0.0, 0.0, 0.0}, acc1 = {0.0, 0.0, 0.0, 0.0};
-      for (int k0 = k_lo; k0 < k_hi; k0 += 16) {
+      for (int k0 = 0; k0 < klen; k0 += 16) {
         float fa[4], fb[4];
 #pragma unroll
         for (int u = 0; u < 4; ++u) {
-          const int kc = min(k0 + 4 * u + qq, k_hi - 1) * cs;
-          fa[u] = pa[kc];
-          fb[u] = pb[kc];
+          const int kc = __mul24(min(k0 + 4 * u + qq, klen - 1), cs);
+          fa[u] = pak[kc];
+          fb[u] = pbk[kc];
         }
 #pragma unroll
         for (int u = 0; u < 4; ++u) {
-          const bool vk = k0 + 4 * u + qq < k_hi;
-          const double av = (va && vk) ? (double)fa[u] : 0.0, bv = (vb && vk) ? (double)fb[u] : 0.0;
-          if (k0 + 4 * u < k_hi) {
+          const bool vk = k0 + 4 * u + qq < klen;
+          const double av = vk ? (double)fa[u] : 0.0, bv = vk ? (double)fb[u] : 0.0;
+          if (k0 + 4 * u < klen) {
             if (u & 1) acc1 = __builtin_amdgcn_mfma_f64_16x16x4f64(av, bv, acc1, 0, 0, 0);
             else acc0 = __builtin_amdgcn_mfma_f64_16x16x4f64(av, bv, acc0, 0, 0, 0);
           }
@@ -542,11 +551,11 @@
       }
       const dvec4 acc = acc0 + acc1;
       const int j = j0 + rr;
-      double *Pk = P0 + (size_t)ks * ne * ne;
+      double *Pk = P0 + (size_t)ks * ne * ne + (__mul24(i0 + qq, ne) + j);
 #pragma unroll
       for (int reg = 0; reg < 4; ++reg) {
         const int i = i0 + qq + 4 * reg;
-        if (i < ne && j < ne) Pk[i * ne + j] = (i < n && j < n) ? acc[reg] : 0.0;
+        if (i < ne && j < ne) Pk[4 * reg * ne] = (i < n && j < n) ? acc[reg] : 0.0;
       }
     }
     lds_barrier();
@@ -606,7 +615,7 @@
 #pragma unroll
   for (int u = 0; u < MAXI; ++u) {
     const int it = gtid + u * NW;
-    itValid[u] = wrank >= NVW && gtid < NW && it < nG;
+    itValid[u] = u * NW < nG && wrank >= NVW && gtid < NW && it < nG;
     int P = 0, Q = 0;
     if (itValid[u]) {
       int rem = it;
@@ -721,7 +730,7 @@
     if (r.level >= 2) k.sFlag[6 + (applied & 1)] = applied + 1;
   };
   int round_idx = 0, last_big1 = 0;
-  auto jacobi_round = [&]() {
+  auto jacobi_round = [&]() -> bool {
         const double *csc = k.dCS + cur * np * 4;
         const int big_slot = k.sFlag[6 + (round_idx & 1)];
         if (isParam) {
@@ -753,7 +762,7 @@
           const float h1 = ra ? fmaf(sA, q0y, cA * q1y) : fmaf(cA, q0y, -sA * q1y);
           const float ng = rb ? fmaf(sB, h0, cB * h1) : fmaf(cB, h0, -sB * h1);
           const RotT r = jacobi_rot_f32(na, nb, ng, fmaxf((float)kept2, kept_lo), (float)abs2, (float)p.svd_stop2);
-          publish(k.dCS + ((cur ^ 1) * np + tid) * 4, r, round_idx + 1);
+          publish(k.dCS + ((cur ? 0 : 4 * np) + 4 * tid), r, round_idx + 1);
         }
         if (isVwave) {
           const double2 tc = *reinterpret_cast<const double2 *>(csc + 4 * (vLaneOk ? vQ : 0));
@@ -796,11 +805,14 @@
           if (!itDiag[u]) Gn[itD21[u]] = n21;
           Gn[itD22[u]] = n22;
         }
+        last_big1 = max(last_big1, big_slot);
+        const int last_big_s = __builtin_amdgcn_readfirstlane(last_big1);
+        const bool done = round_idx + 1 - last_big_s >= ne - 1;
         lds_barrier();
         double *tsw = Gc; Gc = Gn; Gn = tsw;
         cur ^= 1;
-        last_big1 = max(last_big1, big_slot);
         ++round_idx;
+        return done;
   };
   if (n > 1) {
     kept2 = kept_scale(Gc);
@@ -814,8 +826,7 @@
     lds_barrier();
     for (; sweeps < kJacobiMaxSweeps && !converged; ++sweeps) {
       for (int rnd = 0; rnd < ne - 1; ++rnd) {
-        jacobi_round();
-        if (round_idx - __builtin_amdgcn_readfirstlane(last_big1) >= ne - 1) { converged = 1; break; }
+        if (jacobi_round()) { converged = 1; break; }
       }
       if (!converged) kept2 = kept_scale(Gc);
     }
@@ -924,7 +935,7 @@
    }
   lds_barrier();
   const int DM = D * mk;
-  auto store_T2 = [&](int, int i, int j, double v) { k.dT2[i * DM + j] = v; };
+  auto store_T2 = [&](int, int i, int j, double v) { k.dT2[__mul24(i, DM) + j] = v; };
   if (short_rows) {
     int slot = 0;
     if (!p.persist || p.write_ahead)
@@ -966,8 +977,8 @@
     }
     mm_lds(1, mk, mk, h * D, k.sCb, 0, 1, mk, k.dT2, 0, mk, 1,
            [&](int, int i, int j, double v) {
-             Nh_new[i * mk + j] = v;
-             if (p.persist) PL.Nh[i * mk + j] = v;
+             Nh_new[__mul24(i, mk) + j] = v;
+             if (p.persist) PL.Nh[__mul24(i, mk) + j] = v;
            });
     if (p.persist) {
       lds_barrier();
@@ -1121,7 +1132,8 @@
     if (tid == 0) __hip_atomic_fetch_add(t.tcnt, 1u, __ATOMIC_RELAXED, __HIP_MEMORY_SCOPE_AGENT);
     return false;
   }
-  const int cw = (RW + nH - 1) / nH, c0 = min(RW, hid * cw), nc = min(RW, c0 + cw) - c0;
+  const bool even_split = RW % nH == 0;
+  const int cw = (RW + nH - 1) / nH, c0 = even_split ? hid * cw : min(RW, hid * cw), nc = even_split ? cw : min(RW, c0 + cw) - c0;
   const int cw2 = 2 * cw;
   double *sA = (double *)smem_raw;
   double *sIv = sA + (((size_t)zr * h + 1) & ~(size_t)1);
@@ -1169,12 +1181,12 @@
   lds_barrier();
   if (hst) hst[25] = rt();
   if (nc > 0) {
-    mm_lds_f32(h, nc, zr, sAff, 1, h, sZf, cw, 1, [&](int i, int j, float v) { sOut[i * cw + j] = v; });
+    mm_lds_f32(h, nc, zr, sAff, 1, h, sZf, cw, 1, [&](int i, int j, float v) { sOut[__mul24(i, cw) + j] = v; });
     const int slot = (((h + 15) >> 4) * ((nc + 15) >> 4)) & ((NT >> 6) - 1);
     mm_lds(1, h, t.l2_flag ? 2 * cw : cw, zr, sA, 0, 1, h, sS, 0, cw2, 1,
            [&](int, int i, int j, double v) {
-             if (j < cw) { if (j < nc) sOut[(h + i) * cw + j] = (float)(v * sIv[i]); }
-             else sP2[i * cw + (j - cw)] = v * sIv[i];
+             if (j < cw) { if (j < nc) sOut[__mul24(h + i, cw) + j] = (float)(v * sIv[i]); }
+             else sP2[__mul24(i, cw) + (j - cw)] = v * sIv[i];
            }, false, slot);
   }
   if (t.l2_flag) {
@@ -1201,7 +1213,7 @@
   st_sc1_rows(t.prepB, sOut + (size_t)h * cw, h, cw, RW, c0, nc);
   if (t.l2_flag) {
     if (nc > 0) {
-      mm_lds(1, h, nc, h, sNh, 0, 1, h, sP2, 0, cw, 1, [&](int, int i, int j, double v) { sS[i * cw + j] = v; });
+      mm_lds(1, h, nc, h, sNh, 0, 1, h, sP2, 0, cw, 1, [&](int, int i, int j, double v) { sS[__mul24(i, cw) + j] = v; });
     }
     lds_barrier();
     st_sc1_rows(t.prepG, sS, h, cw, RW, c0, nc);
@@ -1214,19 +1226,40 @@
   return false;
 }
 
+template <class Shape>
+struct HelperArgs : PersistHelperParams {
+  static constexpr int zr = Shape::zr, s = Shape::s, g = Shape::g, L = Shape::L, h = Shape::h;
+  __device__ __forceinline__ explicit HelperArgs(const PersistHelperParams &q) : PersistHelperParams(q) {}
+};
+__device__ __forceinline__ int rec_shape(const PersistStep *rec) { return *(const __attribute__((address_space(4))) int *)&rec->shape; }
+
+template <class Shape>
 __global__ __launch_bounds__(kNarrowThreads) void sweep_persist_kernel(const PersistStep *__restrict__ steps_g, int n_steps, int nH) {
   extern __shared__ __attribute__((aligned(16))) unsigned char smem_raw[];
   const int blk = blockIdx.x;
   if (blk == 0) {
 #pragma nounroll
-    for (int k = 0; k < n_steps; ++k)
-      if (narrow_body(PersistArgs(&steps_g[k].n), smem_raw)) break;
+    for (int k = 0; k < n_steps; ++k) {
+      if constexpr (Shape::id != 0) {
+        if (rec_shape(&steps_g[k]) == Shape::id) {
+          if (narrow_body(PersistArgs<Shape>(&steps_g[k].n), smem_raw)) break;
+          continue;
+        }
+      }
+      if (narrow_body(PersistArgs<DynShape>(&steps_g[k].n), smem_raw)) break;
+    }
   } else if (blk <= nH) {
 #pragma nounroll
     for (int ph = 0; ph < 2 * n_steps; ++ph) {
       PersistHelperParams t;
       __builtin_memcpy(&t, &steps_g[ph >> 1].t, sizeof t);
       lds_barrier();
+      if constexpr (Shape::id != 0) {
+        if ((ph & 1) && rec_shape(&steps_g[ph >> 1]) == Shape::id) {
+          if (persist_helper_block(HelperArgs<Shape>(t), blk - 1, kPersistHelpers, smem_raw, true)) break;
+          continue;
+        }
+      }
       if (persist_helper_block(t, blk - 1, nH, smem_raw, (ph & 1) != 0)) break;
     }
   } else {
@@ -1240,15 +1273,24 @@
   }
 }
 
-void launch_sweep_persist(const PersistStep *steps_dev, int n_steps, int n_helpers, int grid, size_t lds_bytes, hipStream_t st) {
-  hipLaunchKernelGGL(sweep_persist_kernel, dim3(grid), dim3(kNarrowThreads), lds_bytes, st, steps_dev, n_steps, n_helpers);
+template <int I>
+using TableShape = FixedShape<kPersistShapes[I].H, kPersistShapes[I].L, I + 1>;
+static_assert(kNumPersistShapes == 2, "one case below per entry of kPersistShapes");
+bool launch_sweep_persist(const PersistStep *steps_dev, int n_steps, int n_helpers, int grid, size_t lds_bytes, hipStream_t st, int shape) {
+  const dim3 gr(grid), bl(kNarrowThreads);
+  switch (shape) {
+    case 0: hipLaunchKernelGGL(sweep_persist_kernel<DynShape>, gr, bl, lds_bytes, st, steps_dev, n_steps, n_helpers); return true;
+    case 1: hipLaunchKernelGGL(sweep_persist_kernel<TableShape<0>>, gr, bl, lds_bytes, st, steps_dev, n_steps, n_helpers); return true;
+    case 2: hipLaunchKernelGGL(sweep_persist_kernel<TableShape<1>>, gr, bl, lds_bytes, st, steps_dev, n_steps, n_helpers); return true;
+  }
+  return false;
 }
 
 __global__ __launch_bounds__(kNarrowThreads) void persist_update_kernel(const PersistStep *__restrict__ steps_g, int n_steps) {
   extern __shared__ __attribute__((aligned(16))) unsigned char smem_raw[];
 #pragma nounroll
   for (int k = 0; k < n_steps; ++k)
-    if (narrow_body(PersistArgs(&steps_g[k].n), smem_raw)) break;
+    if (narrow_body(PersistArgs<DynShape>(&steps_g[k].n), smem_raw)) break;
 }
 __global__ __launch_bounds__(kNarrowThreads) void persist_helper_kernel(const PersistStep *__restrict__ steps_g, int n_steps, int nH) {
   extern __shared__ __attribute__((aligned(16))) unsigned char smem_raw[];
diff --git a/tensornetworkforml_amd/csrc/san/hip_stub.cpp b/tensornetworkforml_amd/csrc/san/hip_stub.cpp
--- a/tensornetworkforml_amd/csrc/san/hip_stub.cpp
+++ b/tensornetworkforml_amd/csrc/san/hip_stub.cpp
@@ -26,6 +26,8 @@
 #define g_kernels kernel_map()
 #define g_launches launch_map()
 static long g_checked_ptrs = 0, g_allreduces = 0;
+static const PersistStep *g_last_persist = nullptr;
+static int g_last_persist_n = 0;
 static long g_alloc_calls = 0, g_fail_call = 0;
 static bool alloc_fails() {
   if (++g_alloc_calls != g_fail_call) return false;
@@ -426,7 +428,7 @@
   I(zr) I(s) I(g) I(L) I(h) I(l2_flag) P(W) V(lab) V(pl) P(Ng) P(T) P(TN) P(Z) P(prepRaw) P(prepB) P(prepG) P(Apub) P(flag) I(want)
   P(aflag) P(nflag) I(awant) P(zready) I(zwant) P(tcnt) P(pcnt) P(abort_flag) P(status) P(stamps)
 }
-static void tr_struct(const PersistStep &p) { tr(" n:"); tr_struct(p.n); tr(" w:"); tr_struct(p.w); tr(" t:"); tr_struct(p.t); }
+static void tr_struct(const PersistStep &p) { tr(" n:"); tr_struct(p.n); tr(" w:"); tr_struct(p.w); tr(" t:"); tr_struct(p.t); tr(" shape=%d", p.shape); }
 static void tr_struct(const PrepParams &p) { V(lab) V(pl) P(Nh) P(Ng) I(h) I(g) I(s) I(L) I(l2_flag) P(prepB) P(prepG) I(nparts) }
 static void tr_struct(const MeetParams &p) { P(Lenv) P(Renv) P(x) P(core) P(f) I(b) I(b_pad) I(ml) I(mr) I(D) I(L) I(rows_per_chunk) }
 static void tr_struct(const InputGradParams &p) {
@@ -538,6 +540,10 @@
     need(st, (size_t)(n + 1) * sizeof(PersistStep), "persistent step records");
     for (int k = 0; k < n; ++k) { check_narrow(st[k].n); check_pipe(st[k].w); scan(&st[k].t, sizeof st[k].t, "PersistHelperParams"); }
     check_pipe(st[n].w);
+    for (int k = 0; k <= n; ++k)
+      if (st[k].shape && (st[k].shape < 1 || st[k].shape > kNumPersistShapes || k == n || !has("sweep_persist_kernel<") || has("DynShape")))
+        die("record %d carries shape %d in a launch of %s", k, st[k].shape, name.c_str());
+    g_last_persist = st; g_last_persist_n = n;
   } else if (has("step_pipe_kernel")) {
     const NarrowParams &n = *(const NarrowParams *)args[0];
     const WidePipeParams &w = *(const WidePipeParams *)args[1];
@@ -776,4 +782,5 @@
 void san_stub_fail_alloc(long nth) { g_fail_call = nth > 0 ? g_alloc_calls + nth : 0; }
 int san_stub_fail_pending(void) { return g_fail_call != 0; }
 void san_stub_poke_int(void *dev, int v) { need(dev, 4, "poke"); memcpy(dev, &v, 4); }
-}
+const void *san_stub_last_persist(int *n_steps) { *n_steps = g_last_persist_n; return g_last_persist; }
+}
diff --git a/tensornetworkforml_amd/csrc/san/plan_shape_main.cpp b/tensornetworkforml_amd/csrc/san/plan_shape_main.cpp
--- /dev/null
+++ b/tensornetworkforml_amd/csrc/san/plan_shape_main.cpp
@@ -0,0 +1,153 @@
+#include <hip/hip_runtime.h>
+
+#include <cstdio>
+#include <cstdlib>
+#include <cstring>
+#include <fstream>
+#include <string>
+#include <vector>
+
+#include "../tnml_internal.h"
+#include "../wide_pipe_device.h"
+
+using namespace tnml;
+
+extern "C" void san_stub_report(void);
+extern "C" long san_stub_launches(const char *substr);
+extern "C" const void *san_stub_last_persist(int *n_steps);
+
+#define OK(call)                                                                              \
+  do {                                                                                        \
+    int rc_ = (call);                                                                         \
+    if (rc_ != TNML_OK) { fprintf(stderr, "%s:%d %s -> %d: %s\n", __FILE__, __LINE__, #call, rc_, tnml_last_error()); exit(1); } \
+  } while (0)
+#define CHECK(cond, ...)                                                                      \
+  do {                                                                                        \
+    if (!(cond)) { fprintf(stderr, "%s:%d %s: ", __FILE__, __LINE__, #cond); fprintf(stderr, __VA_ARGS__); fprintf(stderr, "\n"); exit(1); } \
+  } while (0)
+
+static int uniform_entry(const PersistStep &ps) {
+  const NarrowParams &n = ps.n;
+  const PersistHelperParams &t = ps.t;
+  for (int i = 0; i < kNumPersistShapes; ++i) {
+    const int H = kPersistShapes[i].H, L = kPersistShapes[i].L;
+    const bool update = n.D == kD && n.h == H && n.g == H && n.s == H && n.m == H && n.L == L && n.z_rows == kD * H && n.bsize == H * kD * kD * H * L;
+    const bool helper = t.h == H && t.g == H && t.s == H && t.L == L && t.zr == kD * H;
+    if (update && helper) return i + 1;
+  }
+  return 0;
+}
+
+static long g_marked = 0, g_records = 0;
+
+static int plan_chain(int N, int M, int L, int b, bool on, int mode) {
+  const int D = kD;
+  tnml_ctx *ctx = nullptr;
+  OK(tnml_create(&ctx, N, D, L, M, b, 0));
+  std::vector<int> bond(N - 1, M);
+  size_t total = 0;
+  for (int i = 0; i < N; ++i) total += (size_t)(i == 0 ? 1 : M) * D * (i == N - 1 ? 1 : M) * (i == 0 ? L : 1);
+  std::vector<float> cores(total);
+  for (size_t e = 0; e < total; ++e) cores[e] = 0.1f + 1e-3f * (float)(e % 97);
+  OK(tnml_set_cores(ctx, cores.data(), total, bond.data(), 0));
+  std::vector<float> X((size_t)b * N * D, 0.5f), f((size_t)L * b), met((size_t)2 * (N - 1));
+  std::vector<int> y(b);
+  for (int s = 0; s < b; ++s) y[s] = s % L;
+  OK(tnml_set_input(ctx, X.data(), y.data(), b));
+  OK(tnml_set_persistent(ctx, mode));
+  OK(tnml_set_shape_kernels(ctx, on ? 1 : 0));
+  int marked_all = 0;
+  for (int sw = 0; sw < 3; ++sw) {
+    OK(tnml_forward(ctx, f.data()));
+    const int left = tnml_l_pos(ctx) == N - 1;
+    const long before = san_stub_launches(mode == 1 ? "sweep_persist_kernel" : "persist_update_kernel");
+    OK(tnml_sweep(ctx, left, N - 1, 1, 1e-3f, 1e-3f, 1, TNML_ACT_SOFTMAX, TNML_LOSS_FULL_CROSS_ENT, 0.1f, TNML_TRUNC_FIXED, met.data(), f.data()));
+    CHECK(san_stub_launches(mode == 1 ? "sweep_persist_kernel" : "persist_update_kernel") == before + 1, "N %d bond %d sweep %d took another path", N, M, sw);
+    int n_steps = 0;
+    const PersistStep *st = (const PersistStep *)san_stub_last_persist(&n_steps);
+    CHECK(st && n_steps == N - 1, "records of %d steps", n_steps);
+    int marked = 0, launch_shape = 0;
+    for (int k = 0; k < n_steps; ++k) {
+      const int want = (on && mode == 1) ? uniform_entry(st[k]) : 0;
+      CHECK(st[k].shape == want, "N %d bond %d sweep %d step %d: shape %d, the record shows %d (h %d g %d s %d m %d L %d z_rows %d)", N, M, sw, k,
+            st[k].shape, want, st[k].n.h, st[k].n.g, st[k].n.s, st[k].n.m, st[k].n.L, st[k].n.z_rows);
+      if (st[k].shape) { ++marked; CHECK(!launch_shape || launch_shape == st[k].shape, "two shapes in one launch"); launch_shape = st[k].shape; }
+    }
+    CHECK(st[n_steps].shape == 0, "the prologue record is marked");
+    int said = -1;
+    OK(tnml_fixed_shape_steps(ctx, &said));
+    CHECK(said == marked, "tnml_fixed_shape_steps says %d, %d records are marked", said, marked);
+    marked_all += marked;
+    g_records += n_steps;
+  }
+  OK(tnml_destroy(ctx));
+  g_marked += marked_all;
+  printf("planned shapes N %d bond %d L %d switch %s mode %d: %d of %d steps marked\n", N, M, L, on ? "on" : "off", mode, marked_all, 3 * (N - 1));
+  fflush(stdout);
+  return marked_all;
+}
+
+static void constants_cannot_disagree() {
+  int tried = 0;
+  for (int i = 0; i < kNumPersistShapes; ++i) {
+    const int H = kPersistShapes[i].H, L = kPersistShapes[i].L;
+    int v[8] = {H, H, H, H, L, kD * H, H * kD * kD * H * L, kPersistHelpers};
+    CHECK(persist_step_shape(v[0], v[1], v[2], v[3], v[4], v[5], v[6], v[7]) == i + 1, "entry %d does not fit its own shape", i);
+    for (int j = 0; j < 8; ++j)
+      for (int d = -1; d <= 1; d += 2) {
+        int w[8];
+        memcpy(w, v, sizeof w);
+        w[j] += d;
+        CHECK(persist_step_shape(w[0], w[1], w[2], w[3], w[4], w[5], w[6], w[7]) != i + 1, "entry %d marks a step whose value %d is off by %d", i, j, d);
+        ++tried;
+      }
+  }
+  CHECK(persist_step_shape(1, 20, 20, 2, 2, 1, 160, kPersistHelpers) == 0 && persist_step_shape(5, 5, 5, 5, 3, 10, 300, kPersistHelpers) == 0, "a ramp step is marked");
+  printf("shape constants: %d disagreeing values refused\n", tried);
+}
+
+static std::vector<std::string> normalised(const char *path) {
+  std::ifstream in(path);
+  CHECK(in.good(), "cannot read %s", path);
+  std::vector<std::string> out;
+  for (std::string line; std::getline(in, line);) {
+    for (size_t at; (at = line.find(" shape=")) != std::string::npos;) {
+      size_t end = at + 7;
+      while (end < line.size() && line[end] >= '0' && line[end] <= '9') ++end;
+      line.erase(at, end - at);
+    }
+    const size_t k = line.find("sweep_persist_kernel<");
+    if (k != std::string::npos) {
+      const size_t open = k + 20, geo = line.find(" grid=", open);
+      if (geo != std::string::npos) line.erase(open, geo - open);
+    }
+    out.push_back(line);
+  }
+  return out;
+}
+
+int main(int argc, char **argv) {
+  const std::string what = argc > 1 ? argv[1] : "on";
+  if (what == "compare") {
+    CHECK(argc == 4, "compare needs two traces");
+    const auto a = normalised(argv[2]), b = normalised(argv[3]);
+    CHECK(a.size() == b.size() && a.size() > 100, "%zu and %zu lines", a.size(), b.size());
+    for (size_t i = 0; i < a.size(); ++i) CHECK(a[i] == b[i], "line %zu differs beyond the shape field:\n%.400s\n%.400s", i + 1, a[i].c_str(), b[i].c_str());
+    printf("shape traces: %zu lines equal apart from the shape field\n", a.size());
+    return 0;
+  }
+  const bool on = what == "on";
+  constants_cannot_disagree();
+  const int bonds[3] = {5, 10, 20};
+  for (int M : bonds) {
+    const int marked = plan_chain(24, M, 2, 64, on, 1);
+    CHECK((marked > 0) == (on && M != 5), "bond %d: %d steps marked", M, marked);
+  }
+  CHECK(plan_chain(24, 10, 3, 64, on, 1) == 0, "three labels are not in the table");
+  CHECK(plan_chain(24, 20, 2, 64, on, 2) == 0, "mode 2 has the generic kernels only");
+  plan_chain(784, 20, 2, 5000, on, 1);
+  printf("shape plans, switch %s: %ld of %ld records marked\n", on ? "on" : "off", g_marked, g_records);
+  san_stub_report();
+  printf("shape-kernel host planning under ASan + UBSan: ok\n");
+  return 0;
+}
diff --git a/tensornetworkforml_amd/csrc/tnml_api.hip b/tensornetworkforml_amd/csrc/tnml_api.hip
--- a/tensornetworkforml_amd/csrc/tnml_api.hip
+++ b/tensornetworkforml_amd/csrc/tnml_api.hip
@@ -216,6 +216,8 @@
     unsigned token = 0;
   } pipe;
   bool persist_enabled = true;
+  bool shape_kernels = true;
+  int fixed_steps = 0;
   PersistStep *pst_dev = nullptr, *pst_host[2] = {nullptr, nullptr};
   hipEvent_t pst_ev[2] = {nullptr, nullptr};
   int pst_cur = 0;
@@ -2185,6 +2187,16 @@
   if (lds > kLdsMax || lds_wide > kLdsMax || lds_help > kLdsMax) return give_up();
   const int persist_off = (int)((lds - pbytes) & ~(size_t)15);
   for (int k = 0; k < n_steps; ++k) st[k].n.persist_off = persist_off;
+  int shape = 0, n_fixed = 0;
+  if (c->shape_kernels && c->persist_mode < 2)
+    for (int k = 0; k < n_steps; ++k) {
+      const NarrowParams &n = st[k].n;
+      const PersistHelperParams &t = st[k].t;
+      const int id = persist_step_shape(n.h, n.g, n.s, n.m, n.L, n.z_rows, n.bsize, nH);
+      if (!id || (shape && id != shape) || n.D != kD) continue;
+      if (persist_step_shape(t.h, t.g, t.s, n.m, t.L, t.zr, n.bsize, nH) != id) continue;
+      shape = id; st[k].shape = id; ++n_fixed;
+    }
   HIP_TRY(hipMemcpyAsync(c->pst_dev, st, (size_t)(n_steps + 1) * sizeof(PersistStep), hipMemcpyHostToDevice, c->stream));
   HIP_TRY(hipEventRecord(c->pst_ev[buf], c->stream));
   c->pst_cur ^= 1;
@@ -2201,9 +2213,11 @@
     HIP_TRY(hipStreamWaitEvent(c->stream, c->ev_p2, 0));
     HIP_TRY(hipStreamWaitEvent(c->stream, c->ev_p3, 0));
   } else {
-    launch_sweep_persist(c->pst_dev, n_steps, nH, 1 + nH + nwide, lds, c->stream);
+    if (!launch_sweep_persist(c->pst_dev, n_steps, nH, 1 + nH + nwide, lds, c->stream, shape))
+      return fail(TNML_ERR_STATE, "no persistent sweep kernel for step shape %d", shape);
     HIP_TRY(hipGetLastError());
   }
+  c->fixed_steps = n_fixed;
   c->cnt_steps += n_steps; c->cnt_bytes += bytes; c->cnt_flops += flops;
   c->sweep_launches += 1; c->step_launches += n_steps; c->persist_sweeps += 1;
   c->Bnew_valid = true; c->f_current = true; drop_pregradients(c);
@@ -2848,6 +2862,18 @@
   return TNML_OK;
 }
 
+extern "C" int tnml_set_shape_kernels(tnml_ctx *c, int on) {
+  if (!c) return TNML_ERR_ARG;
+  c->shape_kernels = on != 0;
+  return TNML_OK;
+}
+
+extern "C" int tnml_fixed_shape_steps(tnml_ctx *c, int *n_steps) {
+  if (!c || !n_steps) return TNML_ERR_ARG;
+  *n_steps = c->fixed_steps;
+  return TNML_OK;
+}
+
 extern "C" int tnml_set_persistent(tnml_ctx *c, int on) {
   if (!c) return fail(TNML_ERR_ARG, "ctx is NULL");
   if (on < 0 || on > 2) return fail(TNML_ERR_ARG, "mode %d outside [0, 2]", on);
diff --git a/tensornetworkforml_amd/csrc/wide_pipe_device.h b/tensornetworkforml_amd/csrc/wide_pipe_device.h
--- a/tensornetworkforml_amd/csrc/wide_pipe_device.h
+++ b/tensornetworkforml_amd/csrc/wide_pipe_device.h
@@ -154,8 +154,30 @@
   int *status;
   double *stamps;
 };
-struct PersistStep { NarrowParams n; WidePipeParams w; PersistHelperParams t; };
+struct PersistStep { NarrowParams n; WidePipeParams w; PersistHelperParams t; int shape; int pad_; };
 constexpr int kPersistHelpers = 8;
+struct PersistShape { int H, L; };
+constexpr PersistShape kPersistShapes[] = {{10, 2}, {20, 2}};
+constexpr int kNumPersistShapes = (int)(sizeof(kPersistShapes) / sizeof(kPersistShapes[0]));
+template <int H, int LBL, int ID>
+struct FixedShape {
+  static constexpr int id = ID;
+  static constexpr int h = H, g = H, s = H, m = H, L = LBL, bsize = H * kD * kD * H * LBL, zr = kD * H, nH = kPersistHelpers;
+  static_assert(H >= 1 && H <= 64 && kD * H <= 64 && ((kD * H) & 1) == 0 && bsize <= 8192, "beyond the in-LDS persistent step");
+  template <class R> __device__ __forceinline__ void load_shape(const R *) {}
+  static constexpr bool fits(int h_, int g_, int s_, int m_, int L_, int z_rows_, int bsize_, int nH_) {
+    return h_ == h && g_ == g && s_ == s && m_ == m && L_ == L && z_rows_ == zr && bsize_ == bsize && nH_ == nH;
+  }
+};
+template <int I = 0>
+constexpr int persist_step_shape(int h, int g, int s, int m, int L, int z_rows, int bsize, int nH) {
+  if constexpr (I < kNumPersistShapes) {
+    return FixedShape<kPersistShapes[I].H, kPersistShapes[I].L, I + 1>::fits(h, g, s, m, L, z_rows, bsize, nH)
+               ? I + 1 : persist_step_shape<I + 1>(h, g, s, m, L, z_rows, bsize, nH);
+  } else {
+    return 0;
+  }
+}
 __host__ __device__ inline int persist_pub_off(int na, int h) { return ((na + 1) & ~1) + ((h + 1) & ~1); }
 __host__ __device__ inline size_t persist_pub_doubles(int na, int h) { return (size_t)persist_pub_off(na, h) + (((size_t)h * h + 1) & ~(size_t)1); }
 __host__ __device__ inline size_t persist_helper_ss_doubles(int zr, int h, int cw) {
@@ -171,7 +193,7 @@
                     ((size_t)zr * cw + (size_t)zr * h) * sizeof(float);
   return (p1 > p2 ? p1 : p2) + 64;
 }
-void launch_sweep_persist(const PersistStep *steps_dev, int n_steps, int n_helpers, int grid, size_t lds_bytes, hipStream_t st);
+bool launch_sweep_persist(const PersistStep *steps_dev, int n_steps, int n_helpers, int grid, size_t lds_bytes, hipStream_t st, int shape);
 void launch_sweep_persist_split(const PersistStep *steps_dev, int n_steps, int n_helpers, int n_wide, size_t lds_update, size_t lds_helper,
                                 size_t lds_wide, hipStream_t st_update, hipStream_t st_helper, hipStream_t st_wide);
 
```

New measurement: 22130 sweep-steps/s (median of 6 runs). 4.7% higher.
